# nowal/MASt3R-SLAM

Measured on AMD Instinct MI355X. Metric: keyframe-pair GN iters/sec @512×384, 256 edges; ATE-RMSE vs ref, higher is better.
Workload: dtype f32; 1 GPU; cfg3: gauss_newton_calib op call, 256 keyframe-pair edges (512 directed), 128 keyframes, 384x512, 10 GN iters/step, delta_thresh=0; edges=256, directed_edges=512, keyframes=128, H=384, W=512, parallelism=edge-sharded x1

## Files before the change

include/m3s_backend.h:

```cpp
#ifndef M3S_BACKEND_H
#define M3S_BACKEND_H

#include <stddef.h>
#include <stdint.h>

#ifdef __cplusplus
extern "C" {
#endif

enum {
    M3S_OK = 0,
    M3S_ERR_INVALID = 1,
    M3S_ERR_HIP = 2,
    M3S_ERR_WORKSPACE = 3,
    M3S_ERR_COMM = 4,
    M3S_ERR_TIMEOUT = 5
};

const char* m3s_last_error(void);
const char* m3s_version(void);
void m3s_shutdown(void);

enum {
    M3S_CONTRACT_NVCC = 0,
    M3S_CONTRACT_OFF = 1,
    M3S_CONTRACT_NVCC_RIGHT = 2,
    M3S_CONTRACT_DEFAULT = M3S_CONTRACT_NVCC
};

int m3s_iter_proj(const float* rays, const float* pts, const float* p_init,
                  float* p_new, uint8_t* converged,
                  int64_t B, int64_t H, int64_t W, int64_t N,
                  int max_iter, float lambda_init, float cost_thresh, void* stream);
int m3s_iter_proj_ex(const float* rays, const float* pts, const float* p_init,
                     float* p_new, uint8_t* converged,
                     int64_t B, int64_t H, int64_t W, int64_t N,
                     int max_iter, float lambda_init, float cost_thresh, int contract, void* stream);

int m3s_refine_matches_f16(const uint16_t* D11, const uint16_t* D21,
                           const int64_t* p1, int64_t* p1_new,
                           int64_t B, int64_t H, int64_t W, int64_t N, int64_t F,
                           int radius, int dilation_max, void* stream);
int m3s_refine_matches_f32(const float* D11, const float* D21,
                           const int64_t* p1, int64_t* p1_new,
                           int64_t B, int64_t H, int64_t W, int64_t N, int64_t F,
                           int radius, int dilation_max, void* stream);
int m3s_refine_matches_f64(const double* D11, const double* D21,
                           const int64_t* p1, int64_t* p1_new,
                           int64_t B, int64_t H, int64_t W, int64_t N, int64_t F,
                           int radius, int dilation_max, void* stream);

size_t m3s_match_workspace_bytes(int64_t B, int64_t H, int64_t W, int64_t F);
int m3s_match_iterative_proj(const float* X11, const float* X21, const float* D11, const float* D21,
                             const int64_t* idx_init, int64_t B, int64_t H, int64_t W, int64_t F,
                             int max_iter, float lambda_init, float cost_thresh, float dist_thresh,
                             int radius, int dilation_max, int contract, int64_t* idx_out,
                             uint8_t* valid_out, void* ws, size_t ws_bytes, void* stream);



void m3s_gn_debug_flags(int* out4);
void m3s_gn_pcg_stats(int* out5);
void m3s_gn_pcg_plan(int* out5);

int m3s_gn_check(void* stream);

enum { M3S_GN_POINTS = 0, M3S_GN_RAYS = 1, M3S_GN_CALIB = 2 };

typedef struct m3s_gn_args {
    int mode;
    float* Twc;
    const float* Xs;
    const float* Cs;
    const int64_t* ii;
    const int64_t* jj;
    const int64_t* idx;
    const uint8_t* valid;
    const float* Q;
    int64_t N, HW, E_total, E_local, edge_offset;
    float sigma0;
    float sigma1;
    float C_thresh, Q_thresh;
    const float* K;
    int height, width, pixel_border;
    float z_eps;
    int max_iter;
    float delta_thresh;
    float* dx;
    void* ws;
    size_t ws_bytes;
    void* comm;
    void* stream;
    int order;
    const int64_t* idx_b;
    const uint8_t* valid_b;
    const float* Q_b;
    int64_t E_a;
    int contract;
} m3s_gn_args;
enum {
    M3S_GN_ORDER_DEFAULT = 0,
    M3S_GN_ORDER_FAST = 1,
    M3S_GN_ORDER_REFERENCE = 2
};

size_t m3s_gn_workspace_bytes(int mode, int64_t N, int64_t HW, int64_t E_total, int64_t E_local);

int m3s_gauss_newton(const m3s_gn_args* args);

int m3s_gauss_newton_points(float* Twc, const float* Xs, const float* Cs,
                            const int64_t* ii, const int64_t* jj, const int64_t* idx,
                            const uint8_t* valid, const float* Q,
                            int64_t N, int64_t HW, int64_t E,
                            float sigma_point, float C_thresh, float Q_thresh,
                            int max_iter, float delta_thresh,
                            float* dx, void* ws, size_t ws_bytes, void* stream);
int m3s_gauss_newton_rays(float* Twc, const float* Xs, const float* Cs,
                          const int64_t* ii, const int64_t* jj, const int64_t* idx,
                          const uint8_t* valid, const float* Q,
                          int64_t N, int64_t HW, int64_t E,
                          float sigma_ray, float sigma_dist, float C_thresh, float Q_thresh,
                          int max_iter, float delta_thresh,
                          float* dx, void* ws, size_t ws_bytes, void* stream);
int m3s_gauss_newton_calib(float* Twc, const float* Xs, const float* Cs, const float* K,
                           const int64_t* ii, const int64_t* jj, const int64_t* idx,
                           const uint8_t* valid, const float* Q,
                           int64_t N, int64_t HW, int64_t E,
                           int height, int width, int pixel_border, float z_eps,
                           float sigma_pixel, float sigma_depth, float C_thresh, float Q_thresh,
                           int max_iter, float delta_thresh,
                           float* dx, void* ws, size_t ws_bytes, void* stream);

int m3s_gn_build_system(const m3s_gn_args* args, double* H_host, double* b_host);
int m3s_gn_edge_hessians(const m3s_gn_args* args, float* Hs_host, float* gs_host);

int m3s_gn_plan_info(const int64_t* ii, const int64_t* jj, int64_t E, int64_t N, int32_t* info,
                     int32_t* order, int32_t* round_ptr, int32_t round_cap);

int m3s_prof_begin(void);
int m3s_prof_begin_accum(void);
int m3s_prof_end(double* out , int* n_iter);
int m3s_prof_launch_ms(double* out, int cap);
int m3s_prof_solve_ms(double* out, int cap);


typedef struct m3s_track_args {
    int mode;
    const float* Xf;
    const float* Xk;
    const float* Qk;
    const uint8_t* valid;
    const float* meas_k;
    const uint8_t* valid_meas;
    const float* K;
    const float* T_WCf;
    const float* T_WCk;
    int64_t HW;
    int height, width, pixel_border;
    double z_eps;
    double sigma0;
    double sigma1;
    double huber_k;
    int max_iters;
    double rel_error, delta_norm;
    int check_every;
    float* T_WCf_out;
    float* T_CkCf_out;
    int* info;
    double* cost;
    void* ws;
    size_t ws_bytes;
    void* stream;
} m3s_track_args;

size_t m3s_track_workspace_bytes(int64_t HW);
int m3s_track_workspace_layout(int64_t HW, size_t* partials_offset, int* nblk, int* ld);
int m3s_track_sim3(const m3s_track_args* args);
int m3s_track_last_result(int32_t* info4, double* cost);


int m3s_edge_confidence(const int64_t* idx_i2j, const int64_t* idx_j2i,
                        const uint8_t* valid_match_j, const uint8_t* valid_match_i,
                        const float* Qii, const float* Qjj, const float* Qji, const float* Qij,
                        float Q_conf, int64_t B, int64_t HW, float* Qj, float* Qi, int* counts,
                        void* stream);


enum { M3S_FILTER_WEIGHTED_POINTMAP = 0, M3S_FILTER_INDEP_CONF = 1, M3S_FILTER_RECENT = 2 };

int m3s_pointmap_update(int mode, const float* T, const float* X_new, const float* C_new,
                        float* X, float* C, int64_t HW, void* stream);


typedef struct m3s_recon_args {
  const float* X;
  const float* C;
  const float* n_obs;
  const float* T_WC;
  const uint8_t* rgb;
  const float* K;
  int64_t N, HW;
  int height, width;
  float thresh;
  void* ws;
  size_t ws_bytes;
  void* stream;
} m3s_recon_args;
size_t m3s_recon_workspace_bytes(int64_t N, int64_t HW);
int64_t m3s_recon_tile_points(void);
int m3s_recon_count(const m3s_recon_args* args, int64_t* counts ,
                    int64_t* total );
int m3s_recon_emit(const m3s_recon_args* args, void* out , int64_t capacity);


enum { M3S_HEAD_TOKENS = 0, M3S_HEAD_PLANAR = 1 };
enum { M3S_HEAD_DEPTH_EXP = 0, M3S_HEAD_DEPTH_LINEAR = 1, M3S_HEAD_DEPTH_SQUARE = 2 };
enum { M3S_HEAD_CONF_EXP = 0, M3S_HEAD_CONF_SIGMOID = 1 };
enum { M3S_HEAD_DESC_NORM = 0 };
typedef struct m3s_head_args {
  const float* pts;
  const float* feat;
// ... 65 lines not shown
```

mast3r-slam_amd/csrc/edge_reduce.h:

```cpp
#pragma once

#include <hip/hip_runtime.h>

#include <cstdint>

#include "gn_kernels.h"

namespace m3s {

template <bool COH>
__device__ __forceinline__ void edge_reduce_body(const float* __restrict__ partials, int nchunks,
                                                 const float* __restrict__ Twc,
                                                 const int* __restrict__ ii_loc,
                                                 double* __restrict__ edgeblk, int e) {
    const int tid = threadIdx.x;
    auto ldp = [](const float* q) -> float {
        if constexpr (COH) return __hip_atomic_load(q, __ATOMIC_RELAXED, __HIP_MEMORY_SCOPE_AGENT);
        return *q;
    };
    __shared__ double M[7][7];
    __shared__ double g[7];
    __shared__ double A[7][7];
    __shared__ double AM[7][7];
    float Ti[8];
    if (tid < 3) {
        const float* Tp = Twc + (int64_t)ii_loc[e] * 8;
#pragma unroll
        for (int k = 0; k < 8; k++) Ti[k] = Tp[k];
    }
    if (tid < kNacc) {
        const float* p = partials + (int64_t)e * nchunks * kNaccPad + tid;
        double s = 0.0;
        int c = 0;
        for (; c + 8 <= nchunks; c += 8) {
            float v[8];
#pragma unroll
            for (int u = 0; u < 8; u++) v[u] = ldp(p + (int64_t)(c + u) * kNaccPad);
#pragma unroll
            for (int u = 0; u < 8; u++) s += (double)v[u];
        }
        for (; c < nchunks; c++) s += (double)ldp(p + (int64_t)c * kNaccPad);
        if (tid < 28) {
            int a = 0, r = tid;
            while (r >= 7 - a) { r -= 7 - a; a++; }
            const int b = a + r;
            M[a][b] = s;
            M[b][a] = s;
        } else {
            g[tid - 28] = s;
        }
    }
    if (tid < 49) A[tid / 7][tid % 7] = 0.0;
    __syncthreads();
    if (tid < 3) {
        const double t0 = Ti[0], t1 = Ti[1], t2 = Ti[2];
        const double qx = Ti[3], qy = Ti[4], qz = Ti[5], qw = Ti[6];
        const double s_inv = 1.0 / (double)Ti[7];
        double X[3] = {0, 0, 0};
        X[tid] = 1.0;
        const double uv0 = 2.0 * (qy * X[2] - qz * X[1]);
        const double uv1 = 2.0 * (qz * X[0] - qx * X[2]);
        const double uv2 = 2.0 * (qx * X[1] - qy * X[0]);
        const double R0 = X[0] + qw * uv0 + (qy * uv2 - qz * uv1);
        const double R1 = X[1] + qw * uv1 + (qz * uv0 - qx * uv2);
        const double R2 = X[2] + qw * uv2 + (qx * uv1 - qy * uv0);
        A[0][tid] = s_inv * R0;
        A[1][tid] = s_inv * R1;
        A[2][tid] = s_inv * R2;
        A[3][tid] = s_inv * (t1 * R2 - t2 * R1);
        A[4][tid] = s_inv * (t2 * R0 - t0 * R2);
        A[5][tid] = s_inv * (t0 * R1 - t1 * R0);
        A[6][tid] = s_inv * (t0 * R0 + t1 * R1 + t2 * R2);
        A[3][3 + tid] = R0;
        A[4][3 + tid] = R1;
        A[5][3 + tid] = R2;
        if (tid == 0) A[6][6] = 1.0;
    }
    __syncthreads();
    if (tid < 49) {
        const int a = tid / 7, b = tid % 7;
        double s = 0.0;
#pragma unroll
        for (int p = 0; p < 7; p++) s += A[a][p] * M[p][b];
        AM[a][b] = s;
    }
    __syncthreads();
    double* out = edgeblk + (int64_t)e * kEdgeBlk;
    if (tid < 28) {
        int a = 0, r = tid;
        while (r >= 7 - a) { r -= 7 - a; a++; }
        const int b = a + r;
        double s = 0.0;
#pragma unroll
        for (int p = 0; p < 7; p++) s += AM[a][p] * A[b][p];
        out[tid] = s;
    } else if (tid < 35) {
        const int a = tid - 28;
        double s = 0.0;
#pragma unroll
        for (int p = 0; p < 7; p++) s += A[a][p] * g[p];
        out[tid] = s;
    }
}

}
```

mast3r-slam_amd/csrc/gn_accum.hip:

```cpp
#include <hip/hip_runtime.h>

#include <algorithm>
#include <climits>
#include <cstdint>
#include <type_traits>

#include "edge_reduce.h"
#include "gn_kernels.h"
#include "sim3.h"
#include "wave_reduce.h"

namespace m3s {

__device__ __forceinline__ float vrcp(float a) { return __builtin_amdgcn_rcpf(a); }
__device__ __forceinline__ float vsqrt(float a) { return __builtin_amdgcn_sqrtf(a); }
__device__ __forceinline__ float vlog2(float a) { return __builtin_amdgcn_logf(a); }
__device__ __forceinline__ float sqrt_cr(float a) { return __builtin_sqrtf(a); }
__device__ __forceinline__ bool both(bool a, bool b) { return a && b; }

__device__ __forceinline__ float huber(float r) {
    const float a = fabsf(r);
    return a < 1.345f ? 1.0f : 1.345f * vrcp(a);
}

// ... 767 lines not shown
            put(r * 8u, 0, a);
        } else if constexpr (FIRST) {
            const uchar4 vm4 = ld_off<uchar4>(valid_c, r);
            const longlong2 id01 = ld_off<longlong2>(idx_c, r * 8u);
            const longlong2 id23 = ld_off<longlong2>(idx_c, r * 8u, 1);
            const float4 q4 = ld_off<float4>(Q_c, r * 4u);
            const float4 cj4 = raw.cj_all ? make_float4(0.f, 0.f, 0.f, 0.f) : ld_off<float4>(Cj_c, r * 4u);
            const bool vm[4] = {vm4.x != 0, vm4.y != 0, vm4.z != 0, vm4.w != 0};
            const int64_t ids[4] = {id01.x, id01.y, id23.x, id23.y};
            const float qs[4] = {q4.x, q4.y, q4.z, q4.w};
            const float cjs[4] = {cj4.x, cj4.y, cj4.z, cj4.w};
            int code[4], sqb[4];
#pragma unroll
            for (int s = 0; s < 4; s++) {
                const int ind = match_index(ids[s], vm[s], P.HW);
                const bool ok = vm[s] && (qs[s] > P.Q_thresh) && (raw.ci_all || raw.Ci_b[ind] > P.C_thresh) &&
                                (raw.cj_all || cjs[s] > P.C_thresh);
                code[s] = pack_code(ind, ok, P);
                sqb[s] = __float_as_int(sqrt_cr(qs[s]));
            }
            a = int4{code[0], sqb[0], code[1], sqb[1]};
            b = int4{code[2], sqb[2], code[3], sqb[3]};
            put(r * 8u, 0, a);
            put(r * 8u, 1, b);
        } else {
            a = ld_off<int4>(pk_c, r * 8u);
            if constexpr (NP == 4) b = ld_off<int4>(pk_c, r * 8u, 1);
        }
    };
    auto steps = [&](auto fixc_tag) {
        constexpr bool FIXC = decltype(fixc_tag)::value;
        int4 na = int4{0, 0, 0, 0}, nb = int4{0, 0, 0, 0};
        unsigned r = NP * threadIdx.x;
        if (r < n) {
            records(r, na, nb);
            if constexpr (FIXC) cur.fix_columns(k0 + (int)r, S / P.width);
        }
        auto step = [&](const int4& a, const int4& b, unsigned rr) {
            cur.set(a, b);
            cur.template load<MODE, FIXC>(Xj_c, Xi_b, Zi_b, rr, k0 + (int)rr);
            cur.template compute<MODE>(T, P, acc);
        };
        int4 ma = int4{0, 0, 0, 0}, mb = int4{0, 0, 0, 0};
        if constexpr (FIRST && NP == 4) {
            while (r < n) {
                step(na, nb, r);
                r += S;
                if (r < n) records(r, na, nb);
            }
        } else
        while (r < n) {
            if (r + S < n) records(r + S, ma, mb);
            step(na, nb, r);
            r += S;
            if (r >= n) break;
            if (r + S < n) records(r + S, na, nb);
            step(ma, mb, r);
            r += S;
        }
    };
    if constexpr (RC) {
        if (S % P.width == 0)
            steps(std::true_type{});
        else
            steps(std::false_type{});
    } else {
        steps(std::false_type{});
    }
}

struct FirstSrc {
    EdgeSrc es;
    const float* Cs;
    const int* cok;
    int4* pack_w;
};

template <int MODE, bool COMPACT, bool RCOK = false, bool FIRST = false>
__global__ __launch_bounds__(kAccThreads) void gn_accum_packed_kernel(
    const float* __restrict__ Twc, const float* __restrict__ Xs, const float* __restrict__ Zs,
    const int* __restrict__ ii_loc, const int* __restrict__ jj_loc, const int4* __restrict__ pack,
    AccParams P, const int4* __restrict__ sched, float* __restrict__ partials,
    const int* __restrict__ flags, const float* __restrict__ px, const int* __restrict__ pcnt,
    int* __restrict__ ecnt, double* __restrict__ edgeblk, FirstSrc fs) {
    const int4 tk = sched[blockIdx.x];
    if (flags[kFlagDone]) return;
    const int e = tk.x, c = tk.y, ix = tk.z, jx = tk.w;
    const RelXf T = rel_xf(rel_sim3(load_sim3(Twc + (int64_t)ix * 8), load_sim3(Twc + (int64_t)jx * 8)));

    const int HW = P.HW;
    const int64_t ebase = (int64_t)e * HW;
    const float* __restrict__ Xi_b = Xs + (int64_t)ix * HW * 3;
    const float* __restrict__ Zi_b = MODE == GN_CALIB ? inv_depths(Zs, P) + (int64_t)ix * HW : nullptr;
    const float* __restrict__ Xj_b = Xs + (int64_t)jx * HW * 3;
    const int4* __restrict__ pk_b = pack + ebase / 2;
    const int k0 = c * P.chunk;
    const int k1 = min(k0 + P.chunk, HW);

    float acc[kNacc];
#pragma unroll
    for (int q = 0; q < kNacc; q++) acc[q] = 0.0f;
    if constexpr (COMPACT) {
        const int64_t cb = ((int64_t)e * P.nchunks + c) * P.chunk;
        accum_steps<MODE, false, acc_np<MODE>()>(px + cb * 3, Xi_b, Zi_b, pack + cb / 2, 0, pcnt[(int64_t)e * P.nchunks + c], T, P,
                                 Zs, acc);
    } else {
        RawSrc raw{};
        if constexpr (FIRST) {
            fs.es.at(e, HW, raw.idx, raw.valid, raw.Q);
            raw.Ci_b = fs.Cs + (int64_t)ix * HW;
            raw.Cj_b = fs.Cs + (int64_t)jx * HW;
            raw.pk_w = fs.pack_w + ebase / 2;
            raw.ci_all = fs.cok != nullptr && fs.cok[ix] != 0;
            raw.cj_all = fs.cok != nullptr && fs.cok[jx] != 0;
        }
        constexpr int NP = acc_np<MODE>();
        bool ray = false;
        if constexpr (RCOK && MODE == GN_CALIB) {
            ray = flags[kFlagNotRay] == 0 && (P.width & 3) == 0;
            if (ray) accum_steps<MODE, true, NP, FIRST>(Zs + (int64_t)jx * HW, Xi_b, Zi_b, pk_b, k0, k1, T, P, Zs, acc, raw);
        }
        if (!ray) accum_steps<MODE, false, NP, FIRST>(Xj_b, Xi_b, Zi_b, pk_b, k0, k1, T, P, Zs, acc, raw);
    }
    block_partial(acc, partials + ((int64_t)e * P.nchunks + c) * kNaccPad, ecnt != nullptr);
    if (ecnt != nullptr) {
        __shared__ int s_last;
        asm volatile("s_waitcnt vmcnt(0)" ::: "memory");
        __syncthreads();
        if (threadIdx.x == 0)
            s_last = __hip_atomic_fetch_add(ecnt + e, 1, __ATOMIC_RELAXED, __HIP_MEMORY_SCOPE_AGENT) == P.nchunks - 1;
        __syncthreads();
        if (s_last) {
            edge_reduce_body<true>(partials, P.nchunks, Twc, ii_loc, edgeblk, e);
            if (threadIdx.x == 0) __hip_atomic_store(ecnt + e, 0, __ATOMIC_RELAXED, __HIP_MEMORY_SCOPE_AGENT);
        }
    }
}

hipError_t launch_accum(int mode, bool vec, dim3 grid, hipStream_t st, const float* Twc,
                        const float* Xs, const float* Cs, const int* ii_loc, const int* jj_loc,
                        const EdgeSrc& es, const AccParams& P, const int4* sched, float* partials,
                        const int* flags) {
#define M3S_ACC(MODE, V)                                                                    \
    hipLaunchKernelGGL((gn_accum_kernel<MODE, V>), grid, dim3(kAccThreads), 0, st, Twc, Xs, \
                       Cs, ii_loc, jj_loc, es, P, sched, partials, flags)
    if (mode == GN_RAYS) {
        if (vec) M3S_ACC(GN_RAYS, true); else M3S_ACC(GN_RAYS, false);
    } else if (mode == GN_CALIB) {
        if (vec) M3S_ACC(GN_CALIB, true); else M3S_ACC(GN_CALIB, false);
    } else {
        if (vec) M3S_ACC(GN_POINTS, true); else M3S_ACC(GN_POINTS, false);
    }
#undef M3S_ACC
    return hipGetLastError();
}

hipError_t launch_pack_pre(hipStream_t st, const float* Xs, int64_t N, const float* Cs, const AccParams& P, int* cok,
                           float* Zs, int* flags, const float* K) {
    if (cok != nullptr && N > 0) {
        const int bx = (int)std::max<int64_t>(1, std::min<int64_t>((P.HW + 1023) / 1024, 8192 / std::max<int64_t>(N, 1)));
        hipLaunchKernelGGL(gn_cpass_kernel, dim3(bx, (unsigned)N), dim3(256), 0, st, Cs, P, cok, flags);
    }
    if (Zs) {
        const int64_t total = N * (int64_t)P.HW;
        const int bx = (int)std::max<int64_t>(std::min<int64_t>((P.HW + 255) / 256,
                                                                std::max<int64_t>(8192 / std::max<int64_t>(N, 1), 2)),
                                              (std::max(P.width, P.height) + 255) / 256);
        hipLaunchKernelGGL(gn_depth_kernel, dim3(bx, (unsigned)N), dim3(256), 0, st, Xs, total, Zs, P, flags, K);
    }
    return hipGetLastError();
}

hipError_t launch_pack(int mode, hipStream_t st, int E_local, const float* Xs, int64_t N, const float* Cs,
                       const int* ii_loc, const int* jj_loc, const EdgeSrc& es, const AccParams& P, int* cok,
                       int4* pack, float* px, int* pcnt, const int* flags, bool skip_pack) {
    if (E_local > 0 && px) {
        const dim3 grid((unsigned)P.nchunks, (unsigned)E_local);
        int2* pk = reinterpret_cast<int2*>(pack);
        if (mode == GN_RAYS)
            hipLaunchKernelGGL(gn_pack_compact_kernel<GN_RAYS>, grid, dim3(kAccThreads), 0, st, Xs, Cs, ii_loc,
                               jj_loc, es, P, pk, px, pcnt, flags);
        else if (mode == GN_CALIB)
            hipLaunchKernelGGL(gn_pack_compact_kernel<GN_CALIB>, grid, dim3(kAccThreads), 0, st, Xs, Cs, ii_loc,
                               jj_loc, es, P, pk, px, pcnt, flags);
        else
            hipLaunchKernelGGL(gn_pack_compact_kernel<GN_POINTS>, grid, dim3(kAccThreads), 0, st, Xs, Cs, ii_loc,
                               jj_loc, es, P, pk, px, pcnt, flags);
    } else if (E_local > 0) {
        const dim3 grid((unsigned)((P.HW / 4 + kAccThreads - 1) / kAccThreads), (unsigned)E_local);
        if (!skip_pack)
            hipLaunchKernelGGL(gn_pack_kernel, grid, dim3(kAccThreads), 0, st, Cs, ii_loc, jj_loc, es,
                               P, cok, pack, flags);
    }
    return hipGetLastError();
}

hipError_t launch_accum_packed(int mode, dim3 grid, hipStream_t st, const float* Twc,
                               const float* Xs, const float* Zs, const int* ii_loc,
                               const int* jj_loc, const int4* pack, const AccParams& P,
                               const int4* sched, float* partials, const int* flags, const float* px,
                               const int* pcnt, int* ecnt, double* edgeblk, const EdgeSrc* first_es,
                               const float* Cs, const int* cok) {
    if (P.HW > kPackedMaxHW) return hipErrorInvalidValue;
    if (first_es != nullptr) {
        if (px != nullptr) return hipErrorInvalidValue;
        const FirstSrc fs{*first_es, Cs, cok, const_cast<int4*>(pack)};
        if (mode == GN_RAYS)
            hipLaunchKernelGGL((gn_accum_packed_kernel<GN_RAYS, false, false, true>), grid, dim3(kAccThreads), 0, st,
                               Twc, Xs, Zs, ii_loc, jj_loc, pack, P, sched, partials, flags, px, pcnt, ecnt,
                               edgeblk, fs);
        else if (mode == GN_POINTS)
            hipLaunchKernelGGL((gn_accum_packed_kernel<GN_POINTS, false, false, true>), grid, dim3(kAccThreads), 0, st,
                               Twc, Xs, Zs, ii_loc, jj_loc, pack, P, sched, partials, flags, px, pcnt, ecnt,
                               edgeblk, fs);
        else if (P.raycheck)
            hipLaunchKernelGGL((gn_accum_packed_kernel<GN_CALIB, false, true, true>), grid, dim3(kAccThreads), 0, st,
                               Twc, Xs, Zs, ii_loc, jj_loc, pack, P, sched, partials, flags, px, pcnt, ecnt,
                               edgeblk, fs);
        else
            hipLaunchKernelGGL((gn_accum_packed_kernel<GN_CALIB, false, false, true>), grid, dim3(kAccThreads), 0, st,
                               Twc, Xs, Zs, ii_loc, jj_loc, pack, P, sched, partials, flags, px, pcnt, ecnt,
                               edgeblk, fs);
        return hipGetLastError();
    }
    const FirstSrc fs0{};
#define M3S_ACCP(MODE, CP, RC)                                                                       \
    hipLaunchKernelGGL((gn_accum_packed_kernel<MODE, CP, RC>), grid, dim3(kAccThreads), 0, st, Twc, Xs, Zs, \
                       ii_loc, jj_loc, pack, P, sched, partials, flags, px, pcnt, ecnt, edgeblk, fs0)
#define M3S_ACCP2(MODE, CP) M3S_ACCP(MODE, CP, false)
    const bool cp = px != nullptr;
    if (mode == GN_RAYS) {
        if (cp) M3S_ACCP2(GN_RAYS, true); else M3S_ACCP2(GN_RAYS, false);
    } else if (mode == GN_CALIB) {
        if (cp) M3S_ACCP2(GN_CALIB, true);
        else if (P.raycheck) M3S_ACCP(GN_CALIB, false, true);
        else M3S_ACCP2(GN_CALIB, false);
    } else {
        if (cp) M3S_ACCP2(GN_POINTS, true); else M3S_ACCP2(GN_POINTS, false);
    }
#undef M3S_ACCP2
#undef M3S_ACCP
    return hipGetLastError();
}

}
```

mast3r-slam_amd/csrc/gn_api.hip:

```cpp
#include <hip/hip_runtime.h>

#include <algorithm>
#include <cstdarg>
#include <cstdio>
#include <cstdlib>
#include <cstring>
#include <mutex>
#include <string>
#include <utility>
#include <vector>

#include "gn_host.h"

namespace m3s {

namespace {
thread_local std::string g_err;
}

int g_dbg_flags[4] = {0, 0, 0, 0};
int g_dbg_pcg[5] = {0, 0, 0, 0, 0};
int g_dbg_pcg_plan[5] = {0, 0, 0, 0, 0};

void set_error(const char* fmt, ...) {
    char buf[1024];
    va_list ap;
    va_start(ap, fmt);
    vsnprintf(buf, sizeof(buf), fmt, ap);
    va_end(ap);
    g_err = buf;
}

const char* get_error() { return g_err.c_str(); }

namespace {
struct HostResources {
    std::mutex mu;
    std::vector<std::pair<void*, void (*)(void*)>> items;
    bool shut = false;
};
HostResources& host_resources() {
    static HostResources* r = new HostResources;
    return *r;
}
}

void register_host_resource(void* obj, void (*release)(void*)) {
    HostResources& r = host_resources();
    std::lock_guard<std::mutex> lk(r.mu);
    r.items.emplace_back(obj, release);
}

hipEvent_t Prof::get() {
    if (pool.empty()) {
        static const bool sysfence = env_int("M3S_PROF_SYSFENCE", 0) != 0;
        hipEvent_t e;
        if (sysfence || hipEventCreateWithFlags(&e, hipEventDisableSystemFence) != hipSuccess) {
            (void)hipGetLastError();
            if (hipEventCreate(&e) != hipSuccess) return nullptr;
        }
        return e;
    }
    hipEvent_t e = pool.back();
    pool.pop_back();
    return e;
}

void Prof::mark(hipStream_t st, bool accum, bool first_pack) {
    if (!on || (accum_only && !accum)) return;
    hipEvent_t e = get();
    if (e && hipEventRecord(e, st) == hipSuccess) {
        marks.push_back(e);
        if (accum_only && marks.size() % 2 == 0) first.push_back(first_pack);
    }
}

Prof g_prof;
namespace {
std::vector<double> g_prof_launch_ms;
std::vector<double> g_prof_solve_ms;
}

}

using namespace m3s;

extern "C" const char* m3s_last_error(void) { return m3s::get_error(); }

extern "C" int m3s_gn_check(void* stream) {
    const hipError_t e = hipStreamSynchronize(static_cast<hipStream_t>(stream));
    if (e != hipSuccess) {
        set_error("gn_check: %s", hipGetErrorString(e));
        return M3S_ERR_HIP;
    }
    return m3s::take_deferred_timeout("");
}

extern "C" void m3s_gn_debug_flags(int* out4) {
    for (int k = 0; k < 4; k++) out4[k] = m3s::g_dbg_flags[k];
}

extern "C" void m3s_gn_pcg_stats(int* out5) {
    for (int k = 0; k < 5; k++) out5[k] = m3s::g_dbg_pcg[k];
}

extern "C" void m3s_gn_pcg_plan(int* out5) {
    for (int k = 0; k < 5; k++) out5[k] = m3s::g_dbg_pcg_plan[k];
}

extern "C" const char* m3s_version(void) { return "m3s 0.1.0 gfx950"; }

extern "C" void m3s_shutdown(void) {
    HostResources& r = host_resources();
    std::lock_guard<std::mutex> lk(r.mu);
    if (r.shut) return;
    r.shut = true;
    for (auto& it : r.items) it.second(it.first);
    r.items.clear();
}

namespace {
__attribute__((constructor)) void m3s_register_shutdown() { std::atexit(m3s_shutdown); }
}

extern "C" size_t m3s_gn_workspace_bytes(int mode, int64_t N, int64_t HW, int64_t E_total,
                                         int64_t E_local) {
    if (N < 1 || HW < 1 || E_total < 0 || E_local < 0) return 0;
    return make_layout(mode, N, HW, E_total, E_local).total;
}

extern "C" int m3s_gn_plan_info(const int64_t* ii, const int64_t* jj, int64_t E, int64_t N, int32_t* info,
                                int32_t* order, int32_t* round_ptr, int32_t round_cap) {
    return m3s::plan_info(ii, jj, E, N, info, order, round_ptr, round_cap);
}

extern "C" int m3s_gauss_newton(const m3s_gn_args* args) {
    if (!args) {
        set_error("gauss_newton: null args");
        return M3S_ERR_INVALID;
    }
    return run(*args);
}

namespace {
int ref_edge_records(const m3s_gn_args& a0, Ctx& c, std::vector<float>& rec) {
    m3s_gn_args a = a0;
    a.order = M3S_GN_ORDER_REFERENCE;
    int rc = setup(a, c);
    if (rc) return rc;
    rec.assign((size_t)a.E_local * kRefStride, 0.0f);
    if (a.E_local == 0) return M3S_OK;
    const Layout& L = c.L;
    M3S_HIP_CHECK(launch_accum_ref(a.mode, (int)a.E_local, c.st, a.Twc, a.Xs, a.Cs, c.at<int>(L.ii_loc),
                                   c.at<int>(L.jj_loc), c.es, c.R, c.at<float>(L.edgeblk),
                                   c.at<int>(L.flags)));
    M3S_HIP_CHECK(hipMemcpyAsync(rec.data(), c.at<float>(L.edgeblk), sizeof(float) * rec.size(),
                                 hipMemcpyDeviceToHost, c.st));
    M3S_HIP_CHECK(hipStreamSynchronize(c.st));
    return M3S_OK;
}

double ref_block(const float* D, int blk, int r, int cc) {
    switch (blk) {
        case 0:
        case 3: return (double)D[std::max(r, cc) * 7 + std::min(r, cc)];
        case 1: return -(double)D[cc * 7 + r];
        default: return -(double)D[r * 7 + cc];
    }
}
}

extern "C" int m3s_gn_edge_hessians(const m3s_gn_args* args, float* Hs_host, float* gs_host) {
    if (!args || !Hs_host || !gs_host) {
        set_error("gn_edge_hessians: null argument");
        return M3S_ERR_INVALID;
    }
    Ctx c;
    std::vector<float> rec;
    int rc = ref_edge_records(*args, c, rec);
    if (rc) return rc;
    const int64_t E = args->E_local;
    for (int64_t e = 0; e < E; e++) {
        const float* D = rec.data() + e * kRefStride;
        for (int blk = 0; blk < 4; blk++)
            for (int r = 0; r < 7; r++)
                for (int q = 0; q < 7; q++)
                    Hs_host[((blk * E + e) * 7 + r) * 7 + q] = (float)ref_block(D, blk, r, q);
        for (int q = 0; q < 7; q++) {
            gs_host[(0 * E + e) * 7 + q] = -D[49 + q];
            gs_host[(1 * E + e) * 7 + q] = D[49 + q];
        }
    }
    return M3S_OK;
}

extern "C" int m3s_gn_build_system(const m3s_gn_args* args, double* H_host, double* b_host) {
    if (!args) {
        set_error("gn_build_system: null args");
        return M3S_ERR_INVALID;
    }
    const m3s_gn_args& a = *args;
    if (gn_order(a) == M3S_GN_ORDER_REFERENCE) {
        Ctx c;
        std::vector<float> rec;
        int rc = ref_edge_records(a, c, rec);
        if (rc) return rc;
        const int64_t n = 7 * (a.N - 1);
        std::fill(H_host, H_host + n * n, 0.0);
        std::fill(b_host, b_host + n, 0.0);
        for (int64_t el = 0; el < a.E_local; el++) {
            const float* D = rec.data() + el * kRefStride;
            const int i = c.plan.ii_loc[el] - 1, j = c.plan.jj_loc[el] - 1;
            const int rr[4] = {i, i, j, j}, cc[4] = {i, j, i, j};
            for (int blk = 0; blk < 4; blk++) {
                if (rr[blk] < 0 || cc[blk] < 0) continue;
                for (int r = 0; r < 7; r++)
// ... 177 lines not shown
```

mast3r-slam_amd/csrc/gn_driver.hip:

```cpp
#include <hip/hip_runtime.h>

#include <algorithm>
#include <chrono>
#include <cstdio>
#include <cstring>
#include <mutex>

#include "gn_host.h"
#include "m3s_comm.h"

namespace m3s {

namespace {
void keep_pool() {
    static std::mutex mu;
    static bool done[64] = {false};
    int dev = 0;
    if (hipGetDevice(&dev) != hipSuccess || dev < 0 || dev >= 64) return;
    std::lock_guard<std::mutex> lk(mu);
    if (done[dev]) return;
    done[dev] = true;
    const long mb = env_int("M3S_POOL_KEEP_MB", 1024);
    if (mb <= 0) return;
    hipMemPool_t pool;
// ... 38 lines not shown
    auto al16 = [](const void* ptr) { return ((uintptr_t)ptr & 15) == 0; };
    const bool two = a.idx_b != nullptr;
    c.es.idx[0] = a.idx;
    c.es.valid[0] = a.valid;
    c.es.Q[0] = a.Q;
    c.es.idx[1] = two ? a.idx_b : a.idx;
    c.es.valid[1] = two ? a.valid_b : a.valid;
    c.es.Q[1] = two ? a.Q_b : a.Q;
    c.es.E_a = two ? (int)a.E_a : (int)a.E_local;
    c.vec = (a.HW % 4 == 0) && al16(a.Xs) && al16(a.Cs) && al16(a.idx) && al16(a.valid) &&
            al16(a.Q) && (!two || (al16(a.idx_b) && al16(a.valid_b) && al16(a.Q_b)));
    const int pack_mode = env_int("M3S_GN_PACK", 1);
    c.packed = c.vec && a.E_local > 0 && (pack_mode == 2 || (pack_mode == 1 && a.max_iter >= 3)) &&
               a.HW <= kPackedMaxHW;
    c.compact = c.packed && env_int("M3S_GN_COMPACT", 0) != 0;
    if (a.mode == M3S_GN_CALIB && (a.width >= 65536 || a.height >= 32768)) c.packed = c.compact = false;
    P.pack_uv = c.packed && a.mode == M3S_GN_CALIB;
    P.raycheck = c.packed && !c.compact && a.mode == M3S_GN_CALIB && env_int("M3S_GN_RAYCHECK", 1) != 0;

    c.ref_order = gn_order(a) == M3S_GN_ORDER_REFERENCE;
    if (c.ref_order) {
        c.packed = false;
        RefParams& R = c.R;
        R.s0_inv = (float)(1.0 / (double)a.sigma0);
        R.s1_inv = (a.mode == M3S_GN_POINTS) ? 0.0f : (float)(1.0 / (double)a.sigma1);
        R.C_thresh = a.C_thresh;
        R.Q_thresh = a.Q_thresh;
        R.z_eps = a.z_eps;
        R.width = a.width > 0 ? a.width : 1;
        R.height = a.height;
        R.pixel_border = a.pixel_border;
        R.HW = a.HW;
        R.variant = env_int("M3S_GN_REF_VARIANT", 0);
        R.contract = a.contract;
    }
    int* dflags = c.at<int>(L.flags);
    int* dcok = c.at<int>(L.cok);
    auto pre_pass = [&]() -> int {
        M3S_HIP_CHECK(launch_gn_init(c.st, dflags, P.raycheck ? 0 : 1, dcok, a.N));
        if (c.packed)
            M3S_HIP_CHECK(launch_pack_pre(c.st, a.Xs, a.N, a.Cs, P, !c.compact ? dcok : nullptr,
                                          a.mode == M3S_GN_CALIB ? c.at<float>(L.zs) : nullptr, dflags,
                                          a.mode == M3S_GN_CALIB ? a.K : nullptr));
        return M3S_OK;
    };
    static const bool prepass_early = env_int("M3S_PREPASS", 1) != 0;
    rc = build_plan(a, c.st, c.plan, prepass_early ? pre_pass : std::function<int()>());
    if (!rc && !prepass_early) rc = pre_pass();
    if (rc) return rc;
    if (c.plan.gather)
        M3S_HIP_CHECK(hipMallocAsync((void**)&c.eall,
                                     sizeof(double) * kEdgeBlk * (size_t)c.plan.granks * c.plan.gchunk, c.st));
    const auto s1 = std::chrono::steady_clock::now();
    const Plan& p = c.plan;
    P.fx = p.K[0];
    P.fy = p.K[1];
    P.cx = p.K[2];
    P.cy = p.K[3];
    if (c.ref_order) {
        c.R.fx = p.K[0];
        c.R.fy = p.K[1];
        c.R.cx = p.K[2];
        c.R.cy = p.K[3];
    }
    const size_t ntask = (size_t)a.E_local * L.nchunks;
    const size_t lo = L.ii_loc, hi = L.sched;
    const size_t nslot = c.need_slotmap ? p.slotmap.size() : 0;
    if (c.need_slotmap) {
        rc = c.alloc_dense(L.npad, (int)std::max<int64_t>(a.N - 1, 0));
        if (rc) return rc;
    }
    char* h = stagings().ws.get(hi - lo + sizeof(int) * nslot);
    M3S_REQUIRE(h != nullptr, "gauss_newton: pinned host allocation failed");
    auto put = [&](size_t off, const std::vector<int>& v) {
        if (!v.empty()) std::memcpy(h + (off - lo), v.data(), sizeof(int) * v.size());
    };
    put(L.ii_loc, p.ii_loc);
    put(L.jj_loc, p.jj_loc);
    put(L.blk_ptr, p.blk_ptr);
    put(L.blk_ent, p.blk_ent);
    put(L.blk_ref, p.blk_ref);
    put(L.grad_ptr, p.grad_ptr);
    put(L.grad_ent, p.grad_ent);
    std::memset(h + (L.ecnt - lo), 0, sizeof(int) * (size_t)a.E_local);
    SchedGroups G;
    build_schedule_order(p.ii_loc, p.jj_loc, (int)std::max<int64_t>(a.N, 1), reinterpret_cast<int*>(h + (L.sorder - lo)), G);
    M3S_HIP_CHECK(stagings().ws.upload(c.ws + lo, h, L.sched - lo, c.st));
    M3S_HIP_CHECK(launch_sched_expand(c.st, c.at<int>(L.sorder), c.at<int>(L.ii_loc), c.at<int>(L.jj_loc), L.nchunks,
                                      G, (int64_t)ntask, c.at<int>(L.sched)));
    c.first_pack = early_pack && c.packed && !c.compact && !c.ref_order && a.max_iter > 0 &&
                   env_int("M3S_GN_PACK_FIRST", 1) != 0;
    if (early_pack) {
        rc = prepare_iterations(a, c);
        if (rc) return rc;
        c.pack_issued = true;
    }
    const auto s2 = std::chrono::steady_clock::now();
    if (nslot) {
        std::memcpy(h + (hi - lo), p.slotmap.data(), sizeof(int) * nslot);
        M3S_HIP_CHECK(hipMemcpyAsync(c.dyn + c.o_slot, h + (hi - lo), sizeof(int) * nslot,
                                     hipMemcpyHostToDevice, c.st));
    }
    M3S_HIP_CHECK(stagings().ws.mark(c.st));
    if (prof_host) {
        auto us = [](std::chrono::steady_clock::time_point x, std::chrono::steady_clock::time_point y) {
            return std::chrono::duration<double, std::micro>(y - x).count();
        };
        fprintf(stderr, "gn host: build_plan %.0f us (of which copies + sync %.0f us), params+lists+schedule+pack "
                "%.0f us, rest %.0f us\n", us(s0, s1), g_plan_sync_us, us(s1, s2), us(s2, std::chrono::steady_clock::now()));
    }
    return M3S_OK;
}

int take_deferred_timeout(const char* which) {
    Stagings& sg = stagings();
    if (!sg.tmo_armed) return M3S_OK;
    const int kind = sg.tmo_armed;
    sg.tmo_armed = 0;
    const char* h = sg.tmo.get(64);
    const bool hit = kind == 2 ? *reinterpret_cast<const double*>(h) > 0.0 : *reinterpret_cast<const int*>(h) != 0;
    if (hit) {
        set_error("gauss_newton: %sa device-side wait of the factorisation timed out (the solve was "
                  "discarded; not a singular system)", which);
        return M3S_ERR_TIMEOUT;
    }
    return M3S_OK;
}

int run(const m3s_gn_args& a) {
    static const bool prof_host = env_int("M3S_PROF_HOST", 0) != 0;
    auto now = [] { return std::chrono::steady_clock::now(); };
    auto us = [](std::chrono::steady_clock::time_point x, std::chrono::steady_clock::time_point y) {
        return std::chrono::duration<double, std::micro>(y - x).count();
    };
    const auto t0 = now();
    Ctx c;
    c.need_slotmap = env_int("M3S_SOLVER_DENSE", 0) != 0;
    int rc = setup(a, c, a.N > 1);
    if (rc) return rc;
    rc = take_deferred_timeout("an earlier call: ");
    if (rc) return rc;
    const auto t1 = now();
    const int npose = (int)(a.N - 1);
    if (npose <= 0) return M3S_OK;
    const Layout& L = c.L;
    int* flags = c.at<int>(L.flags);
    std::chrono::steady_clock::time_point t2 = t1, t3 = t1;
    if (!c.ref_order && a.max_iter > 0 && env_int("M3S_EARLY_ACC", 1) != 0) {
        g_prof.mark(c.st);
        rc = enqueue_accumulate(a, c);
        if (rc) return rc;
        c.acc_enqueued = true;
        static const int early_gather = env_int("M3S_EARLY_GATHER", -1);
        if (c.plan.gather && (early_gather > 0 || (early_gather < 0 && comm_is_async(a.comm)))) {
            rc = comm_allgather_f64(a.comm, c.eall, (size_t)c.plan.gchunk * kEdgeBlk, c.st);
            if (rc) return rc;
            c.gathered = true;
        }
    }
    const auto t1b = now();
    if (env_int("M3S_SOLVER_DENSE", 0) == 0 || c.ref_order) {
        choose_sparse_plan(c.plan, npose, c.sp);
        choose_pcg(a, c, c.plan, npose, c.sp);
        t2 = now();
        M3S_REQUIRE(c.sp.npad_tail <= kMaxNpad,
                    "gauss_newton: the dense core of the elimination (%d unknowns) exceeds the "
                    "dense solve limit (%d)", c.sp.npad_tail, kMaxNpad);
        rc = upload_sparse_plan(c.sp, npose, c.st);
        if (rc) return rc;
        t3 = now();
    }
    if (prof_host)
        fprintf(stderr, "gn host: setup %.0f us, early enqueue %.0f us, plan %.0f us, upload %.0f us\n", us(t0, t1),
                us(t1, t1b), us(t1b, t2), us(t2, t3));
    for (int itr = 0; itr < a.max_iter; itr++) {
        if (!c.acc_enqueued) g_prof.mark(c.st);
        rc = enqueue_system(a, c);
        if (rc) return rc;
        g_prof.mark(c.st);
        if (itr == 0) M3S_HIP_CHECK(launch_twc_save(c.st, a.Twc, c.at<float>(L.twc_save), (int)(8 * a.N)));
        const int from = c.sp.pcg_from, lag = c.sp.pcg_lag;
        if (c.sp.pcg && itr >= from) {
            if (c.inv_pending) {
                M3S_HIP_CHECK(hipStreamWaitEvent(c.st, c.inv_done, 0));
                c.inv_pending = false;
            }
            rc = enqueue_pcg(a, c);
            if (rc) return rc;
        }
        rc = enqueue_solve(a, c, c.sp.pcg && itr >= from);
        if (rc) return rc;
        g_prof.mark(c.st);
        if (!c.sp.fused && !c.sp.hybrid)
            M3S_HIP_CHECK(launch_retract(c.st, a.Twc, c.at<double>(L.x), a.dx, (int)a.N,
                                         a.delta_thresh, flags, a.contract));
        if (c.sp.pcg && (itr == from - lag || itr >= from) && itr + 1 < a.max_iter) {
            rc = enqueue_inverse(a, c, itr < from - 1);
            if (rc) return rc;
        }
        g_prof.mark(c.st);
    }
    if (c.may_timeout && a.max_iter > 0) {
        Stagings& sg = stagings();
        char* h = sg.tmo.get(64);
        M3S_REQUIRE(h != nullptr, "gauss_newton: pinned host allocation failed");
        float* save = c.at<float>(L.twc_save);
        const int n8 = (int)(8 * a.N);
        if (a.comm) {
            double* dv = c.at<double>(L.x);
            M3S_HIP_CHECK(launch_flag_export(c.st, flags + kFlagTimeout, dv, 1));
            rc = comm_allreduce_sum_f64(a.comm, dv, 1, c.st);
            if (rc) return rc;
            M3S_HIP_CHECK(launch_twc_restore_on_flag(c.st, a.Twc, save, n8, dv, 1, sg.tmo.dev));
            if (!sg.tmo.dev) M3S_HIP_CHECK(hipMemcpyAsync(h, dv, sizeof(double), hipMemcpyDeviceToHost, c.st));
            sg.tmo_armed = 2;
        } else {
            M3S_HIP_CHECK(launch_twc_restore_on_flag(c.st, a.Twc, save, n8, flags + kFlagTimeout, 0, sg.tmo.dev));
            if (!sg.tmo.dev)
                M3S_HIP_CHECK(hipMemcpyAsync(h, flags + kFlagTimeout, sizeof(int), hipMemcpyDeviceToHost, c.st));
            sg.tmo_armed = 1;
        }
        M3S_HIP_CHECK(sg.tmo.mark(c.st));
        static const bool sync_report = env_int("M3S_GN_TIMEOUT_SYNC", 0) != 0;
        if (sync_report) {
            rc = take_deferred_timeout("");
            if (rc) return rc;
        }
    }
    if (const int dbg = env_int("M3S_GN_DEBUG_FLAGS", 0)) {
        int hf[kNumFlags];
        M3S_HIP_CHECK(hipMemcpyAsync(hf, flags, sizeof(hf), hipMemcpyDeviceToHost, c.st));
        M3S_HIP_CHECK(hipStreamSynchronize(c.st));
        g_dbg_flags[0] = hf[kFlagDone];
        g_dbg_flags[1] = (hf[kFlagFail] | hf[kFlagFailed]) != 0;
        g_dbg_flags[2] = c.packed ? 1 : 0;
        g_dbg_flags[3] = (c.packed && c.P.raycheck && hf[kFlagNotRay] == 0) ? 1 : 0;
        g_dbg_pcg[0] = hf[kFlagPcgRuns];
        g_dbg_pcg[1] = hf[kFlagPcgSteps];
        g_dbg_pcg[2] = hf[kFlagPcgFall];
        g_dbg_pcg[3] = c.sp.pcg ? 1 : 0;
        g_dbg_pcg[4] = c.sp.pcg ? c.sp.pcg_from : 0;
        g_dbg_pcg_plan[0] = c.sp.pcg ? c.sp.pcg_R : 0;
        g_dbg_pcg_plan[1] = c.sp.pcg ? c.sp.pcg_nwg : 0;
        g_dbg_pcg_plan[2] = c.sp.pcg && c.sp.pcg_onex ? 1 : 0;
        g_dbg_pcg_plan[3] = c.sp.pcg ? c.sp.pcg_lag : 0;
        g_dbg_pcg_plan[4] = c.sp.pcg ? c.sp.pcg_nitem : 0;
        if (dbg != 2)
            fprintf(stderr, "gn flags: done %d fail %d not_ray %d timeout %d packed %d pcg runs %d steps %d fallbacks %d\n",
                    hf[kFlagDone], g_dbg_flags[1], hf[kFlagNotRay], hf[kFlagTimeout], (int)c.packed,
                    hf[kFlagPcgRuns], hf[kFlagPcgSteps], hf[kFlagPcgFall]);
    }
    return M3S_OK;
}

}
```

mast3r-slam_amd/csrc/gn_enqueue.hip:

```cpp
#include <hip/hip_runtime.h>

#include <algorithm>
#include <cstdio>
#include <cstdlib>

#include "gn_host.h"
#include "m3s_comm.h"

namespace m3s {

namespace {
struct PcgSide {
    static constexpr int kMaxDev = 64;
    hipStream_t ss[kMaxDev] = {};
    hipEvent_t e1[kMaxDev] = {}, e2[kMaxDev] = {};
    static void release(void* p) {
        PcgSide* s = static_cast<PcgSide*>(p);
        for (int d = 0; d < kMaxDev; d++) {
            if (s->e1[d]) (void)hipEventDestroy(s->e1[d]);
            if (s->e2[d]) (void)hipEventDestroy(s->e2[d]);
            if (s->ss[d]) (void)hipStreamDestroy(s->ss[d]);
            s->e1[d] = s->e2[d] = nullptr;
            s->ss[d] = nullptr;
        }
    }
};
thread_local PcgSide* t_pcg_side = nullptr;
int pcg_side(hipStream_t& ss, hipEvent_t& e1, hipEvent_t& e2) {
    if (!t_pcg_side) {
        t_pcg_side = new PcgSide;
        register_host_resource(t_pcg_side, &PcgSide::release);
    }
    int dev = 0;
    M3S_HIP_CHECK(hipGetDevice(&dev));
    M3S_REQUIRE(dev >= 0 && dev < PcgSide::kMaxDev, "gauss_newton: device %d out of range", dev);
    PcgSide& p = *t_pcg_side;
    if (!p.ss[dev]) {
        M3S_HIP_CHECK(hipStreamCreateWithFlags(&p.ss[dev], hipStreamNonBlocking));
        M3S_HIP_CHECK(hipEventCreateWithFlags(&p.e1[dev], hipEventDisableTiming | hipEventDisableSystemFence));
        M3S_HIP_CHECK(hipEventCreateWithFlags(&p.e2[dev], hipEventDisableTiming | hipEventDisableSystemFence));
    }
    ss = p.ss[dev];
    e1 = p.e1[dev];
    e2 = p.e2[dev];
    return M3S_OK;
}
}

int prepare_iterations(const m3s_gn_args& a, Ctx& c) {
    if (!c.packed) return M3S_OK;
    const Layout& L = c.L;
    M3S_HIP_CHECK(launch_pack(a.mode, c.st, (int)a.E_local, a.Xs, a.N, a.Cs, c.at<int>(L.ii_loc),
                              c.at<int>(L.jj_loc), c.es, c.P, c.at<int>(L.cok), c.at<int4>(L.pack),
                              c.compact ? c.at<float>(L.packx) : nullptr, c.at<int>(L.pcnt),
                              c.at<int>(L.flags), c.first_pack));
    return M3S_OK;
}

int enqueue_system(const m3s_gn_args& a, Ctx& c) {
    const Layout& L = c.L;
    int* flags = c.at<int>(L.flags);
    const int npose_r = (int)(a.N - 1);
    if (c.ref_order) {
        M3S_REQUIRE(c.sp.enabled, "gauss_newton: the reference order needs the block-sparse solver");
        g_prof.mark(c.st, true);
        M3S_HIP_CHECK(launch_accum_ref(a.mode, (int)a.E_local, c.st, a.Twc, a.Xs, a.Cs,
                                       c.at<int>(L.ii_loc), c.at<int>(L.jj_loc), c.es,
                                       c.R, c.at<float>(L.edgeblk), flags));
        g_prof.mark(c.st, true);
        SparsePlan& sp = c.sp;
        double* sys = sp.dptr<double>(sp.o_sys);
        M3S_HIP_CHECK(launch_assemble_ref(c.st, c.at<float>(L.edgeblk), c.at<int>(L.blk_ptr),
                                          c.at<int>(L.blk_ref), c.at<int>(L.grad_ptr),
                                          c.at<int>(L.grad_ent), c.plan.nblk, sp.nblocks, npose_r,
                                          sp.bpad, sys, flags));
        if (a.comm) {
            const size_t count = (size_t)sp.bpad + (size_t)c.plan.nblk * 49;
            int rc = comm_allreduce_sum_f64(a.comm, sys, count, c.st);
            if (rc) return rc;
        }
        return M3S_OK;
    }
    if (!c.acc_enqueued) {
        int rc = enqueue_accumulate(a, c);
        if (rc) return rc;
    }
    c.acc_enqueued = false;
    return enqueue_assembly(a, c);
}

int enqueue_accumulate(const m3s_gn_args& a, Ctx& c) {
    const Layout& L = c.L;
    int* flags = c.at<int>(L.flags);
    if (a.E_local > 0) {
        g_prof.mark(c.st, true);
        const dim3 grid((unsigned)(L.nchunks * a.E_local));
        const bool fuse_reduce = env_int("M3S_GN_FUSE_REDUCE", 1) != 0;
        const bool fused = c.packed && fuse_reduce;
        const bool was_first = c.packed && c.first_pack;
        if (c.packed) {
            M3S_HIP_CHECK(launch_accum_packed(a.mode, grid, c.st, a.Twc, a.Xs, c.at<float>(L.zs),
                                              c.at<int>(L.ii_loc), c.at<int>(L.jj_loc),
                                              c.at<int4>(L.pack), c.P, c.at<int4>(L.sched),
                                              c.at<float>(L.partials), flags,
                                              c.compact ? c.at<float>(L.packx) : nullptr,
                                              c.at<int>(L.pcnt), fused ? c.at<int>(L.ecnt) : nullptr,
                                              c.eblk(), c.first_pack ? &c.es : nullptr,
                                              a.Cs, c.at<int>(L.cok)));
            c.first_pack = false;
        } else
            M3S_HIP_CHECK(launch_accum(a.mode, c.vec, grid, c.st, a.Twc, a.Xs, a.Cs,
                                       c.at<int>(L.ii_loc), c.at<int>(L.jj_loc), c.es, c.P,
                                       c.at<int4>(L.sched), c.at<float>(L.partials),
                                       flags));
        g_prof.mark(c.st, true, was_first);
        if (!fused)
            M3S_HIP_CHECK(launch_edge_reduce((int)a.E_local, c.st, c.at<float>(L.partials), L.nchunks,
                                             a.Twc, c.at<int>(L.ii_loc), c.eblk(), flags));
    }
    return M3S_OK;
}

int enqueue_assembly(const m3s_gn_args& a, Ctx& c) {
    const Layout& L = c.L;
    int* flags = c.at<int>(L.flags);
    const int npose = (int)(a.N - 1);
    if (c.plan.gather && !c.gathered) {
        int rc = comm_allgather_f64(a.comm, c.eall, (size_t)c.plan.gchunk * kEdgeBlk, c.st);
        if (rc) return rc;
    }
    c.gathered = false;
    const bool reduce = a.comm && !c.plan.gather;
    if (c.sp.enabled) {
        SparsePlan& sp = c.sp;
        double* sys = sp.dptr<double>(sp.o_sys);
        M3S_HIP_CHECK(launch_assemble(c.st, c.eblk_all(), c.at<int>(L.blk_ptr),
                                      c.at<int>(L.blk_ent), c.at<int>(L.grad_ptr),
                                      c.at<int>(L.grad_ent), c.plan.nblk, sp.nblocks, npose, sp.bpad,
                                      sys, flags));
        if (reduce) {
            const size_t count = (size_t)sp.bpad + (size_t)c.plan.nblk * 49;
            int rc = comm_allreduce_sum_f64(a.comm, sys, count, c.st);
            if (rc) return rc;
        }
        return M3S_OK;
    }
    M3S_HIP_CHECK(launch_compact(c.st, c.eblk_all(), c.at<int>(L.blk_ptr),
                                 c.at<int>(L.blk_ent), c.at<int>(L.grad_ptr),
                                 c.at<int>(L.grad_ent), c.plan.nblk, npose,
                                 c.at<double>(L.compact), flags));
    if (reduce) {
        const size_t count = (size_t)c.plan.nblk * 28 + (size_t)npose * 7;
        int rc = comm_allreduce_sum_f64(a.comm, c.at<double>(L.compact), count, c.st);
        if (rc) return rc;
    }
    return M3S_OK;
}

namespace {
constexpr int kSolveDbgWords = kSolveDbgCycles + 1;
unsigned long long* solve_dbg_buffer() {
    static unsigned long long* p = nullptr;
    if (p == nullptr && hipMalloc(&p, sizeof(unsigned long long) * kSolveDbgWords) != hipSuccess) p = nullptr;
    if (p != nullptr) (void)hipMemset(p, 0, sizeof(unsigned long long) * kSolveDbgWords);
    return p;
}
hipError_t launch_gn_solve_dbg(hipStream_t st, const SolveArgs& S) {
    hipError_t e = launch_gn_solve(st, S);
    if (e != hipSuccess || !S.debug || S.dbg == nullptr) return e;
    unsigned long long h[kSolveDbgWords];
    e = hipMemcpyAsync(h, S.dbg, sizeof(h), hipMemcpyDeviceToHost, st);
    if (e == hipSuccess) e = hipStreamSynchronize(st);
    if (e == hipSuccess) print_solve_debug(h);
    return e;
}
}

int enqueue_solve(const m3s_gn_args& a, Ctx& c, bool fallback) {
    const Layout& L = c.L;
    const int npose = (int)(a.N - 1);
    int* flags = c.at<int>(L.flags);
    if (!c.sp.enabled) {
        c.may_timeout = true;
        M3S_HIP_CHECK(launch_solve(c.st, c.at<double>(L.compact), c.dyn_at<int>(c.o_slot), c.plan.nblk,
                                   npose, 7 * npose, L.npad, c.dyn_at<double>(c.o_dense),
                                   c.dyn_at<double>(c.o_linv), c.at<double>(L.x), flags, ++c.chol_epoch));
        return M3S_OK;
    }
    SparsePlan& sp = c.sp;
    SolveArgs S{};
    S.npose = npose;
    S.b = sp.dptr<double>(sp.o_sys);
    S.A = S.b + sp.bpad;
    S.y = sp.dptr<double>(sp.o_y);
    S.Lstore = sp.dptr<double>(sp.o_L);
    S.W = sp.dptr<double>(sp.o_W);
    S.Lg = sp.dptr<double>(sp.o_Lg);
    S.x = c.at<double>(L.x);
    S.meta = sp.iptr(0);
    S.nmeta = (int)sp.nints;
    S.meta_lds = solve_lds_bytes(S.nmeta) <= (size_t)kSolveMaxLds && env_int("M3S_SOLVE_META_LDS", 1);
    S.o_rounds = (int)sp.i_rounds;
    S.o_nodes = (int)sp.i_nodes;
    S.o_fptr = (int)sp.i_fptr;
    S.o_fronts = (int)sp.i_fronts;
    S.o_tg = (int)sp.i_tg;
    S.o_tc = (int)sp.i_tc;
    S.o_rtg = (int)sp.i_rtg;
    S.o_rc = (int)sp.i_rc;
    S.o_tail = (int)sp.i_tail;
    S.o_tmap = (int)sp.i_tmap;
    S.nrounds = (int)sp.rounds.size();
    S.zero_blk = sp.zero_blk;
    S.ntail = sp.ntail;
// ... 38 lines not shown
        }
        S.do_fwd = S.do_tail = S.do_back = 1;
        M3S_HIP_CHECK(launch_gn_solve_dbg(c.st, S));
        return M3S_OK;
    }
    double* A = S.A;
    double* b = S.b;
    double* y = S.y;
    double* Ls = S.Lstore;
    double* W = S.W;
    double* x = S.x;
    static const int df_mode = env_int("M3S_SOLVE_DF", 1);
    const bool df = df_mode == 2 || (df_mode == 1 && fallback);
    if (df) {
        c.may_timeout = true;
        SpRoundsArgs ca{};
        ca.inl = sp.iptr(sp.i_inl);
        ca.tc3 = sp.iptr(sp.i_tc3);
        ca.rc4 = sp.iptr(sp.i_rc4);
        ca.rounds = sp.iptr(sp.i_rounds);
        ca.tmap = sp.iptr(sp.i_tmap);
        ca.tail = sp.iptr(sp.i_tail);
        ca.A = A;
        ca.b = b;
        ca.Lstore = Ls;
        ca.W = W;
        ca.y = y;
        ca.Hd = sp.ntail > 0 ? sp.dptr<double>(sp.o_dense) : nullptr;
        ca.flags = flags;
        ca.nrounds = (int)sp.rounds.size();
        ca.ntail = sp.ntail;
        ca.npad = sp.npad_tail;
        M3S_HIP_CHECK(launch_sp_rounds_df(c.st, ca, sp.dptr<int>(sp.o_dfcnt)));
    } else {
        for (const SpRound& R : sp.rounds)
            M3S_HIP_CHECK(launch_sp_round(c.st, sp.iptr(sp.i_inl), R.tbeg + R.rbeg, R.nbt, R.nrt,
                                          sp.iptr(sp.i_tc3), sp.iptr(sp.i_rc4), A, b, Ls, W, y, flags));
    }
    const bool core_df = sp.core_df;
    if (sp.hybrid && core_df && sp.ntail > 0) {
        c.may_timeout = true;
        if (!df)
            M3S_HIP_CHECK(launch_sp_tail_fill(c.st, A, b, sp.iptr(sp.i_tmap), sp.iptr(sp.i_tail), sp.ntail,
                                              sp.npad_tail, sp.dptr<double>(sp.o_dense), flags));
        M3S_HIP_CHECK(launch_dense_factor_solve(c.st, sp.npad_tail, sp.dptr<double>(sp.o_dense),
                                                sp.dptr<double>(sp.o_linv), sp.dptr<double>(sp.o_xd), flags,
                                                ++c.chol_epoch));
        S.xd = sp.dptr<double>(sp.o_xd);
        S.Hd = nullptr;
        S.nmeta = (int)sp.nints_back;
        S.meta_lds = 1;
        S.do_fwd = 0;
        S.do_tail = 0;
        S.do_back = 1;
        S.x_tail_global = 1;
        M3S_HIP_CHECK(launch_gn_solve_dbg(c.st, S));
        return M3S_OK;
    }
    if (sp.hybrid) {
        M3S_REQUIRE(sp.fused_tail, "gauss_newton: a %d-pose hybrid core exceeds the in-register factorisation",
                    sp.ntail);
        if (!df)
            M3S_HIP_CHECK(launch_sp_tail_fill(c.st, A, b, sp.iptr(sp.i_tmap), sp.iptr(sp.i_tail),
                                              sp.ntail, sp.npad_tail, sp.dptr<double>(sp.o_dense), flags));
        S.Hd = sp.ntail > 0 ? sp.dptr<double>(sp.o_dense) : nullptr;
        S.npad_h = sp.npad_tail;
        S.nmeta = (int)sp.nints_back;
        S.meta_lds = 1;
        S.do_fwd = 0;
        S.do_tail = S.do_back = 1;
        M3S_HIP_CHECK(launch_gn_solve_dbg(c.st, S));
        return M3S_OK;
    }
    if (sp.ntail > 0) c.may_timeout = true;
    M3S_HIP_CHECK(launch_sp_tail(c.st, A, b, sp.iptr(sp.i_tmap), sp.iptr(sp.i_tail), sp.ntail,
                                 sp.npad_tail, sp.dptr<double>(sp.o_dense), sp.dptr<double>(sp.o_linv),
                                 sp.dptr<double>(sp.o_xd), x, flags, ++c.chol_epoch, !df));
    for (auto it = sp.rounds.rbegin(); it != sp.rounds.rend(); ++it)
        M3S_HIP_CHECK(launch_sp_back(c.st, it->nnodes, sp.iptr(sp.i_nodes), sp.iptr(sp.i_fptr),
                                     sp.iptr(sp.i_fronts), it->node_begin, Ls, W, y, x, flags));
    return M3S_OK;
}

int enqueue_inverse(const m3s_gn_args& a, Ctx& c, bool snapshot) {
    const SparsePlan& sp = c.sp;
    const size_t shift = snapshot ? sp.o_snap - sp.o_L : 0;
    if (snapshot) {
        M3S_REQUIRE(sp.snap_bytes > 0, "PCG: no factor snapshot buffer");
        M3S_HIP_CHECK(hipMemcpyAsync(sp.dbuf + sp.o_snap, sp.dbuf + sp.o_L, sp.snap_bytes, hipMemcpyDeviceToDevice, c.st));
    }
    InvArgs v{};
    v.n = 7 * (int)(a.N - 1);
    v.ldx = sp.pcg_ldx;
    v.nrounds = (int)sp.rounds.size();
    v.ntail = sp.ntail;
    v.npad = sp.npad_tail;
    v.rounds = sp.iptr(sp.i_rounds);
    v.nodes = sp.iptr(sp.i_nodes);
    v.fptr = sp.iptr(sp.i_fptr);
    v.fronts = sp.iptr(sp.i_fronts);
    v.inl = sp.iptr(sp.i_inl);
    v.rc4 = sp.iptr(sp.i_rc4);
    v.tail = sp.iptr(sp.i_tail);
    v.Lstore = sp.dptr<double>(sp.o_L + shift);
    v.W = sp.dptr<double>(sp.o_W + shift);
    v.Hd = sp.dptr<double>(sp.o_dense + shift);
    v.Linv = sp.dptr<double>(sp.o_linv + shift);
    v.X = sp.dptr<double>(sp.o_pcgx);
    v.Xt = sp.dptr<float>(sp.o_pcgxt);
    v.ldt = sp.pcg_ldt;
    v.flags = c.at<int>(c.L.flags);
    static const bool side = env_int("M3S_PCG_SIDE", 1) != 0;
    if (!side) {
        M3S_HIP_CHECK(launch_sp_inverse(c.st, v));
        return M3S_OK;
    }
    hipStream_t ss;
    hipEvent_t e1, e2;
    int rc = pcg_side(ss, e1, e2);
    if (rc) return rc;
    M3S_HIP_CHECK(hipEventRecord(e1, c.st));
    M3S_HIP_CHECK(hipStreamWaitEvent(ss, e1, 0));
    static const bool dbg = env_int("M3S_PCG_DEBUG", 0) != 0;
    hipEvent_t t0 = nullptr, t1 = nullptr;
    static long long* ibuf = nullptr;
    if (dbg && !ibuf && hipMalloc(&ibuf, sizeof(long long) * 8) != hipSuccess) ibuf = nullptr;
    v.dbg = dbg ? ibuf : nullptr;
    if (dbg) {
        if (ibuf) M3S_HIP_CHECK(hipMemsetAsync(ibuf, 0, sizeof(long long) * 8, ss));
        M3S_HIP_CHECK(hipEventCreate(&t0));
        M3S_HIP_CHECK(hipEventCreate(&t1));
        M3S_HIP_CHECK(hipEventRecord(t0, ss));
    }
    M3S_HIP_CHECK(launch_sp_inverse(ss, v));
    if (dbg) {
        M3S_HIP_CHECK(hipEventRecord(t1, ss));
        M3S_HIP_CHECK(hipEventSynchronize(t1));
        float ms = 0.f;
        M3S_HIP_CHECK(hipEventElapsedTime(&ms, t0, t1));
        long long h[8] = {0};
        if (ibuf) M3S_HIP_CHECK(hipMemcpy(h, ibuf, sizeof(h), hipMemcpyDeviceToHost));
        fprintf(stderr, "pcg inverse (M refresh): %.1f us, %d workgroups; wg0: init %.1f fwd rounds %.1f core %.1f back rounds %.1f f32 copy %.1f us\n",
                ms * 1e3, (v.n + 15) / 16, (h[1] - h[0]) * 0.01, (h[2] - h[1]) * 0.01, (h[3] - h[2]) * 0.01,
                (h[4] - h[3]) * 0.01, (h[5] - h[4]) * 0.01);
        (void)hipEventDestroy(t0);
        (void)hipEventDestroy(t1);
    }
    M3S_HIP_CHECK(hipEventRecord(e2, ss));
    c.inv_pending = true;
    c.inv_done = e2;
    return M3S_OK;
}

int enqueue_pcg(const m3s_gn_args& a, Ctx& c) {
    const SparsePlan& sp = c.sp;
    PcgArgs g{};
    g.b = sp.dptr<double>(sp.o_sys);
    g.A = g.b + sp.bpad;
    g.adj_ptr = sp.iptr(sp.i_apt);
    g.adj = reinterpret_cast<const int2*>(sp.iptr(sp.i_adj));
    g.nitem = sp.pcg_nitem;
    g.R4 = pcg_r4(sp.pcg_R);
    g.Xt = sp.dptr<float>(sp.o_pcgxt);
    g.ldt = sp.pcg_ldt;
    g.n = 7 * (int)(a.N - 1);
    g.nv = sp.pcg_nv;
    g.onex = sp.pcg_onex ? 1 : 0;
    g.R = sp.pcg_R;
    g.nwg = sp.pcg_nwg;
    g.gran = reinterpret_cast<unsigned long long*>(sp.dbuf + sp.o_gran);
    static const int kmax = std::max(1, std::min(200, env_int("M3S_PCG_KMAX", 30)));
    static const double tol = [] {
        const char* e = getenv("M3S_PCG_TOL");
        return e ? atof(e) : 1e-6;
    }();
    g.kmax = kmax;
    g.tol2 = tol * tol;
    g.tag0 = 1u + (unsigned)c.pcg_launches * (unsigned)(2 * kmax + 2);
    c.pcg_launches++;
    const char* ft = getenv("M3S_TEST_FORCE_TIMEOUT");
    g.spin_limit = (ft && atoi(ft) != 0) ? 0 : (1 << 22);
    g.Twc = a.Twc;
    g.dx = a.dx;
    g.N = (int)a.N;
    g.delta_thresh = a.delta_thresh;
    g.contract = a.contract;
    g.flags = c.at<int>(c.L.flags);
    static const bool dbg = env_int("M3S_PCG_DEBUG", 0) != 0;
    static long long* dbuf = nullptr;
    if (dbg && !dbuf && hipMalloc(&dbuf, sizeof(long long) * kPcgDbgSlots) != hipSuccess) dbuf = nullptr;
    if (dbg && dbuf) M3S_HIP_CHECK(hipMemsetAsync(dbuf, 0, sizeof(long long) * kPcgDbgSlots, c.st));
    g.dbg = dbg ? dbuf : nullptr;
    M3S_HIP_CHECK(launch_pcg(c.st, g));
    if (g.dbg) {
        long long h[kPcgDbgSlots];
        M3S_HIP_CHECK(hipMemcpyAsync(h, dbuf, sizeof(h), hipMemcpyDeviceToHost, c.st));
// ... 16 lines not shown
```

mast3r-slam_amd/csrc/gn_host.h:

```cpp
#pragma once

#include <hip/hip_runtime.h>

#include <algorithm>
#include <cstdint>
#include <functional>
#include <utility>
#include <vector>

#include "../../include/m3s_backend.h"
#include "gn_kernels.h"
#include "m3s_common.h"
#include "sparse_plan.h"

namespace m3s {

int env_int(const char* name, int dflt);

inline size_t align_up(size_t x, size_t a) { return (x + a - 1) / a * a; }

struct Prof {
    bool on = false;
    std::vector<hipEvent_t> pool;
    std::vector<hipEvent_t> marks;
    hipEvent_t get();
    bool accum_only = false;
    std::vector<char> first;
    void mark(hipStream_t st, bool accum = false, bool first_pack = false);
};
extern Prof g_prof;

extern int g_dbg_flags[4];
extern int g_dbg_pcg[5];
extern int g_dbg_pcg_plan[5];

struct Staging {
    char* buf = nullptr;
    char* dev = nullptr;
    size_t cap = 0;
    hipEvent_t done = nullptr;
    bool pending = false;
    static void release(void* p);
    char* get(size_t bytes);
    hipError_t upload(void* dst, const char* h, size_t bytes, hipStream_t st);
    hipError_t download(char* h, const void* src, size_t bytes, hipStream_t st);
    hipError_t mark(hipStream_t st);
};
struct Stagings {
    Staging in;
    Staging out;
    Staging ws;
    Staging tmo;
    int tmo_armed = 0;
    static void release(void* p);
};
Stagings& stagings();

struct Layout {
    size_t partials, edgeblk, compact, x, flags, ii_loc, jj_loc, blk_ptr, blk_ent, blk_ref, grad_ptr,
        grad_ent, ecnt, cok, sorder, sched, pack, packx, pcnt, zs, twc_save, total;
    int nchunks, npad, nblk_max;
};
Layout make_layout(int mode, int64_t N, int64_t HW, int64_t E_total, int64_t E_local);
int chunk_points(int64_t HW, int nchunks);

struct Plan {
    int nblk = 0;
    std::vector<int> ii_loc, jj_loc;
    std::vector<int> blk_ptr, blk_ent;
    std::vector<int> blk_ref;
    std::vector<int> grad_ptr, grad_ent;
    std::vector<int> slotmap;
    std::vector<std::pair<int, int>> pairs;
    float K[4] = {0, 0, 0, 0};
    bool gather = false;
    int grank = 0, granks = 1, gchunk = 0;
};

Plan& tls_plan();
SparsePlan& tls_sparse_plan();

struct Ctx {
    bool need_slotmap = false;
    bool packed = false;
    bool compact = false;
    bool ref_order = false;
    bool pack_issued = false;
    bool acc_enqueued = false;
    bool gathered = false;
    bool first_pack = false;
    RefParams R;
    Layout L;
    Plan& plan = tls_plan();
    SparsePlan& sp = tls_sparse_plan();
    AccParams P;
    EdgeSrc es{};
    bool vec;
    char* ws;
    hipStream_t st = nullptr;
    char* dyn = nullptr;
    size_t o_dense = 0, o_linv = 0, o_slot = 0;
    double* eall = nullptr;
    double* eblk() const {
        return eall ? eall + (size_t)plan.grank * plan.gchunk * kEdgeBlk : at<double>(L.edgeblk);
    }
    const double* eblk_all() const { return eall ? eall : at<double>(L.edgeblk); }
    int chol_epoch = 0;
    int pcg_launches = 0;
    bool inv_pending = false;
    hipEvent_t inv_done = nullptr;
    bool may_timeout = false;
    template <typename T>
    T* at(size_t off) const { return reinterpret_cast<T*>(ws + off); }
    template <typename T>
    T* dyn_at(size_t off) const { return reinterpret_cast<T*>(dyn + off); }
    int alloc_dense(int npad, int npose) {
        size_t off = 0;
        auto take = [&](size_t bytes) {
            size_t o = off;
            off = align_up(off + std::max<size_t>(bytes, 8), 256);
            return o;
        };
        o_dense = take(sizeof(double) * (size_t)(npad + kCholTile) * npad);
        o_linv = take(chol_linv_bytes(npad));
        o_slot = take(sizeof(int) * (size_t)npose * npose);
        M3S_HIP_CHECK(hipMallocAsync((void**)&dyn, off, st));
        M3S_HIP_CHECK(hipMemsetAsync(chol_ready_ptr(dyn_at<double>(o_linv), npad), 0, chol_ready_bytes(npad), st));
        return M3S_OK;
    }
    Ctx() { sp.reset(); }
    Ctx(const Ctx&) = delete;
    Ctx& operator=(const Ctx&) = delete;
    ~Ctx() {
        if (inv_pending && inv_done) (void)hipStreamWaitEvent(st, inv_done, 0);
        if (sp.dbuf) (void)hipFreeAsync(sp.dbuf, st);
        sp.dbuf = nullptr;
        if (dyn) (void)hipFreeAsync(dyn, st);
        if (eall) (void)hipFreeAsync(eall, st);
    }
};

extern double g_plan_sync_us;
int gn_order(const m3s_gn_args& a);
int validate(const m3s_gn_args& a);
void build_schedule_order(const std::vector<int>& ii_loc, const std::vector<int>& jj_loc, int nkey, int* order,
                          SchedGroups& G);
int build_plan(const m3s_gn_args& a, hipStream_t st, Plan& plan, const std::function<int()>& before_wait = {});
void choose_sparse_plan(const Plan& plan, int npose, SparsePlan& sp);
void choose_pcg(const m3s_gn_args& a, const Ctx& c, const Plan& plan, int npose, SparsePlan& sp);
int upload_sparse_plan(SparsePlan& sp, int npose, hipStream_t st);
int plan_info(const int64_t* ii, const int64_t* jj, int64_t E, int64_t N, int32_t* info, int32_t* order,
              int32_t* round_ptr, int32_t round_cap);

int prepare_iterations(const m3s_gn_args& a, Ctx& c);
int enqueue_system(const m3s_gn_args& a, Ctx& c);
int enqueue_accumulate(const m3s_gn_args& a, Ctx& c);
int enqueue_assembly(const m3s_gn_args& a, Ctx& c);
int enqueue_solve(const m3s_gn_args& a, Ctx& c, bool fallback = false);
int enqueue_inverse(const m3s_gn_args& a, Ctx& c, bool snapshot);
int enqueue_pcg(const m3s_gn_args& a, Ctx& c);

int setup(const m3s_gn_args& a, Ctx& c, bool early_pack = false);
int run(const m3s_gn_args& a);
int take_deferred_timeout(const char* which);

}
```

mast3r-slam_amd/csrc/gn_kernels.h:

```cpp
#pragma once

#include <hip/hip_runtime.h>

#include <cstdint>

namespace m3s {

enum { GN_POINTS = 0, GN_RAYS = 1, GN_CALIB = 2 };

#ifndef M3S_ACC_THREADS
#define M3S_ACC_THREADS 256
#endif
constexpr int kAccThreads = M3S_ACC_THREADS;
constexpr int kNacc = 35;
constexpr int kNaccPad = 36;
constexpr int kEdgeBlk = 36;
constexpr int kCholTile = 64;
constexpr int64_t kPackedMaxHW = int64_t(1) << 28;

constexpr int kFlagDone = 0;
constexpr int kFlagFail = 1;
constexpr int kFlagNotRay = 2;
constexpr int kFlagTimeout = 3;
constexpr int kFlagFailed = 4;
constexpr int kFlagSkipSolve = 6;
constexpr int kFlagPcgRuns = 7;
constexpr int kFlagPcgSteps = 8;
constexpr int kFlagPcgFall = 9;
constexpr int kFlagPcgAbort = 10;
constexpr int kNumFlags = 16;
__device__ __forceinline__ bool solve_skipped(const int* flags) {
    return (flags[kFlagDone] | flags[kFlagSkipSolve]) != 0;
}

struct EdgeSrc {
    const int64_t* idx[2];
    const uint8_t* valid[2];
    const float* Q[2];
    int E_a;
    __device__ __forceinline__ void at(int e, int64_t HW, const int64_t*& i, const uint8_t*& v,
                                       const float*& q) const {
        const int h = e >= E_a;
        const int64_t off = (int64_t)(h ? e - E_a : e) * HW;
        i = idx[h] + off;
        v = valid[h] + off;
        q = Q[h] + off;
    }
};

__host__ __device__ constexpr int sym_idx(int a, int b) {
    return a * 7 - a * (a - 1) / 2 + (b - a);
}

struct AccParams {
    float s0_inv, s1_inv;
    float C_thresh, Q_thresh;
    float fx, fy, cx, cy;
    float pb_lo, pb_hi_u, pb_hi_v;
    float z_eps;
    unsigned div_m;
    int div_sh;
    int width, height;
    int HW;
    int chunk;
    int nchunks;
    int nkf;
    int pack_uv;
    int raycheck;
};

constexpr int kRefVals = 56;
constexpr int kRefStride = 64;
struct RefParams {
    float s0_inv, s1_inv;
    float C_thresh, Q_thresh;
    float fx, fy, cx, cy;
    float z_eps;
    int width, height, pixel_border;
    int64_t HW;
    int variant;
    int contract;
};
constexpr int kRefVarLogRatio = 1;
constexpr int kRefVarRcp = 2;
constexpr int kRefVarHuberMin = 4;
hipError_t launch_accum_ref(int mode, int E_local, hipStream_t st, const float* Twc, const float* Xs,
                            const float* Cs, const int* ii_loc, const int* jj_loc, const EdgeSrc& es,
                            const RefParams& P, float* out, const int* flags);
hipError_t launch_assemble_ref(hipStream_t st, const float* ref, const int* blk_ptr, const int* blk_ref,
                               const int* grad_ptr, const int* grad_ent, int nblk, int nblocks,
                               int npose, int bpad, double* out, const int* flags);

hipError_t launch_accum(int mode, bool vec, dim3 grid, hipStream_t st, const float* Twc,
                        const float* Xs, const float* Cs, const int* ii_loc, const int* jj_loc,
                        const EdgeSrc& es, const AccParams& P, const int4* sched, float* partials,
                        const int* flags);
hipError_t launch_pack(int mode, hipStream_t st, int E_local, const float* Xs, int64_t N, const float* Cs,
                       const int* ii_loc, const int* jj_loc, const EdgeSrc& es, const AccParams& P, int* cok,
                       int4* pack, float* px, int* pcnt, const int* flags, bool skip_pack = false);
hipError_t launch_pack_pre(hipStream_t st, const float* Xs, int64_t N, const float* Cs, const AccParams& P, int* cok,
                           float* Zs, int* flags, const float* K);
hipError_t launch_gn_init(hipStream_t st, int* flags, int not_ray, int* cok, int64_t n);
hipError_t launch_accum_packed(int mode, dim3 grid, hipStream_t st, const float* Twc,
                               const float* Xs, const float* Zs, const int* ii_loc,
                               const int* jj_loc, const int4* pack, const AccParams& P,
                               const int4* sched, float* partials, const int* flags, const float* px,
                               const int* pcnt, int* ecnt = nullptr, double* edgeblk = nullptr,
                               const EdgeSrc* first_es = nullptr, const float* Cs = nullptr,
                               const int* cok = nullptr);
hipError_t launch_edge_reduce(int E_local, hipStream_t st, const float* partials, int nchunks,
                              const float* Twc, const int* ii_loc, double* edgeblk,
                              const int* flags);
hipError_t launch_compact(hipStream_t st, const double* edgeblk, const int* blk_ptr,
                          const int* blk_ent, const int* grad_ptr, const int* grad_ent, int nblk,
                          int npose, double* compact, const int* flags);
hipError_t launch_assemble(hipStream_t st, const double* edgeblk, const int* blk_ptr,
                           const int* blk_ent, const int* grad_ptr, const int* grad_ent, int nblk,
                           int nblocks, int npose, int bpad, double* out, const int* flags);
hipError_t launch_solve(hipStream_t st, const double* compact, const int* slotmap, int nblk,
                        int npose, int n, int npad, double* Hd, double* Linv, double* x,
                        int* flags, int epoch);
constexpr int kMaxNpad = 8192;
size_t chol_ready_bytes(int npad);
inline size_t chol_linv_bytes(int npad) {
    return sizeof(double) * (size_t)npad * kCholTile + chol_ready_bytes(npad);
}
inline int* chol_ready_ptr(double* Linv, int npad) {
    return reinterpret_cast<int*>(Linv + (size_t)npad * kCholTile);
}
struct DfScatter {
    const int* tail;
    int ntail;
    double* xpose;
};
hipError_t launch_chol_dataflow(hipStream_t st, int npad, double* Hd, double* Linv, int* ready,
                                int epoch, int* flags, double* x = nullptr, const DfScatter* g = nullptr);
hipError_t launch_dense_factor_solve(hipStream_t st, int npad, double* Hd, double* Linv,
                                     double* x, int* flags, int epoch, const DfScatter* g = nullptr);
hipError_t launch_sp_tail_scatter(hipStream_t st, const double* xd, const int* tail, int ntail, double* x,
                                  const int* flags);
constexpr int kSpInline = 9;
constexpr int kSpRec = 4 + 4 * kSpInline;
struct SpRoundsArgs {
    const int *inl, *tc3, *rc4, *rounds, *tmap, *tail;
    double *A, *b, *Lstore, *W, *y, *Hd;
    int* flags;
    int nrounds, ntail, npad;
};
hipError_t launch_sp_rounds_df(hipStream_t st, const SpRoundsArgs& args, int* cnt);
inline int sp_rounds_df_words(int nrounds) { return (4 + nrounds + 31) / 32 * 32; }
hipError_t launch_sp_round(hipStream_t st, const int* inl, int ibeg, int nbt, int nrt, const int* tc3,
                           const int* rc4, double* A, double* b, double* Lstore, double* W, double* y,
                           int* flags);
hipError_t launch_sp_back(hipStream_t st, int nnodes, const int* nodes, const int* fptr,
                          const int* fronts, int node_begin, const double* Lstore, const double* W,
                          const double* y, double* x, const int* flags);
hipError_t launch_sp_tail_fill(hipStream_t st, const double* A, const double* b, const int* tmap,
                               const int* tail, int ntail, int npad, double* Hd, const int* flags);
hipError_t launch_sp_tail(hipStream_t st, const double* A, const double* b, const int* tmap,
                          const int* tail, int ntail, int npad, double* Hd, double* Linv,
                          double* xd, double* x, int* flags, int epoch, bool fill = true);
hipError_t launch_fill_only(hipStream_t st, const double* compact, const int* slotmap, int nblk,
                            int npose, int n, int npad, double* Hd, const int* flags);
struct InvArgs {
    int n, ldx, nrounds, ntail, npad;
    const int *rounds, *nodes, *fptr, *fronts, *inl, *rc4, *tail;
    const double *Lstore, *W, *Hd, *Linv;
    double* X;
    float* Xt;
    int ldt;
    const int* flags;
    long long* dbg;
};
size_t inverse_lds_bytes(int npad);
hipError_t launch_sp_inverse(hipStream_t st, const InvArgs& a);
constexpr int kPcgThreads = 768;
constexpr int kPcgMaxN = 2304;
constexpr int kPcgMaxLds = 160 * 1024 - 1024;
struct PcgArgs {
    const double *b, *A;
    const int* adj_ptr;
    const int2* adj;
    int nitem, R4;
    const float* Xt;
    int ldt;
    int n, nv, R, nwg;
    int onex;
    unsigned long long* gran;
    unsigned tag0;
    double tol2;
    int kmax, spin_limit;
    float* Twc;
// ... 68 lines not shown
```

mast3r-slam_amd/csrc/gn_kernels.hip:

```cpp
#include <hip/hip_runtime.h>

#include <algorithm>
#include <cstdint>

#include "edge_reduce.h"
#include "gn_kernels.h"
#include "sim3.h"

namespace m3s {


__global__ __launch_bounds__(64) void gn_edge_reduce_kernel(const float* __restrict__ partials,
                                                            int nchunks,
                                                            const float* __restrict__ Twc,
                                                            const int* __restrict__ ii_loc,
                                                            double* __restrict__ edgeblk,
                                                            const int* __restrict__ flags) {
    if (flags[kFlagDone]) return;
    edge_reduce_body<false>(partials, nchunks, Twc, ii_loc, edgeblk, blockIdx.x);
}

__global__ __launch_bounds__(64) void gn_compact_kernel(
    const double* __restrict__ edgeblk, const int* __restrict__ blk_ptr,
    const int* __restrict__ blk_ent, const int* __restrict__ grad_ptr,
    const int* __restrict__ grad_ent, int nblk, int npose, double* __restrict__ compact,
    const int* __restrict__ flags) {
    if (flags[kFlagDone]) return;
    const int s = blockIdx.x;
    const int tid = threadIdx.x;
    if (s < nblk) {
        if (tid < 28) {
            double acc = 0.0;
            const int k1 = blk_ptr[s + 1];
            for (int k = blk_ptr[s]; k < k1; k += 8) {
                int code[8];
                double v[8];
#pragma unroll
                for (int u = 0; u < 8; u++) code[u] = k + u < k1 ? blk_ent[k + u] : 0;
#pragma unroll
                for (int u = 0; u < 8; u++) v[u] = k + u < k1 ? edgeblk[(int64_t)(code[u] >> 1) * kEdgeBlk + tid] : 0.0;
#pragma unroll
                for (int u = 0; u < 8; u++)
                    if (k + u < k1) acc += (code[u] & 1) ? -v[u] : v[u];
            }
            compact[(int64_t)s * 28 + tid] = acc;
        }
    } else {
        const int p = s - nblk;
        if (p < npose && tid < 7) {
            double acc = 0.0;
            const int k1 = grad_ptr[p + 1];
            for (int k = grad_ptr[p]; k < k1; k += 8) {
                int code[8];
                double v[8];
#pragma unroll
                for (int u = 0; u < 8; u++) code[u] = k + u < k1 ? grad_ent[k + u] : 0;
#pragma unroll
                for (int u = 0; u < 8; u++) v[u] = k + u < k1 ? edgeblk[(int64_t)(code[u] >> 1) * kEdgeBlk + 28 + tid] : 0.0;
#pragma unroll
                for (int u = 0; u < 8; u++)
                    if (k + u < k1) acc += (code[u] & 1) ? -v[u] : v[u];
            }
            compact[(int64_t)nblk * 28 + p * 7 + tid] = acc;
        }
    }
}

__global__ __launch_bounds__(64) void gn_assemble_kernel(
    const double* __restrict__ edgeblk, const int* __restrict__ blk_ptr,
    const int* __restrict__ blk_ent, const int* __restrict__ grad_ptr,
    const int* __restrict__ grad_ent, int nblk, int nblocks, int npose, int bpad,
    double* __restrict__ out, const int* __restrict__ flags) {
    if (flags[kFlagDone]) return;
    const int s = blockIdx.x;
    const int tid = threadIdx.x;
    if (s < nblk) {
        if (tid < 28) {
            double acc = 0.0;
            const int k1 = blk_ptr[s + 1];
            for (int k = blk_ptr[s]; k < k1; k += 8) {
                int code[8];
                double v[8];
#pragma unroll
                for (int u = 0; u < 8; u++) code[u] = k + u < k1 ? blk_ent[k + u] : 0;
#pragma unroll
                for (int u = 0; u < 8; u++) v[u] = k + u < k1 ? edgeblk[(int64_t)(code[u] >> 1) * kEdgeBlk + tid] : 0.0;
#pragma unroll
                for (int u = 0; u < 8; u++)
                    if (k + u < k1) acc += (code[u] & 1) ? -v[u] : v[u];
            }
            int a = 0, r = tid;
            while (r >= 7 - a) {
                r -= 7 - a;
                a++;
            }
            const int b = a + r;
            double* blk = out + bpad + (int64_t)s * 49;
            blk[a * 7 + b] = acc;
            blk[b * 7 + a] = acc;
        }
    } else if (s < nblocks) {
        if (tid < 49) out[bpad + (int64_t)s * 49 + tid] = 0.0;
    } else {
        const int p = s - nblocks;
        if (p < npose && tid < 7) {
            double acc = 0.0;
            const int k1 = grad_ptr[p + 1];
            for (int k = grad_ptr[p]; k < k1; k += 8) {
                int code[8];
                double v[8];
#pragma unroll
                for (int u = 0; u < 8; u++) code[u] = k + u < k1 ? grad_ent[k + u] : 0;
#pragma unroll
                for (int u = 0; u < 8; u++) v[u] = k + u < k1 ? edgeblk[(int64_t)(code[u] >> 1) * kEdgeBlk + 28 + tid] : 0.0;
#pragma unroll
                for (int u = 0; u < 8; u++)
                    if (k + u < k1) acc += (code[u] & 1) ? -v[u] : v[u];
            }
            out[p * 7 + tid] = acc;
        }
    }
}

__global__ __launch_bounds__(256) void gn_fill_dense_kernel(const double* __restrict__ compact,
                                                            const int* __restrict__ slotmap,
                                                            int nblk, int npose, int n, int npad,
                                                            double* __restrict__ Hd,
                                                            const int* __restrict__ flags) {
    if (solve_skipped(flags)) return;
    const int64_t total = (int64_t)(npad + kCholTile) * npad;
    for (int64_t id = (int64_t)blockIdx.x * blockDim.x + threadIdx.x; id < total;
         id += (int64_t)gridDim.x * blockDim.x) {
        const int r = (int)(id / npad), c = (int)(id % npad);
        double val;
        if (r > npad) {
            val = 0.0;
        } else if (r == npad) {
            val = c < n ? compact[(int64_t)nblk * 28 + c] : 0.0;
        } else if (r < n && c < n) {
            const int br = r / 7, bc = c / 7;
            const int slot = slotmap[(int64_t)br * npose + bc];
            const int a = r % 7, b = c % 7;
            val = slot >= 0 ? compact[(int64_t)slot * 28 + (a <= b ? sym_idx(a, b) : sym_idx(b, a))]
                            : 0.0;
        } else {
            val = (r == c) ? 1.0 : 0.0;
        }
        Hd[id] = val;
    }
}


constexpr int T = kCholTile;

__device__ __forceinline__ double rcp_f64(double d) {
    double r = __builtin_amdgcn_rcp(d);
    r = r * (2.0 - d * r);
    r = r * (2.0 - d * r);
    return r;
}

constexpr int kPotrfThreads = 512;
constexpr int LDP = T + 1;

__device__ __forceinline__ double rsqrt_f64(double d) {
    double r = __builtin_amdgcn_rsq(d);
    r = r * (1.5 - 0.5 * d * r * r);
    r = r * (1.5 - 0.5 * d * r * r);
    return r;
}

template <int S>
__device__ __forceinline__ void inverse_stage(const double (*L)[LDP], double (*Li)[LDP],
                                              double (*Tm)[LDP], int tid) {
    constexpr int P = T / (2 * S);
    constexpr int NOUT = P * S * S;
    for (int id = tid; id < NOUT; id += kPotrfThreads) {
        const int pi = id / (S * S), rem = id % (S * S);
        const int a = rem / S, bb = rem % S;
        const int p = pi * 2 * S;
        double acc = 0.0;
#pragma unroll
        for (int m = 0; m < S; m++)
            if (m >= bb) acc = fma(L[p + S + a][p + m], Li[p + m][p + bb], acc);
        Tm[p + S + a][p + bb] = acc;
    }
    __syncthreads();
    for (int id = tid; id < NOUT; id += kPotrfThreads) {
        const int pi = id / (S * S), rem = id % (S * S);
        const int a = rem / S, bb = rem % S;
        const int p = pi * 2 * S;
        double acc = 0.0;
#pragma unroll
        for (int m = 0; m < S; m++)
            if (m <= a) acc = fma(Li[p + S + a][p + S + m], Tm[p + S + m][p + bb], acc);
        Li[p + S + a][p + bb] = -acc;
    }
    __syncthreads();
}

__global__ __launch_bounds__(kPotrfThreads) void chol_potrf_kernel(double* __restrict__ Hd,
                                                                   int npad, int k,
                                                                   double* __restrict__ Linv,
// ... 482 lines not shown
```

mast3r-slam_amd/csrc/gn_plan.hip:

```cpp
#include <hip/hip_runtime.h>

#include <algorithm>
#include <chrono>
#include <cstdlib>
#include <cstring>

#include "gn_host.h"
#include "m3s_comm.h"

namespace m3s {

void Staging::release(void* p) {
    Staging* s = static_cast<Staging*>(p);
    if (s->pending) (void)hipEventSynchronize(s->done);
    if (s->done) (void)hipEventDestroy(s->done);
    if (s->buf) (void)hipHostFree(s->buf);
    s->buf = s->dev = nullptr;
    s->cap = 0;
    s->done = nullptr;
    s->pending = false;
}
char* Staging::get(size_t bytes) {
    if (pending) {
        (void)hipEventSynchronize(done);
// ... 30 lines not shown
    return hipMemcpyAsync(h, src, bytes, hipMemcpyDeviceToHost, st);
}
hipError_t Staging::mark(hipStream_t st) {
    if (!done) {
        hipError_t e = hipEventCreateWithFlags(&done, hipEventDisableTiming);
        if (e != hipSuccess) return e;
    }
    hipError_t e = hipEventRecord(done, st);
    pending = e == hipSuccess;
    return e;
}
void Stagings::release(void* p) {
    Stagings* s = static_cast<Stagings*>(p);
    Staging::release(&s->in);
    Staging::release(&s->out);
    Staging::release(&s->ws);
    Staging::release(&s->tmo);
    s->tmo_armed = 0;
}
namespace {
thread_local Stagings* t_stagings = nullptr;
}
Stagings& stagings() {
    if (!t_stagings) {
        t_stagings = new Stagings;
        register_host_resource(t_stagings, &Stagings::release);
    }
    return *t_stagings;
}

namespace {
int chunk_target() {
    static int t = [] {
        const char* e = getenv("M3S_ACC_CHUNK");
        return e ? std::max(1024, atoi(e)) : 16384;
    }();
    return t;
}

int choose_nchunks(int64_t HW, int64_t E_local) {
    int64_t nc = (HW + chunk_target() - 1) / chunk_target();
    const int64_t want = (4096 + std::max<int64_t>(E_local, 1) - 1) / std::max<int64_t>(E_local, 1);
    nc = std::max(nc, want);
    const int64_t max_nc = std::max<int64_t>(1, (HW + 1023) / 1024);
    nc = std::min(std::max<int64_t>(nc, 1), max_nc);
    int64_t chunk = align_up((size_t)((HW + nc - 1) / nc), 4);
    nc = (HW + chunk - 1) / chunk;
    return (int)std::max<int64_t>(nc, 1);
}
}

int chunk_points(int64_t HW, int nchunks) {
    return (int)align_up((size_t)((HW + nchunks - 1) / nchunks), 4);
}

Layout make_layout(int mode, int64_t N, int64_t HW, int64_t E_total, int64_t E_local) {
    Layout L{};
    const int64_t npose = std::max<int64_t>(N - 1, 0);
    const int64_t n = 7 * npose;
    L.nchunks = choose_nchunks(HW, E_total);
    L.npad = (int)std::max<int64_t>(kCholTile, align_up((size_t)n, kCholTile));
    L.nblk_max = (int)(npose + E_total);
    size_t off = 0;
    auto take = [&](size_t bytes) {
        size_t o = off;
        off = align_up(off + std::max<size_t>(bytes, 1), 256);
        return o;
    };
    L.partials = take(sizeof(float) * (size_t)E_local * L.nchunks * kNaccPad);
    static_assert(sizeof(float) * kRefStride <= sizeof(double) * kEdgeBlk, "edge record");
    L.edgeblk = take(sizeof(double) * (size_t)E_local * kEdgeBlk);
    L.compact = take(sizeof(double) * ((size_t)L.nblk_max * 28 + (size_t)npose * 7));
    L.x = take(sizeof(double) * (size_t)L.npad);
    L.flags = take(sizeof(int) * kNumFlags);
    L.cok = take(sizeof(int) * (size_t)std::max<int64_t>(N, 1));
    L.twc_save = take(sizeof(float) * 8 * (size_t)std::max<int64_t>(N, 1));
    L.ii_loc = take(sizeof(int) * (size_t)E_local);
    L.jj_loc = take(sizeof(int) * (size_t)E_local);
    L.blk_ptr = take(sizeof(int) * ((size_t)L.nblk_max + 1));
    L.blk_ent = take(sizeof(int) * (size_t)std::max(E_local, E_total) * 4);
    L.blk_ref = take(sizeof(int) * (size_t)E_local * 4);
    L.grad_ptr = take(sizeof(int) * ((size_t)npose + 1));
    L.grad_ent = take(sizeof(int) * (size_t)std::max(E_local, E_total) * 2);
    L.ecnt = take(sizeof(int) * (size_t)E_local);
    L.sorder = take(sizeof(int) * (size_t)E_local);
    L.sched = take(sizeof(int) * 4 * (size_t)E_local * L.nchunks);
    if (env_int("M3S_GN_COMPACT", 0) != 0) {
        const size_t cap = (size_t)E_local * (size_t)L.nchunks * (size_t)chunk_points(HW, L.nchunks);
        L.pack = take(8 * std::max(cap, (size_t)E_local * (size_t)HW));
        L.packx = take(12 * cap);
        L.pcnt = take(sizeof(int) * (size_t)E_local * L.nchunks);
    } else {
        L.pack = take(8 * (size_t)E_local * (size_t)HW);
        L.packx = L.pcnt = L.pack;
    }
    L.zs = take(mode == M3S_GN_CALIB ? sizeof(float) * (2 * (size_t)N + 1) * (size_t)HW + 64 : 0);
    L.total = off;
    return L;
}

void build_schedule_order(const std::vector<int>& ii_loc, const std::vector<int>& jj_loc, int nkey, int* order,
                          SchedGroups& G) {
    const int E = (int)ii_loc.size();
    static const bool off = [] {
        const char* e = getenv("M3S_ACC_SCHED");
        return e && atoi(e) == 0;
    }();
    G = SchedGroups{};
    G.off = off ? 1 : 0;
    if (off || E == 0) return;
    static thread_local std::vector<int> tmp, cnt;
    tmp.resize(E);
    auto pass = [&](const std::vector<int>& key, const int* src, int* dst) {
        cnt.assign((size_t)nkey + 1, 0);
        for (int k = 0; k < E; k++) cnt[key[src ? src[k] : k] + 1]++;
        for (int v = 0; v < nkey; v++) cnt[v + 1] += cnt[v];
        for (int k = 0; k < E; k++) {
            const int e = src ? src[k] : k;
            dst[cnt[key[e]]++] = e;
        }
    };
    pass(ii_loc, nullptr, tmp.data());
    pass(jj_loc, tmp.data(), order);
    constexpr int NG = 8;
    G.q = E;
    for (int g = 0; g < NG; g++) {
        G.lo[g] = (int)((int64_t)E * g / NG);
        G.n[g] = (int)((int64_t)E * (g + 1) / NG) - G.lo[g];
        G.q = std::min(G.q, G.n[g]);
    }
    for (int g = 0; g < NG; g++)
        if (G.n[g] > G.q) G.big[G.nbig++] = g;
}

namespace {
int plan_pairs(const int64_t* hii, const int64_t* hjj, int64_t E, int64_t N, Plan& plan, std::vector<int>& iopt,
               std::vector<int>& jopt) {
    const int npose = (int)(N - 1);
    iopt.resize(E);
    jopt.resize(E);
    int64_t lo = 0, hi = -1;
    for (int64_t e = 0; e < E; e++) {
        lo = std::min({lo, hii[e], hjj[e]});
        hi = std::max({hi, hii[e], hjj[e]});
    }
    size_t nuniq = 0;
    if (lo >= 0 && hi < std::max<int64_t>(1 << 16, 8 * (E + N))) {
        static thread_local std::vector<int> rank;
        rank.assign((size_t)hi + 1, 0);
        for (int64_t e = 0; e < E; e++) rank[hii[e]] = rank[hjj[e]] = 1;
        for (int64_t id = 0; id <= hi; id++)
            if (rank[id]) rank[id] = (int)nuniq++;
        if ((int64_t)nuniq <= N)
            for (int64_t e = 0; e < E; e++) {
                iopt[e] = rank[hii[e]] - 1;
                jopt[e] = rank[hjj[e]] - 1;
            }
    } else {
        std::vector<int64_t> u(hii, hii + E);
        u.insert(u.end(), hjj, hjj + E);
        std::sort(u.begin(), u.end());
        u.erase(std::unique(u.begin(), u.end()), u.end());
        nuniq = u.size();
        auto row_of = [&](int64_t id) { return (int)(std::lower_bound(u.begin(), u.end(), id) - u.begin()); };
        if ((int64_t)nuniq <= N)
            for (int64_t e = 0; e < E; e++) {
                iopt[e] = row_of(hii[e]) - 1;
                jopt[e] = row_of(hjj[e]) - 1;
            }
    }
    M3S_REQUIRE((int64_t)nuniq <= N,
                "gauss_newton: %lld unique keyframe ids in ii/jj but only %lld poses in Twc/Xs",
                (long long)nuniq, (long long)N);
    plan.slotmap.assign((size_t)std::max(npose, 0) * std::max(npose, 0), -1);
    for (int q = 0; q < npose; q++) plan.slotmap[(size_t)q * npose + q] = q;
    plan.nblk = npose;
    plan.pairs.clear();
    for (int64_t e = 0; e < E; e++) {
        const int i = iopt[e], j = jopt[e];
        if (i >= 0 && j >= 0 && i != j && plan.slotmap[(size_t)i * npose + j] < 0) {
            plan.slotmap[(size_t)i * npose + j] = plan.slotmap[(size_t)j * npose + i] = plan.nblk++;
            plan.pairs.push_back(std::make_pair(std::min(i, j), std::max(i, j)));
        }
    }
    return M3S_OK;
}
}

double g_plan_sync_us = 0;

int build_plan(const m3s_gn_args& a, hipStream_t st, Plan& plan, const std::function<int()>& before_wait) {
    const int64_t E = a.E_total;
    int grank = 0, granks = 1;
    if (a.comm && gn_order(a) != M3S_GN_ORDER_REFERENCE && env_int("M3S_GN_GATHER", 1) != 0) {
        int rc = comm_rank_size(a.comm, &grank, &granks);
        if (rc) return rc;
    }
    const size_t hb_ranges = align_up(sizeof(int64_t) * 2 * (size_t)E + 64, 64);
    char* hb = stagings().in.get(hb_ranges + sizeof(double) * 2 * (size_t)granks);
    M3S_REQUIRE(hb != nullptr, "gauss_newton: pinned host allocation failed");
    int64_t* hii = reinterpret_cast<int64_t*>(hb);
    int64_t* hjj = hii + E;
    float* Kh = reinterpret_cast<float*>(hjj + E);
    double* hr = reinterpret_cast<double*>(hb + hb_ranges);
    double* dr = nullptr;
    if (granks > 1) {
        hr[2 * grank] = (double)a.edge_offset;
        hr[2 * grank + 1] = (double)a.E_local;
        M3S_HIP_CHECK(hipMallocAsync((void**)&dr, sizeof(double) * 2 * (size_t)granks, st));
        Staging& in = stagings().in;
        M3S_HIP_CHECK(in.upload(dr + 2 * grank, reinterpret_cast<const char*>(hr + 2 * grank), sizeof(double) * 2, st));
        int rc = comm_allgather_f64(a.comm, dr, 2, st);
        if (rc) {
            (void)hipFreeAsync(dr, st);
            return rc;
        }
        M3S_HIP_CHECK(in.download(reinterpret_cast<char*>(hr), dr, sizeof(double) * 2 * (size_t)granks, st));
        M3S_HIP_CHECK(hipFreeAsync(dr, st));
    }
    const auto c0 = std::chrono::steady_clock::now();
    Staging& in = stagings().in;
    if (E > 0) {
        M3S_HIP_CHECK(in.download(reinterpret_cast<char*>(hii), a.ii, sizeof(int64_t) * E, st));
        M3S_HIP_CHECK(in.download(reinterpret_cast<char*>(hjj), a.jj, sizeof(int64_t) * E, st));
    }
    if (a.mode == M3S_GN_CALIB)
        M3S_HIP_CHECK(in.download(reinterpret_cast<char*>(Kh), a.K, sizeof(float) * 9, st));
    if (before_wait) {
        static thread_local hipEvent_t copied = nullptr;
        if (!copied) M3S_HIP_CHECK(hipEventCreateWithFlags(&copied, hipEventDisableTiming));
        M3S_HIP_CHECK(hipEventRecord(copied, st));
        int rc = before_wait();
        if (rc) return rc;
        M3S_HIP_CHECK(hipEventSynchronize(copied));
    } else {
        M3S_HIP_CHECK(hipStreamSynchronize(st));
    }
    g_plan_sync_us = std::chrono::duration<double, std::micro>(std::chrono::steady_clock::now() - c0).count();
    std::vector<int> gpos;
    plan.gather = false;
    plan.grank = grank;
    plan.granks = granks;
    plan.gchunk = 0;
    if (granks > 1) {
        int64_t chunk = 0;
        std::vector<int> cover(E, 0);
        bool ok = true;
        gpos.assign(E, -1);
        for (int r = 0; r < granks && ok; r++) {
            const int64_t off = (int64_t)hr[2 * r], cnt = (int64_t)hr[2 * r + 1];
            ok = off >= 0 && cnt >= 0 && off + cnt <= E;
            chunk = std::max(chunk, cnt);
        }
        for (int r = 0; r < granks && ok; r++) {
            const int64_t off = (int64_t)hr[2 * r], cnt = (int64_t)hr[2 * r + 1];
            for (int64_t k = 0; k < cnt && ok; k++) {
                ok = cover[off + k]++ == 0;
                gpos[off + k] = (int)(r * chunk + k);
            }
        }
        for (int64_t e = 0; e < E && ok; e++) ok = cover[e] == 1;
        ok = ok && (int64_t)granks * chunk < (int64_t)(INT32_MAX >> 3);
        if (ok && chunk > 0) {
            plan.gather = true;
            plan.gchunk = (int)chunk;
        }
    }
    if (a.mode == M3S_GN_CALIB) {
        plan.K[0] = Kh[0];
        plan.K[1] = Kh[4];
        plan.K[2] = Kh[2];
        plan.K[3] = Kh[5];
    }

    const int npose = (int)(a.N - 1);
    std::vector<int> iopt, jopt;
    int rc = plan_pairs(hii, hjj, E, a.N, plan, iopt, jopt);
    if (rc) return rc;
    auto slot = [&](int r, int c) { return plan.slotmap[(size_t)r * npose + c]; };

    plan.ii_loc.resize(a.E_local);
    plan.jj_loc.resize(a.E_local);
    plan.blk_ptr.assign(plan.nblk + 1, 0);
    plan.grad_ptr.assign(std::max(npose, 0) + 1, 0);
    for (int pass = 0; pass < 2; pass++) {
        std::vector<int> bfill, gfill;
        if (pass == 1) {
            for (int k = 0; k < plan.nblk; k++) plan.blk_ptr[k + 1] += plan.blk_ptr[k];
            for (int k = 0; k < npose; k++) plan.grad_ptr[k + 1] += plan.grad_ptr[k];
            plan.blk_ent.assign(plan.blk_ptr[plan.nblk], 0);
            plan.blk_ref.assign(plan.gather ? 0 : plan.blk_ptr[plan.nblk], 0);
            plan.grad_ent.assign(plan.grad_ptr[npose], 0);
            bfill.assign(plan.blk_ptr.begin(), plan.blk_ptr.end() - 1);
            gfill.assign(plan.grad_ptr.begin(), plan.grad_ptr.end() - 1);
        }
        const int64_t nlist = plan.gather ? E : a.E_local;
        for (int64_t el = 0; el < nlist; el++) {
            const int64_t e = plan.gather ? el : a.edge_offset + el;
            const int64_t code = plan.gather ? gpos[e] : el;
            const int i = iopt[e], j = jopt[e];
            if (pass == 0 && !plan.gather) {
                plan.ii_loc[el] = i + 1;
                plan.jj_loc[el] = j + 1;
            }
            const int rr[4] = {i, i, j, j}, cc[4] = {i, j, i, j}, neg[4] = {0, 1, 1, 0};
            for (int b = 0; b < 4; b++) {
                if (rr[b] >= 0 && cc[b] >= 0 && rr[b] <= cc[b]) {
                    const int sl = slot(rr[b], cc[b]);
                    if (pass == 0) {
                        plan.blk_ptr[sl + 1]++;
                    } else {
                        const int type = (b == 0 || b == 3) ? 0 : (i == j ? (b == 1 ? 3 : 4) : (b == 1 ? 2 : 1));
                        if (!plan.gather) plan.blk_ref[bfill[sl]] = (int)(el << 3) | type;
                        plan.blk_ent[bfill[sl]++] = (int)(code << 1) | neg[b];
                    }
                }
            }
            if (i >= 0) {
                if (pass == 0) plan.grad_ptr[i + 1]++;
                else plan.grad_ent[gfill[i]++] = (int)(code << 1) | 1;
            }
            if (j >= 0) {
                if (pass == 0) plan.grad_ptr[j + 1]++;
                else plan.grad_ent[gfill[j]++] = (int)(code << 1);
            }
        }
    }
    if (plan.gather) {
        for (int64_t el = 0; el < a.E_local; el++) {
            plan.ii_loc[el] = iopt[a.edge_offset + el] + 1;
            plan.jj_loc[el] = jopt[a.edge_offset + el] + 1;
        }
        plan.blk_ref.clear();
    }
    return M3S_OK;
}


int env_int(const char* name, int dflt) {
    const char* e = getenv(name);
    return e ? atoi(e) : dflt;
}

namespace {
RoundPolicy fused_policy() {
    return {true, env_int("M3S_SPARSE_DCAP", 64), env_int("M3S_SPARSE_RMIN", 1),
            env_int("M3S_SPARSE_RMAX", 64),
            std::min(kTailPoseMax, env_int("M3S_SPARSE_TAILCAP", kTailPoseMax)),
            env_int("M3S_SPARSE_KMIN", 4), env_int("M3S_SPARSE_MMD", 1) != 0};
}
RoundPolicy multi_policy() {
    return {false, env_int("M3S_MULTI_DCAP", 32), env_int("M3S_MULTI_RMIN", 2),
            env_int("M3S_MULTI_RMAX", 64), 0, env_int("M3S_MULTI_KMIN", 4), env_int("M3S_MULTI_MMD", 0) != 0};
}
constexpr int kHybDfTailMax = 64;
constexpr int kHybDfTailDefault = 36;
bool hyb_core_df() { return env_int("M3S_HYB_CORE", 1) != 0; }
RoundPolicy hybrid_policy() {
    const bool df = hyb_core_df();
    return {false, env_int("M3S_HYB_DCAP", 64), env_int("M3S_HYB_RMIN", 1),
            env_int("M3S_HYB_RMAX", 64),
            std::min(df ? kHybDfTailMax : kTailPoseMax, env_int("M3S_HYB_TAILCAP", df ? kHybDfTailDefault : kTailPoseMax)),
            env_int("M3S_HYB_KMIN", 4), env_int("M3S_HYB_MMD", 1) != 0};
}
bool hyb_core_fits(const SparsePlan& p) {
    return hyb_core_df() ? p.ntail <= kHybDfTailMax : p.fused_tail;
}
}

int upload_sparse_plan(SparsePlan& sp, int npose, hipStream_t st) {
    size_t off = 0;
    auto take = [&](size_t bytes) {
        size_t o = off;
        off = align_up(off + std::max<size_t>(bytes, 8), 256);
        return o;
    };
    sp.bpad = (int)align_up((size_t)npose * 7, 49);
    sp.o_sys = take(sizeof(double) * ((size_t)sp.bpad + 49 * (size_t)sp.nblocks));
    sp.o_y = take(sizeof(double) * 7 * (size_t)npose);
    sp.o_L = take(sizeof(double) * std::max(kLStoreRec, 49) * sp.nodes.size());
    sp.o_W = take(sizeof(double) * 49 * (size_t)sp.nW);
    sp.o_xd = take(sizeof(double) * (size_t)std::max(sp.npad_tail, 1));
    if (sp.npad_tail > 0) {
        sp.o_dense = take(sizeof(double) * (size_t)(sp.npad_tail + kCholTile) * sp.npad_tail);
        sp.o_linv = take(chol_linv_bytes(sp.npad_tail));
    }
    sp.o_Lg = take(sp.fused_tail ? sizeof(double) * 49 * (size_t)sp.ntail * sp.ntail : 0);
    sp.o_dfcnt = take(sizeof(int) * (size_t)sp_rounds_df_words((int)sp.rounds.size()));
    if (sp.pcg) {
        sp.snap_bytes = 0;
        if (sp.pcg_lag >= 2) {
            sp.snap_bytes = (sp.npad_tail > 0 ? sp.o_linv + chol_linv_bytes(sp.npad_tail) : sp.o_xd) - sp.o_L;
            sp.o_snap = take(sp.snap_bytes);
        }
        sp.o_pcgx = take(sizeof(double) * (size_t)npose * 7 * sp.pcg_ldx);
        sp.o_pcgxt = take(sizeof(float) * (size_t)npose * 7 * sp.pcg_ldt);
        sp.o_gran = take(16 * 4 * (size_t)sp.pcg_nv);
    }
    std::vector<const std::vector<int>*> parts = {&sp.nodes, &sp.fptr, &sp.fronts, &sp.tail,
                                                  &sp.tmap, &sp.tg, &sp.tc, &sp.rtg, &sp.rc,
                                                  &sp.tc3, &sp.rc4, &sp.inl, &sp.apt, &sp.adj};
    size_t* offs[] = {&sp.i_nodes, &sp.i_fptr, &sp.i_fronts, &sp.i_tail, &sp.i_tmap, &sp.i_tg,
                      &sp.i_tc, &sp.i_rtg, &sp.i_rc, &sp.i_tc3, &sp.i_rc4, &sp.i_inl, &sp.i_apt, &sp.i_adj};
    auto len = [&](size_t k) { return parts[k] == &sp.inl ? sp.ninl : parts[k]->size(); };
    size_t n = 0;
    for (size_t k = 0; k < parts.size(); k++) {
        if (k == 4) {
            sp.i_rounds = n;
            n += 8 * sp.rounds.size();
        }
        if (parts[k] == &sp.inl) n = align_up(n, 4);
        if (parts[k] == &sp.adj) n = align_up(n, 2);
        *offs[k] = n;
        n += len(k);
    }
    sp.o_int = take(sizeof(int) * std::max<size_t>(n, 1));
    M3S_HIP_CHECK(hipMallocAsync((void**)&sp.dbuf, off, st));
    M3S_HIP_CHECK(hipMemsetAsync(sp.dbuf + sp.o_dfcnt, 0, sizeof(int) * (size_t)sp_rounds_df_words((int)sp.rounds.size()), st));
    if (sp.npad_tail > 0)
        M3S_HIP_CHECK(hipMemsetAsync(chol_ready_ptr(sp.dptr<double>(sp.o_linv), sp.npad_tail), 0,
                                     chol_ready_bytes(sp.npad_tail), st));
    if (sp.pcg)
        M3S_HIP_CHECK(hipMemsetAsync(sp.dbuf + sp.o_gran, 0, 16 * 4 * (size_t)sp.pcg_nv, st));
    if (n > 0) {
        int* h = reinterpret_cast<int*>(stagings().out.get(sizeof(int) * n));
        M3S_REQUIRE(h != nullptr, "gauss_newton: pinned host allocation failed");
        for (size_t k = 0; k < parts.size(); k++)
            if (len(k) > 0) std::memcpy(h + *offs[k], parts[k]->data(), sizeof(int) * len(k));
        int* hr = h + sp.i_rounds;
        for (const SpRound& R : sp.rounds) {
            const int v[8] = {R.node_begin, R.nnodes, R.tbeg, R.nbt, R.rbeg, R.nrt, R.wbeg, R.wcount};
            std::memcpy(hr, v, sizeof(v));
            hr += 8;
        }
        M3S_HIP_CHECK(stagings().out.upload(sp.dbuf + sp.o_int, reinterpret_cast<const char*>(h), sizeof(int) * n, st));
        M3S_HIP_CHECK(stagings().out.mark(st));
    }
    return M3S_OK;
}

int gn_order(const m3s_gn_args& a) {
    if (a.order == M3S_GN_ORDER_FAST || a.order == M3S_GN_ORDER_REFERENCE) return a.order;
    static const int env = [] {
        const char* e = getenv("M3S_GN_ORDER");
        if (e && (!strcmp(e, "reference") || !strcmp(e, "ref") || !strcmp(e, "2"))) return (int)M3S_GN_ORDER_REFERENCE;
        return (int)M3S_GN_ORDER_FAST;
    }();
    return env;
}

int validate(const m3s_gn_args& a) {
    M3S_REQUIRE(a.order >= M3S_GN_ORDER_DEFAULT && a.order <= M3S_GN_ORDER_REFERENCE,
                "gauss_newton: bad summation order %d", a.order);
    M3S_REQUIRE(a.mode == M3S_GN_POINTS || a.mode == M3S_GN_RAYS || a.mode == M3S_GN_CALIB,
                "gauss_newton: bad mode %d", a.mode);
    M3S_REQUIRE(a.contract == M3S_CONTRACT_NVCC || a.contract == M3S_CONTRACT_OFF ||
                    a.contract == M3S_CONTRACT_NVCC_RIGHT,
                "gauss_newton: unknown contraction convention %d", a.contract);
    M3S_REQUIRE(a.N >= 1 && a.HW >= 1, "gauss_newton: need N >= 1 poses and HW >= 1 points");
    M3S_REQUIRE(a.E_total >= 0 && a.E_local >= 0 && a.edge_offset >= 0 &&
                    a.edge_offset + a.E_local <= a.E_total,
                "gauss_newton: bad edge range");
    M3S_REQUIRE(a.HW < ((int64_t)1 << 31) && a.E_local < (1 << 30),
                "gauss_newton: sizes exceed int32 indexing");
    if (env_int("M3S_SOLVER_DENSE", 0) != 0 && a.order != M3S_GN_ORDER_REFERENCE)
        M3S_REQUIRE(7 * (a.N - 1) <= kMaxNpad,
                    "gauss_newton: %lld poses exceed the dense solve limit (%d unknowns)",
                    (long long)a.N, kMaxNpad);
    M3S_REQUIRE(a.mode != M3S_GN_CALIB || (a.K != nullptr && a.width > 0 && a.height > 0),
                "gauss_newton_calib: K / image size required");
    M3S_REQUIRE(a.Twc && a.Xs && a.Cs && a.dx, "gauss_newton: null pointer");
    if (a.E_total > 0) M3S_REQUIRE(a.ii && a.jj, "gauss_newton: null ii/jj");
    if (a.E_local > 0) M3S_REQUIRE(a.idx && a.valid && a.Q, "gauss_newton: null edge data");
    if (a.idx_b || a.valid_b || a.Q_b) {
        M3S_REQUIRE(a.idx_b && a.valid_b && a.Q_b, "gauss_newton: incomplete second edge half");
        M3S_REQUIRE(a.E_a >= 0 && a.E_a <= a.E_local, "gauss_newton: bad edge split E_a = %lld",
                    (long long)a.E_a);
    }
    const size_t need = make_layout(a.mode, a.N, a.HW, a.E_total, a.E_local).total;
    M3S_REQUIRE(a.ws != nullptr && a.ws_bytes >= need,
                "gauss_newton: workspace too small (%zu < %zu bytes)", a.ws_bytes, need);
    return M3S_OK;
}

Plan& tls_plan() {
    static thread_local Plan p;
    return p;
}
SparsePlan& tls_sparse_plan() {
    static thread_local SparsePlan sp;
    return sp;
}

namespace {
int pcg_from_for(int tiles) {
    const int v = env_int("M3S_PCG_FROM", 0);
    return v > 0 ? v : (tiles >= 8 ? 3 : 4);
}
int pcg_lag_for(int from) { return std::max(1, std::min(from, env_int("M3S_PCG_LAG", 2))); }
}
void choose_pcg(const m3s_gn_args& a, const Ctx& c, const Plan& plan, int npose, SparsePlan& sp) {
    sp.pcg = false;
    const int n = 7 * npose;
    const int mode = env_int("M3S_GN_PCG", 1);
    const int min_tiles = env_int("M3S_PCG_MIN_TILES", 1);
    const int tiles = sp.npad_tail / kCholTile;
    sp.pcg_from = pcg_from_for(tiles);
    sp.pcg_lag = pcg_lag_for(sp.pcg_from);
    if (mode == 0 || (mode == 1 && tiles < min_tiles) || c.ref_order || !sp.enabled || sp.fused ||
        (sp.hybrid && !sp.core_df) || a.max_iter <= sp.pcg_from || n > kPcgMaxN || n < 7)
        return;
    const int wg_cap = std::max(1, env_int("M3S_PCG_WG", 64));
    std::vector<int> deg((size_t)npose, 1);
    for (const auto& pr : plan.pairs) {
        deg[pr.first]++;
        deg[pr.second]++;
    }
    const int maxdeg = npose > 0 ? *std::max_element(deg.begin(), deg.end()) : 1;
    auto items = [&](int R) { return 7 * maxdeg * (R / 7 + 2); };
    auto pick = [&](bool ox) {
        int R = kPcgThreads / 64;
        auto fits = [&](int r) { return pcg_lds_bytes(n, r, items(r), ox) <= (size_t)kPcgMaxLds && (!ox || r <= kPcgMaxR); };
        if ((n + R - 1) / R > wg_cap && fits(2 * R)) R *= 2;
        return (n + R - 1) / R > 240 || !fits(R) ? 0 : R;
    };
    bool onex = env_int("M3S_PCG_ONEX", 0) != 0 && pick(true) > 0;
    const int R = pick(onex);
    if (R == 0) return;
    if (inverse_lds_bytes(sp.npad_tail) > (size_t)kPcgMaxLds) return;
    sp.pcg_nitem = items(R);
    sp.pcg = true;
    sp.pcg_R = R;
    sp.pcg_onex = onex;
    sp.pcg_nwg = (n + R - 1) / R;
    sp.pcg_ldx = (int)align_up((size_t)n, 16);
    sp.pcg_ldt = (int)align_up((size_t)n, 4);
    sp.pcg_nv = pcg_nv(n);
    sp.apt.assign((size_t)npose + 1, 0);
    for (const auto& pr : plan.pairs) {
        sp.apt[pr.first + 1]++;
        sp.apt[pr.second + 1]++;
    }
    for (int v = 0; v < npose; v++) sp.apt[v + 1] += sp.apt[v] + 1;
    sp.adj.assign(2 * (size_t)sp.apt[npose], 0);
    std::vector<int> fill(sp.apt.begin(), sp.apt.end() - 1);
    for (int v = 0; v < npose; v++) {
        sp.adj[2 * (size_t)fill[v]] = v;
        sp.adj[2 * (size_t)fill[v] + 1] = v;
        fill[v]++;
    }
    for (size_t k = 0; k < plan.pairs.size(); k++) {
        const int x = plan.pairs[k].first, y = plan.pairs[k].second, slot = npose + (int)k;
        sp.adj[2 * (size_t)fill[x]] = slot;
        sp.adj[2 * (size_t)fill[x]++ + 1] = y;
        sp.adj[2 * (size_t)fill[y]] = slot;
        sp.adj[2 * (size_t)fill[y]++ + 1] = x;
    }
}

void choose_sparse_plan(const Plan& plan, int npose, SparsePlan& sp) {
    const int choice = env_int("M3S_SOLVER", 0);
    const int max_fused_rounds = env_int("M3S_FUSED_MAX_ROUNDS", 3);
    const bool hybrid_on = env_int("M3S_HYBRID", 1) != 0;
    bool planned = false;
    if (choice == 0 && hybrid_on) {
        static thread_local SparsePlan probe;
        build_sparse_plan(plan.pairs, plan.nblk, npose, hybrid_policy(), probe, true);
        if ((int)probe.rounds.size() > max_fused_rounds) {
            const bool hyb = hyb_core_fits(probe) && npose <= solve_max_poses() &&
                             solve_lds_bytes((int)probe.nints_back) <= (size_t)kSolveMaxLds;
            build_sparse_plan(plan.pairs, plan.nblk, npose, hyb ? hybrid_policy() : multi_policy(), sp);
            sp.hybrid = hyb;
            planned = true;
        }
    }
    bool fused_ok = false, meta_fits = false;
    if (!planned) {
        build_sparse_plan(plan.pairs, plan.nblk, npose, fused_policy(), sp);
        meta_fits = solve_lds_bytes((int)sp.nints) <= (size_t)kSolveMaxLds;
        fused_ok = sp.fused && meta_fits && npose <= solve_max_poses() &&
                   (choice == 1 || (choice == 0 && (int)sp.rounds.size() <= max_fused_rounds));
    }
    if (env_int("M3S_SOLVE_DEBUG", 0) && !fused_ok && !planned)
        fprintf(stderr, "fused solve rejected: fused_tail %d (ntail %d) rounds %zu nints %zu meta_fits %d\n",
                (int)sp.fused, sp.ntail, sp.rounds.size(), sp.nints, (int)meta_fits);
    if (!fused_ok && !planned) {
        bool hyb = false;
        if (choice == 3 || (choice == 0 && hybrid_on)) {
            build_sparse_plan(plan.pairs, plan.nblk, npose, hybrid_policy(), sp);
            hyb = hyb_core_fits(sp) && npose <= solve_max_poses() &&
                  solve_lds_bytes((int)sp.nints_back) <= (size_t)kSolveMaxLds;
        }
        if (!hyb) build_sparse_plan(plan.pairs, plan.nblk, npose, multi_policy(), sp);
        sp.hybrid = hyb;
    }
    sp.core_df = hyb_core_df();
}

int plan_info(const int64_t* ii, const int64_t* jj, int64_t E, int64_t N, int32_t* info, int32_t* order,
              int32_t* round_ptr, int32_t round_cap) {
    M3S_REQUIRE(info != nullptr && N >= 1 && E >= 0 && (E == 0 || (ii != nullptr && jj != nullptr)),
                "gn_plan_info: bad arguments");
    Plan& plan = tls_plan();
    std::vector<int> iopt, jopt;
    int rc = plan_pairs(ii, jj, E, N, plan, iopt, jopt);
    if (rc) return rc;
    const int npose = (int)(N - 1);
    SparsePlan& sp = tls_sparse_plan();
    sp.reset();
    if (npose > 0) choose_sparse_plan(plan, npose, sp);
    info[0] = npose <= 0 ? -1 : sp.fused ? 0 : sp.hybrid ? 1 : 2;
    info[1] = (int32_t)sp.rounds.size();
    info[2] = (int32_t)sp.nodes.size();
    info[3] = sp.ntail;
    info[4] = sp.npad_tail;
    info[5] = (int32_t)plan.pairs.size();
    info[6] = (int32_t)sp.nints;
    info[7] = sp.npad_tail <= kMaxNpad ? 1 : 0;
    if (order) {
        std::copy(sp.nodes.begin(), sp.nodes.end(), order);
        std::copy(sp.tail.begin(), sp.tail.end(), order + sp.nodes.size());
    }
    if (round_ptr && round_cap >= (int32_t)sp.rounds.size() + 1) {
        for (size_t k = 0; k < sp.rounds.size(); k++) round_ptr[k] = sp.rounds[k].node_begin;
        round_ptr[sp.rounds.size()] = (int32_t)sp.nodes.size();
    }
    return M3S_OK;
}

}
```

mast3r-slam_amd/csrc/sparse_plan.h:

```cpp
#pragma once

#include <algorithm>
#include <cstdint>
#include <cstdlib>
#include <utility>
#include <vector>

#include "gn_kernels.h"

namespace m3s {

inline size_t sp_align_up(size_t x, size_t a) { return (x + a - 1) / a * a; }

struct SpRound {
    int node_begin, nnodes, tbeg, nbt, rbeg, nrt, wbeg, wcount;
};

struct SparsePlan {
    bool enabled = false;
    bool fused = false;
    bool fused_tail = false;
    bool hybrid = false;
    bool core_df = true;
    bool pcg = false, pcg_onex = false;
    int pcg_from = 0, pcg_lag = 0;
    int pcg_R = 0, pcg_nwg = 0, pcg_ldx = 0, pcg_ldt = 0, pcg_nv = 0, pcg_nitem = 0;
    size_t o_pcgx = 0, o_pcgxt = 0, o_gran = 0;
    size_t o_snap = 0, snap_bytes = 0;
    size_t o_dfcnt = 0;
    int nblocks = 0, nW = 0, ntail = 0, npad_tail = 0, zero_blk = 0;
    std::vector<SpRound> rounds;
    std::vector<int> nodes, fptr, fronts, tg, tc, rtg, rc, tail, tmap;
    std::vector<int> tc3, rc4;
    std::vector<int> inl;
    size_t ninl = 0;
    std::vector<int> apt, adj;
    char* dbuf = nullptr;
    size_t o_dense = 0, o_linv = 0;
    int bpad = 0;
    size_t o_sys = 0, o_y = 0, o_L = 0, o_W = 0, o_xd = 0, o_Lg = 0, o_int = 0;
    size_t i_nodes = 0, i_fptr = 0, i_fronts = 0, i_tg = 0, i_tc = 0, i_rtg = 0, i_rc = 0,
           i_tail = 0, i_tmap = 0, i_rounds = 0, i_tc3 = 0, i_rc4 = 0, i_inl = 0, i_apt = 0, i_adj = 0,
           nints = 0, nints_back = 0;
    template <typename T>
    T* dptr(size_t off) const { return reinterpret_cast<T*>(dbuf + off); }
    const int* iptr(size_t i) const { return reinterpret_cast<const int*>(dbuf + o_int) + i; }
    void reset() {
        SparsePlan fresh;
        for (auto v : {&SparsePlan::nodes, &SparsePlan::fptr, &SparsePlan::fronts, &SparsePlan::tg,
                       &SparsePlan::tc, &SparsePlan::rtg, &SparsePlan::rc, &SparsePlan::tail,
                       &SparsePlan::tmap, &SparsePlan::tc3, &SparsePlan::rc4, &SparsePlan::apt,
                       &SparsePlan::adj}) {
            (this->*v).clear();
            (fresh.*v).swap(this->*v);
        }
        fresh.inl.swap(inl);
        rounds.clear();
        fresh.rounds.swap(rounds);
        *this = std::move(fresh);
    }
};

struct RoundPolicy {
    bool fused;
    int dcap, rmin, rmax, tailcap, kmin;
    bool mmd;
};
inline void build_sparse_plan(const std::vector<std::pair<int, int>>& pairs, int nblk, int npose,
                              const RoundPolicy& pol, SparsePlan& sp, bool symbolic = false) {
    sp.reset();
    sp.nodes.reserve(npose);
    sp.fptr.reserve(npose + 1);
    const int dcap = pol.dcap, rmin = pol.rmin, rmax = pol.rmax, tailcap = pol.tailcap, kmin = pol.kmin;
    struct TC { int ki, kj; };
    struct Scratch {
        std::vector<uint64_t> adj, fmask;
        std::vector<int> deg, bidm, cand, chosen, cnt;
        std::vector<char> alive, blocked;
        std::vector<std::vector<int>> F;
        std::vector<TC> tcs, tcs2;
        std::vector<int> rcs, rcs2, fq;
    };
    static thread_local Scratch S;
    const int nw = (npose + 63) / 64;
    auto& adj = S.adj;
    auto& fmask = S.fmask;
    auto& deg = S.deg;
    adj.assign((size_t)npose * nw, 0);
    fmask.assign(nw, 0);
    deg.assign(npose, 0);
    auto row = [&](int x) { return &adj[(size_t)x * nw]; };
    auto unlink = [&](int x, int y) {
        uint64_t& w = row(x)[y >> 6];
        const uint64_t m = 1ull << (y & 63);
        if (w & m) {
            w &= ~m;
            deg[x]--;
        }
    };
    auto neighbours = [&](int x, std::vector<int>& out) {
        out.clear();
        const uint64_t* a = row(x);
        for (int k = 0; k < nw; k++)
            for (uint64_t w = a[k]; w; w &= w - 1) out.push_back(64 * k + __builtin_ctzll(w));
    };
    auto& bidm = S.bidm;
    if (!symbolic) bidm.assign((size_t)npose * npose, -1);
    for (size_t k = 0; k < pairs.size(); k++) {
        const int a = pairs[k].first, b = pairs[k].second;
        for (int t = 0; t < 2; t++) {
            const int x = t ? b : a, y = t ? a : b;
            uint64_t& w = row(x)[y >> 6];
            const uint64_t m = 1ull << (y & 63);
            if (!(w & m)) {
                w |= m;
                deg[x]++;
            }
        }
        if (!symbolic) bidm[(size_t)a * npose + b] = npose + (int)k;
    }
    sp.nblocks = nblk;
    auto block_of = [&](int x, int y) -> int {
        if (x == y) return x;
        int& id = bidm[(size_t)std::min(x, y) * npose + std::max(x, y)];
        if (id < 0) id = sp.nblocks++;
        return id;
// ... 250 lines not shown
```

mast3r-slam_amd/mast3r_slam_backends/__init__.py:

```python
from __future__ import annotations

import atexit
import ctypes
import os

import numpy as np
import torch

__all__ = [
    "gn_debug_flags",
    "iter_proj",
    "refine_matches",
    "gauss_newton_points",
    "gauss_newton_rays",
    "gauss_newton_calib",
    "track_sim3",
    "track_workspace_layout",
    "CholeskyError",
    "pointmap_update",
    "edge_confidence",
    "reconstruct",
    "ReconPass",
    "RECON_DTYPE",
    "recon_tile_points",
    "head_finish",
    "rope_2d",
    "rope_2d_pair",
    "RetrievalHandle",
    "retrieval_create",
    "retrieval_destroy",
    "retrieval_size",
    "retrieval_term_table",
    "retrieval_quantize",
    "retrieval_aggregate",
    "retrieval_query",
    "retrieval_add",
    "retrieval_image",
    "gn_plan_info",
    "library_path",
    "set_gn_order",
    "set_gn_contract",
    "lib",
]

_HERE = os.path.dirname(os.path.abspath(__file__))
library_path = os.environ.get(
    "M3S_BACKEND_LIB", os.path.join(os.path.dirname(_HERE), "lib", "libm3s_backend.so")
)

if not os.path.exists(library_path):
    raise ImportError(
        f"mast3r_slam_backends: HIP backend library not found at {library_path}; "
        "build it with `make -C mast3r-slam_amd` (or __graft_entry__.build())"
    )

lib = ctypes.CDLL(library_path)

_c_int64 = ctypes.c_int64
_vp = ctypes.c_void_p
_f = ctypes.c_float
_i = ctypes.c_int

lib.m3s_last_error.restype = ctypes.c_char_p
lib.m3s_shutdown.restype = None
atexit.register(lib.m3s_shutdown)
lib.m3s_version.restype = ctypes.c_char_p
lib.m3s_iter_proj.argtypes = [_vp] * 5 + [_c_int64] * 4 + [_i, _f, _f, _vp]
lib.m3s_iter_proj_ex.argtypes = [_vp] * 5 + [_c_int64] * 4 + [_i, _f, _f, _i, _vp]
lib.m3s_refine_matches_f16.argtypes = [_vp] * 4 + [_c_int64] * 5 + [_i, _i, _vp]
lib.m3s_refine_matches_f32.argtypes = [_vp] * 4 + [_c_int64] * 5 + [_i, _i, _vp]
lib.m3s_refine_matches_f64.argtypes = [_vp] * 4 + [_c_int64] * 5 + [_i, _i, _vp]
lib.m3s_match_workspace_bytes.argtypes = [_c_int64] * 4
lib.m3s_match_workspace_bytes.restype = ctypes.c_size_t
lib.m3s_match_iterative_proj.argtypes = ([_vp] * 5 + [_c_int64] * 4 + [_i, _f, _f, _f, _i, _i, _i]
                                         + [_vp, _vp, _vp, ctypes.c_size_t, _vp])

CONTRACT = {"nvcc": 0, "off": 1, "nvcc_right": 2}


def _contract(c):
    if c is None:
        return CONTRACT["nvcc"]
    if c not in CONTRACT:
        raise ValueError(f"unknown contraction convention {c!r} (expected one of {sorted(CONTRACT)})")
    return CONTRACT[c]
lib.m3s_gn_workspace_bytes.restype = ctypes.c_size_t
lib.m3s_gn_workspace_bytes.argtypes = [_i, _c_int64, _c_int64, _c_int64, _c_int64]
lib.m3s_gn_plan_info.argtypes = [_vp, _vp, _c_int64, _c_int64, _vp, _vp, _vp, ctypes.c_int32]


class GNArgs(ctypes.Structure):

    _fields_ = [
        ("mode", _i),
        ("Twc", _vp),
        ("Xs", _vp),
        ("Cs", _vp),
        ("ii", _vp),
        ("jj", _vp),
        ("idx", _vp),
        ("valid", _vp),
        ("Q", _vp),
        ("N", _c_int64),
        ("HW", _c_int64),
        ("E_total", _c_int64),
        ("E_local", _c_int64),
        ("edge_offset", _c_int64),
        ("sigma0", _f),
        ("sigma1", _f),
        ("C_thresh", _f),
        ("Q_thresh", _f),
        ("K", _vp),
        ("height", _i),
        ("width", _i),
        ("pixel_border", _i),
        ("z_eps", _f),
        ("max_iter", _i),
        ("delta_thresh", _f),
        ("dx", _vp),
        ("ws", _vp),
        ("ws_bytes", ctypes.c_size_t),
        ("comm", _vp),
        ("stream", _vp),
        ("order", _i),
        ("idx_b", _vp),
        ("valid_b", _vp),
        ("Q_b", _vp),
        ("E_a", _c_int64),
        ("contract", _i),
    ]


lib.m3s_gauss_newton.argtypes = [ctypes.POINTER(GNArgs)]
lib.m3s_gn_check.argtypes = [_vp]
lib.m3s_gn_build_system.argtypes = [ctypes.POINTER(GNArgs), _vp, _vp]
lib.m3s_gn_edge_hessians.argtypes = [ctypes.POINTER(GNArgs), _vp, _vp]
lib.m3s_comm_get_unique_id.argtypes = [_vp]
lib.m3s_comm_init.argtypes = [_vp, _i, _i, ctypes.POINTER(_vp)]
lib.m3s_comm_destroy.argtypes = [_vp]
lib.m3s_comm_size.argtypes = [_vp, ctypes.POINTER(_i)]
HOST_ALLREDUCE_FN = ctypes.CFUNCTYPE(_i, _vp, ctypes.POINTER(ctypes.c_double), ctypes.c_size_t)
lib.m3s_comm_init_host.argtypes = [HOST_ALLREDUCE_FN, _vp, _i, _i, ctypes.POINTER(_vp)]

GN_POINTS, GN_RAYS, GN_CALIB = 0, 1, 2

GN_ORDERS = {"default": 0, "fast": 1, "reference": 2}
_gn_order = [0]


_gn_contract = [0]


def set_gn_contract(contract: str) -> str:
    prev = [k for k, v in CONTRACT.items() if v == _gn_contract[0]][0]
    _gn_contract[0] = _contract(contract)
    return prev


def set_gn_order(order: str) -> str:
    if order not in GN_ORDERS:
        raise ValueError(f"unknown GN order {order!r} (expected one of {sorted(GN_ORDERS)})")
    prev = [k for k, v in GN_ORDERS.items() if v == _gn_order[0]][0]
    _gn_order[0] = GN_ORDERS[order]
    return prev


_DT_NAME = {
    torch.float32: "Float",
    torch.float16: "Half",
    torch.float64: "Double",
    torch.int64: "Long",
    torch.int32: "Int",
    torch.bool: "Bool",
    torch.uint8: "Byte",
}


def _check(t, name, dtype, ndim):
    if not isinstance(t, torch.Tensor):
        raise TypeError(f"{name} must be a torch.Tensor")
    if not t.is_contiguous():
        raise RuntimeError(f"{name} must be contiguous")
    dts = dtype if isinstance(dtype, tuple) else (dtype,)
    if t.dtype not in dts:
        raise RuntimeError(
            f"expected scalar type {_DT_NAME.get(dts[0], dts[0])} but found "
            f"{_DT_NAME.get(t.dtype, t.dtype)} ({name})"
        )
    if t.dim() != ndim:
        raise RuntimeError(f"packed_accessor32 expects {ndim} dims but tensor has {t.dim()} ({name})")


def _on_device(**tensors):
    dev = None
    for name, t in tensors.items():
        if t is None:
            continue
        if t.device.type != "cuda":
            raise RuntimeError(
                f"{name} must be a HIP (cuda) tensor: mast3r_slam_backends has no CPU path"
            )
        if dev is None:
            dev = t.device
        elif t.device != dev:
            raise RuntimeError(f"{name} must be on {dev}, got {t.device}")
    return dev


def _raise(rc, what):
    if rc != 0:
        msg = lib.m3s_last_error().decode(errors="replace")
        raise RuntimeError(f"{what}: {msg} (code {rc})")


def gn_plan_info(ii, jj, N):
    import numpy as np

    ii = np.ascontiguousarray(np.asarray(ii, dtype=np.int64))
    jj = np.ascontiguousarray(np.asarray(jj, dtype=np.int64))
    if ii.shape != jj.shape or ii.ndim != 1:
        raise ValueError("ii and jj must be 1-D of equal length")
    info = np.zeros(8, dtype=np.int32)
    npose = max(int(N) - 1, 0)
    order = np.zeros(max(npose, 1), dtype=np.int32)
    cap = npose + 2
    rptr = np.zeros(cap, dtype=np.int32)
    rc = lib.m3s_gn_plan_info(ii.ctypes.data, jj.ctypes.data, ii.shape[0], int(N), info.ctypes.data,
                              order.ctypes.data, rptr.ctypes.data, cap)
    _raise(rc, "gn_plan_info")
    rounds = int(info[1])
    return {"solver": {0: "fused", 1: "hybrid", 2: "multi"}.get(int(info[0])), "rounds": rounds,
            "eliminated": int(info[2]), "core_poses": int(info[3]), "core_unknowns_padded": int(info[4]),
            "pairs": int(info[5]), "plan_ints": int(info[6]), "core_fits": bool(info[7]),
            "order": order[:npose].tolist(), "round_ptr": rptr[:rounds + 1].tolist()}


def _stream(device):
    return ctypes.c_void_p(torch.cuda.current_stream(device).cuda_stream)


def _ptr(t):
    return ctypes.c_void_p(t.data_ptr()) if t is not None else ctypes.c_void_p(0)




def iter_proj(rays_img_with_grad, pts_3d_norm, p_init, max_iter, lambda_init, cost_thresh,
              contract=None):
    _check(rays_img_with_grad, "rays_img_with_grad", torch.float32, 4)
    _check(pts_3d_norm, "pts_3d_norm", torch.float32, 3)
    _check(p_init, "p_init", torch.float32, 3)
    dev = _on_device(rays_img_with_grad=rays_img_with_grad, pts_3d_norm=pts_3d_norm, p_init=p_init)
    B, H, W, C = rays_img_with_grad.shape
    if C != 9:
        raise RuntimeError(f"rays_img_with_grad must have 9 channels (ray, d/du, d/dv), got {C}")
    Bp, N = p_init.shape[0], p_init.shape[1]
    if p_init.shape[2] != 2 or pts_3d_norm.shape[2] != 3:
        raise RuntimeError("p_init must be [B,N,2] and pts_3d_norm [B,N,3]")
    if pts_3d_norm.shape[:2] != p_init.shape[:2] or Bp != B:
        raise RuntimeError("batch / point counts of rays_img_with_grad, pts_3d_norm, p_init differ")
    p_new = torch.zeros((Bp, N, 2), dtype=p_init.dtype, device=dev)
    converged = torch.zeros((Bp, N), dtype=torch.bool, device=dev)
    with torch.cuda.device(dev):
        rc = lib.m3s_iter_proj_ex(
            _ptr(rays_img_with_grad), _ptr(pts_3d_norm), _ptr(p_init), _ptr(p_new),
            _ptr(converged), B, H, W, N, int(max_iter), float(lambda_init),
            float(cost_thresh), _contract(contract), _stream(dev),
        )
    _raise(rc, "iter_proj")
    return [p_new, converged]


def refine_matches(D11, D21, p1, window_size, dilation_max):
    _check(D11, "D11", (torch.float16, torch.float32, torch.float64), 4)
    _check(D21, "D21", D11.dtype, 3)
    _check(p1, "p1", torch.int64, 3)
    dev = _on_device(D11=D11, D21=D21, p1=p1)
    B, H, W, F = D11.shape
    Bq, N = p1.shape[0], p1.shape[1]
    if p1.shape[2] != 2 or D21.shape[0] != Bq or D21.shape[1] != N or D21.shape[2] != F or Bq != B:
        raise RuntimeError("refine_matches: expected D11 [B,H,W,F], D21 [B,N,F], p1 [B,N,2]")
    p1_new = torch.zeros((Bq, N, 2), dtype=p1.dtype, device=dev)
    fn = {torch.float16: lib.m3s_refine_matches_f16, torch.float32: lib.m3s_refine_matches_f32,
          torch.float64: lib.m3s_refine_matches_f64}[D11.dtype]
    with torch.cuda.device(dev):
        rc = fn(
            _ptr(D11), _ptr(D21), _ptr(p1), _ptr(p1_new), B, H, W, N, F,
            int(window_size), int(dilation_max), _stream(dev),
        )
    _raise(rc, "refine_matches")
    return [p1_new]


def match_iterative_proj(X11, X21, D11, D21, idx_1_to_2_init, max_iter, lambda_init, cost_thresh,
                         dist_thresh, radius, dilation_max, contract=None):
    _check(X11, "X11", torch.float32, 4)
    _check(X21, "X21", torch.float32, 4)
    _check(D11, "D11", torch.float32, 4)
    _check(D21, "D21", torch.float32, 4)
    if idx_1_to_2_init is not None:
        _check(idx_1_to_2_init, "idx_1_to_2_init", torch.int64, 2)
    dev = _on_device(X11=X11, X21=X21, D11=D11, D21=D21, idx_1_to_2_init=idx_1_to_2_init)
    B, H, W, _ = X11.shape
    F = D11.shape[3]
    if X11.shape[3] != 3 or X21.shape != X11.shape or D21.shape != D11.shape or D11.shape[:3] != (B, H, W):
        raise RuntimeError("match_iterative_proj: expected X11, X21 [B,H,W,3] and D11, D21 [B,H,W,F]")
    if idx_1_to_2_init is not None and tuple(idx_1_to_2_init.shape) != (B, H * W):
        raise RuntimeError("match_iterative_proj: idx_1_to_2_init must be [B,H*W]")
    idx = torch.empty((B, H * W), dtype=torch.int64, device=dev)
    valid = torch.empty((B, H * W, 1), dtype=torch.bool, device=dev)
    nbytes = int(lib.m3s_match_workspace_bytes(B, H, W, F))
    ws = torch.empty((max(nbytes, 1),), dtype=torch.uint8, device=dev)
    with torch.cuda.device(dev):
        rc = lib.m3s_match_iterative_proj(
            _ptr(X11), _ptr(X21), _ptr(D11), _ptr(D21), _ptr(idx_1_to_2_init), B, H, W, F,
            int(max_iter), float(lambda_init), float(cost_thresh), float(dist_thresh), int(radius),
            int(dilation_max), _contract(contract), _ptr(idx), _ptr(valid), _ptr(ws), nbytes,
# ... 672 lines not shown


def retrieval_size(db):
    n = _c_int64()
    _raise(lib.m3s_retrieval_size(db.ptr, ctypes.byref(n)), "retrieval_size")
    return int(n.value)


def retrieval_quantize(db, feat, ma):
    dev, n = _retrieval_feat(db, feat, "retrieval_quantize")
    ma = int(ma)
    if not 1 <= ma <= min(RETRIEVAL_MA_MAX, db.K):
        raise RuntimeError(f"retrieval_quantize: ma = {ma} outside 1..{min(RETRIEVAL_MA_MAX, db.K)}")
    ids = torch.empty((n, ma), dtype=torch.int32, device=dev)
    with torch.cuda.device(dev):
        rc = lib.m3s_retrieval_quantize(db.ptr, _ptr(feat), n, ma, _ptr(ids), _stream(dev))
    _raise(rc, "retrieval_quantize")
    return ids


def retrieval_aggregate(db, feat, ids):
    dev, n = _retrieval_feat(db, feat, "retrieval_aggregate")
    _check(ids, "ids", torch.int32, 2)
    _on_device(feat=feat, ids=ids)
    ma = ids.shape[1]
    if ids.shape[0] != n or not 1 <= ma <= db.ma_query:
        raise RuntimeError(f"retrieval_aggregate: ids must be [n, 1..{db.ma_query}]")
    words = torch.zeros((n * ma,), dtype=torch.int32, device=dev)
    codes = torch.zeros((n * ma, db.W), dtype=torch.int32, device=dev)
    count = torch.zeros((1,), dtype=torch.int32, device=dev)
    with torch.cuda.device(dev):
        rc = lib.m3s_retrieval_aggregate(db.ptr, _ptr(feat), _ptr(ids), n, ma, _ptr(words),
                                         _ptr(codes), _ptr(count), _stream(dev))
    _raise(rc, "retrieval_aggregate")
    return words, codes, count


def retrieval_query(db, feat):
    dev, n = _retrieval_feat(db, feat, "retrieval_query")
    scores = torch.empty((retrieval_size(db),), dtype=torch.float64, device=dev)
    with torch.cuda.device(dev):
        rc = lib.m3s_retrieval_query(db.ptr, _ptr(feat), n, _ptr(scores), _stream(dev))
    _raise(rc, "retrieval_query")
    return scores


def retrieval_add(db, feat, reuse_last_query=False):
    dev, n = _retrieval_feat(db, feat, "retrieval_add")
    with torch.cuda.device(dev):
        rc = lib.m3s_retrieval_add(db.ptr, _ptr(feat), n, int(bool(reuse_last_query)), _stream(dev))
    _raise(rc, "retrieval_add")


def retrieval_image(db, m):
    if not isinstance(db, RetrievalHandle) or db.ptr is None:
        raise RuntimeError("retrieval_image: not an open retrieval database")
    dev = db.device
    row = db.max_feat * db.ma_build
    words = torch.empty((row,), dtype=torch.int32, device=dev)
    codes = torch.empty((row, db.W), dtype=torch.int32, device=dev)
    count = torch.empty((1,), dtype=torch.int32, device=dev)
    with torch.cuda.device(dev):
        rc = lib.m3s_retrieval_image(db.ptr, int(m), _ptr(words), _ptr(codes), _ptr(count), _stream(dev))
    _raise(rc, "retrieval_image")
    k = int(count.item())
    return words[:k], codes[:k]


def gn_check(device=None):
    dev = torch.device("cuda", torch.cuda.current_device()) if device is None else torch.device(device)
    _raise(lib.m3s_gn_check(_stream(dev)), "gauss_newton")


def gn_debug_flags() -> dict:
    f = (ctypes.c_int * 4)()
    lib.m3s_gn_debug_flags(f)
    q = (ctypes.c_int * 5)()
    lib.m3s_gn_pcg_stats(q)
    pl = (ctypes.c_int * 5)()
    lib.m3s_gn_pcg_plan(pl)
    return {"done": f[0], "fail": f[1], "packed": bool(f[2]), "ray_constrained": bool(f[3]),
            "pcg_planned": bool(q[3]), "pcg_runs": q[0], "pcg_steps": q[1], "pcg_fallbacks": q[2],
            "pcg_from": q[4], "pcg_R": pl[0], "pcg_nwg": pl[1], "pcg_onex": pl[2], "pcg_lag": pl[3],
            "pcg_nitem": pl[4]}


def version() -> str:
    return lib.m3s_version().decode()
```

Before: 567,100 keyframe-pair GN iters/s.

## Fuse sparse block assembly into accumulate kernel tail; refresh PCG inverse in-line

Adds an optional path in which the last block to finish reducing an edge also assembles the sparse Hessian blocks and gradient rows that edge feeds. It uses per-target atomic counters and a per-edge target map, so the separate assembly pass can be skipped. This path is off by default and needs M3S_GN_FUSE_ASSEMBLE to be set. Separately, once PCG is active, the preconditioner inverse refresh now runs on the main stream instead of the side stream unless M3S_PCG_REFRESH_SIDE is set. That trades overlap for less cross-stream synchronisation. It also adds a host API to inspect the assembly map.

```diff
diff --git a/include/m3s_backend.h b/include/m3s_backend.h
--- a/include/m3s_backend.h
+++ b/include/m3s_backend.h
@@ -62,6 +62,7 @@
 void m3s_gn_debug_flags(int* out4);
 void m3s_gn_pcg_stats(int* out5);
 void m3s_gn_pcg_plan(int* out5);
+int m3s_gn_fused_assemblies(void);
 
 int m3s_gn_check(void* stream);
 
@@ -137,6 +138,10 @@
 int m3s_gn_plan_info(const int64_t* ii, const int64_t* jj, int64_t E, int64_t N, int32_t* info,
                      int32_t* order, int32_t* round_ptr, int32_t round_cap);
 
+int m3s_gn_assemble_map(const int64_t* ii, const int64_t* jj, int64_t E, int64_t N, int32_t* sizes,
+                        int32_t* blk_ptr, int32_t* blk_ent, int32_t* grad_ptr, int32_t* grad_ent,
+                        int32_t* emap);
+
 int m3s_prof_begin(void);
 int m3s_prof_begin_accum(void);
 int m3s_prof_end(double* out , int* n_iter);
diff --git a/mast3r-slam_amd/csrc/edge_reduce.h b/mast3r-slam_amd/csrc/edge_reduce.h
--- a/mast3r-slam_amd/csrc/edge_reduce.h
+++ b/mast3r-slam_amd/csrc/edge_reduce.h
@@ -12,7 +12,8 @@
 __device__ __forceinline__ void edge_reduce_body(const float* __restrict__ partials, int nchunks,
                                                  const float* __restrict__ Twc,
                                                  const int* __restrict__ ii_loc,
-                                                 double* __restrict__ edgeblk, int e) {
+                                                 double* __restrict__ edgeblk, int e,
+                                                 bool publish = false) {
     const int tid = threadIdx.x;
     auto ldp = [](const float* q) -> float {
         if constexpr (COH) return __hip_atomic_load(q, __ATOMIC_RELAXED, __HIP_MEMORY_SCOPE_AGENT);
@@ -86,6 +87,10 @@
     }
     __syncthreads();
     double* out = edgeblk + (int64_t)e * kEdgeBlk;
+    auto stv = [publish](double* q, double v) {
+        if (publish) __hip_atomic_store(q, v, __ATOMIC_RELAXED, __HIP_MEMORY_SCOPE_AGENT);
+        else *q = v;
+    };
     if (tid < 28) {
         int a = 0, r = tid;
         while (r >= 7 - a) { r -= 7 - a; a++; }
@@ -93,13 +98,99 @@
         double s = 0.0;
 #pragma unroll
         for (int p = 0; p < 7; p++) s += AM[a][p] * A[b][p];
-        out[tid] = s;
+        stv(out + tid, s);
     } else if (tid < 35) {
         const int a = tid - 28;
         double s = 0.0;
 #pragma unroll
         for (int p = 0; p < 7; p++) s += A[a][p] * g[p];
-        out[tid] = s;
+        stv(out + tid, s);
+    }
+}
+
+template <bool COH>
+__device__ __forceinline__ double assemble_sum(const double* __restrict__ edgeblk,
+                                               const int* __restrict__ ent, int k0, int k1, int q) {
+    auto ldv = [](const double* p) -> double {
+        if constexpr (COH) return __hip_atomic_load(p, __ATOMIC_RELAXED, __HIP_MEMORY_SCOPE_AGENT);
+        return *p;
+    };
+    double acc = 0.0;
+    for (int k = k0; k < k1; k += 8) {
+        int code[8];
+        double v[8];
+#pragma unroll
+        for (int u = 0; u < 8; u++) code[u] = k + u < k1 ? ent[k + u] : 0;
+#pragma unroll
+        for (int u = 0; u < 8; u++) v[u] = k + u < k1 ? ldv(edgeblk + (int64_t)(code[u] >> 1) * kEdgeBlk + q) : 0.0;
+#pragma unroll
+        for (int u = 0; u < 8; u++)
+            if (k + u < k1) acc += (code[u] & 1) ? -v[u] : v[u];
+    }
+    return acc;
+}
+
+template <bool COH>
+__device__ __forceinline__ void assemble_block(const double* __restrict__ edgeblk,
+                                               const int* __restrict__ blk_ptr,
+                                               const int* __restrict__ blk_ent, int s, int lane,
+                                               double* __restrict__ blk) {
+    if (lane < 28) {
+        const double acc = assemble_sum<COH>(edgeblk, blk_ent, blk_ptr[s], blk_ptr[s + 1], lane);
+        int a = 0, r = lane;
+        while (r >= 7 - a) {
+            r -= 7 - a;
+            a++;
+        }
+        const int b = a + r;
+        blk[a * 7 + b] = acc;
+        blk[b * 7 + a] = acc;
+    }
+}
+
+template <bool COH>
+__device__ __forceinline__ void assemble_grad(const double* __restrict__ edgeblk,
+                                              const int* __restrict__ grad_ptr,
+                                              const int* __restrict__ grad_ent, int p, int lane,
+                                              double* __restrict__ row) {
+    if (lane < 7) row[lane] = assemble_sum<COH>(edgeblk, grad_ent, grad_ptr[p], grad_ptr[p + 1], 28 + lane);
+}
+
+__device__ __forceinline__ void fused_assemble_tail(const FuseAsm* __restrict__ fa, int e) {
+    __shared__ int s_tgt[kEdgeTargets];
+    const int tid = threadIdx.x;
+    asm volatile("s_waitcnt vmcnt(0)" ::: "memory");
+    __syncthreads();
+    const int nblk = fa->nblk;
+    if (tid < kEdgeTargets) {
+        const int code = fa->emap[(int64_t)e * kEdgeTargets + tid];
+        int done = -1;
+        if (code >= 0) {
+            const int t = code >> 1;
+            const int* ptr = t < nblk ? fa->blk_ptr + t : fa->grad_ptr + (t - nblk);
+            const int expect = ptr[1] - ptr[0];
+            if (__hip_atomic_fetch_add(fa->tcnt + t, 1, __ATOMIC_RELAXED, __HIP_MEMORY_SCOPE_AGENT) == expect - 1)
+                done = t;
+        }
+        s_tgt[tid] = done;
+    }
+    __syncthreads();
+    const int g = tid >> 5, lane = tid & 31;
+    if (g < kEdgeTargets) {
+        const int t = s_tgt[g];
+        if (t >= 0) {
+            if (t < nblk)
+                assemble_block<true>(fa->edgeblk, fa->blk_ptr, fa->blk_ent, t, lane,
+                                     fa->sys + fa->bpad + (int64_t)t * 49);
+            else
+                assemble_grad<true>(fa->edgeblk, fa->grad_ptr, fa->grad_ent, t - nblk, lane,
+                                    fa->sys + (int64_t)(t - nblk) * 7);
+            if (lane == 0) __hip_atomic_store(fa->tcnt + t, 0, __ATOMIC_RELAXED, __HIP_MEMORY_SCOPE_AGENT);
+        }
+    } else {
+        const int q = tid - 32 * kEdgeTargets;
+        for (int s = nblk + e; s < fa->nblocks; s += fa->nedge)
+            if (q < 49) fa->sys[fa->bpad + (int64_t)s * 49 + q] = 0.0;
     }
 }
 
diff --git a/mast3r-slam_amd/csrc/gn_accum.hip b/mast3r-slam_amd/csrc/gn_accum.hip
--- a/mast3r-slam_amd/csrc/gn_accum.hip
+++ b/mast3r-slam_amd/csrc/gn_accum.hip
@@ -873,7 +873,8 @@
     const int* __restrict__ ii_loc, const int* __restrict__ jj_loc, const int4* __restrict__ pack,
     AccParams P, const int4* __restrict__ sched, float* __restrict__ partials,
     const int* __restrict__ flags, const float* __restrict__ px, const int* __restrict__ pcnt,
-    int* __restrict__ ecnt, double* __restrict__ edgeblk, FirstSrc fs) {
+    int* __restrict__ ecnt, double* __restrict__ edgeblk, FirstSrc fs,
+    const FuseAsm* __restrict__ fuse_asm) {
     const int4 tk = sched[blockIdx.x];
     if (flags[kFlagDone]) return;
     const int e = tk.x, c = tk.y, ix = tk.z, jx = tk.w;
@@ -922,8 +923,10 @@
             s_last = __hip_atomic_fetch_add(ecnt + e, 1, __ATOMIC_RELAXED, __HIP_MEMORY_SCOPE_AGENT) == P.nchunks - 1;
         __syncthreads();
         if (s_last) {
-            edge_reduce_body<true>(partials, P.nchunks, Twc, ii_loc, edgeblk, e);
+            edge_reduce_body<true>(partials, P.nchunks, Twc, ii_loc, edgeblk, e, fuse_asm != nullptr);
             if (threadIdx.x == 0) __hip_atomic_store(ecnt + e, 0, __ATOMIC_RELAXED, __HIP_MEMORY_SCOPE_AGENT);
+            static_assert(kAccThreads >= 32 * kEdgeTargets + 49, "fused_assemble_tail's thread groups");
+            if (fuse_asm != nullptr) fused_assemble_tail(fuse_asm, e);
         }
     }
 }
@@ -991,7 +994,8 @@
                                const int* jj_loc, const int4* pack, const AccParams& P,
                                const int4* sched, float* partials, const int* flags, const float* px,
                                const int* pcnt, int* ecnt, double* edgeblk, const EdgeSrc* first_es,
-                               const float* Cs, const int* cok) {
+                               const float* Cs, const int* cok, const FuseAsm* fuse_asm) {
+    if (fuse_asm != nullptr && ecnt == nullptr) return hipErrorInvalidValue;
     if (P.HW > kPackedMaxHW) return hipErrorInvalidValue;
     if (first_es != nullptr) {
         if (px != nullptr) return hipErrorInvalidValue;
@@ -999,25 +1003,25 @@
         if (mode == GN_RAYS)
             hipLaunchKernelGGL((gn_accum_packed_kernel<GN_RAYS, false, false, true>), grid, dim3(kAccThreads), 0, st,
                                Twc, Xs, Zs, ii_loc, jj_loc, pack, P, sched, partials, flags, px, pcnt, ecnt,
-                               edgeblk, fs);
+                               edgeblk, fs, fuse_asm);
         else if (mode == GN_POINTS)
             hipLaunchKernelGGL((gn_accum_packed_kernel<GN_POINTS, false, false, true>), grid, dim3(kAccThreads), 0, st,
                                Twc, Xs, Zs, ii_loc, jj_loc, pack, P, sched, partials, flags, px, pcnt, ecnt,
-                               edgeblk, fs);
+                               edgeblk, fs, fuse_asm);
         else if (P.raycheck)
             hipLaunchKernelGGL((gn_accum_packed_kernel<GN_CALIB, false, true, true>), grid, dim3(kAccThreads), 0, st,
                                Twc, Xs, Zs, ii_loc, jj_loc, pack, P, sched, partials, flags, px, pcnt, ecnt,
-                               edgeblk, fs);
+                               edgeblk, fs, fuse_asm);
         else
             hipLaunchKernelGGL((gn_accum_packed_kernel<GN_CALIB, false, false, true>), grid, dim3(kAccThreads), 0, st,
                                Twc, Xs, Zs, ii_loc, jj_loc, pack, P, sched, partials, flags, px, pcnt, ecnt,
-                               edgeblk, fs);
+                               edgeblk, fs, fuse_asm);
         return hipGetLastError();
     }
     const FirstSrc fs0{};
 #define M3S_ACCP(MODE, CP, RC)                                                                       \
     hipLaunchKernelGGL((gn_accum_packed_kernel<MODE, CP, RC>), grid, dim3(kAccThreads), 0, st, Twc, Xs, Zs, \
-                       ii_loc, jj_loc, pack, P, sched, partials, flags, px, pcnt, ecnt, edgeblk, fs0)
+                       ii_loc, jj_loc, pack, P, sched, partials, flags, px, pcnt, ecnt, edgeblk, fs0, fuse_asm)
 #define M3S_ACCP2(MODE, CP) M3S_ACCP(MODE, CP, false)
     const bool cp = px != nullptr;
     if (mode == GN_RAYS) {
diff --git a/mast3r-slam_amd/csrc/gn_api.hip b/mast3r-slam_amd/csrc/gn_api.hip
--- a/mast3r-slam_amd/csrc/gn_api.hip
+++ b/mast3r-slam_amd/csrc/gn_api.hip
@@ -21,6 +21,7 @@
 int g_dbg_flags[4] = {0, 0, 0, 0};
 int g_dbg_pcg[5] = {0, 0, 0, 0, 0};
 int g_dbg_pcg_plan[5] = {0, 0, 0, 0, 0};
+int g_dbg_asm_fused = 0;
 
 void set_error(const char* fmt, ...) {
     char buf[1024];
@@ -104,6 +105,7 @@
     for (int k = 0; k < 5; k++) out5[k] = m3s::g_dbg_pcg[k];
 }
 
+extern "C" int m3s_gn_fused_assemblies(void) { return m3s::g_dbg_asm_fused; }
 extern "C" void m3s_gn_pcg_plan(int* out5) {
     for (int k = 0; k < 5; k++) out5[k] = m3s::g_dbg_pcg_plan[k];
 }
@@ -132,6 +134,12 @@
 extern "C" int m3s_gn_plan_info(const int64_t* ii, const int64_t* jj, int64_t E, int64_t N, int32_t* info,
                                 int32_t* order, int32_t* round_ptr, int32_t round_cap) {
     return m3s::plan_info(ii, jj, E, N, info, order, round_ptr, round_cap);
+}
+
+extern "C" int m3s_gn_assemble_map(const int64_t* ii, const int64_t* jj, int64_t E, int64_t N, int32_t* sizes,
+                                   int32_t* blk_ptr, int32_t* blk_ent, int32_t* grad_ptr, int32_t* grad_ent,
+                                   int32_t* emap) {
+    return m3s::assemble_map(ii, jj, E, N, sizes, blk_ptr, blk_ent, grad_ptr, grad_ent, emap);
 }
 
 extern "C" int m3s_gauss_newton(const m3s_gn_args* args) {
diff --git a/mast3r-slam_amd/csrc/gn_driver.hip b/mast3r-slam_amd/csrc/gn_driver.hip
--- a/mast3r-slam_amd/csrc/gn_driver.hip
+++ b/mast3r-slam_amd/csrc/gn_driver.hip
@@ -144,7 +144,9 @@
     put(L.blk_ref, p.blk_ref);
     put(L.grad_ptr, p.grad_ptr);
     put(L.grad_ent, p.grad_ent);
+    put(L.emap, p.emap);
     std::memset(h + (L.ecnt - lo), 0, sizeof(int) * (size_t)a.E_local);
+    std::memset(h + (L.tcnt - lo), 0, sizeof(int) * ((size_t)L.nblk_max + (size_t)std::max<int64_t>(a.N - 1, 0)));
     SchedGroups G;
     build_schedule_order(p.ii_loc, p.jj_loc, (int)std::max<int64_t>(a.N, 1), reinterpret_cast<int*>(h + (L.sorder - lo)), G);
     M3S_HIP_CHECK(stagings().ws.upload(c.ws + lo, h, L.sched - lo, c.st));
@@ -228,7 +230,23 @@
         M3S_REQUIRE(c.sp.npad_tail <= kMaxNpad,
                     "gauss_newton: the dense core of the elimination (%d unknowns) exceeds the "
                     "dense solve limit (%d)", c.sp.npad_tail, kMaxNpad);
-        rc = upload_sparse_plan(c.sp, npose, c.st);
+        c.fuse_asm = c.packed && !c.ref_order && a.comm == nullptr && c.sp.enabled && c.plan.asm_fusable &&
+                     a.E_local > 0 && env_int("M3S_GN_FUSE_REDUCE", 1) != 0 &&
+                     env_int("M3S_GN_FUSE_ASSEMBLE", 0) != 0;
+        FuseAsm fa{};
+        if (c.fuse_asm) {
+            fa.emap = c.at<int>(L.emap);
+            fa.tcnt = c.at<int>(L.tcnt);
+            fa.blk_ptr = c.at<int>(L.blk_ptr);
+            fa.blk_ent = c.at<int>(L.blk_ent);
+            fa.grad_ptr = c.at<int>(L.grad_ptr);
+            fa.grad_ent = c.at<int>(L.grad_ent);
+            fa.edgeblk = c.eblk_all();
+            fa.nblk = c.plan.nblk;
+            fa.npose = npose;
+            fa.nedge = (int)a.E_local;
+        }
+        rc = upload_sparse_plan(c.sp, npose, c.st, c.fuse_asm ? &fa : nullptr);
         if (rc) return rc;
         t3 = now();
     }
@@ -257,7 +275,8 @@
             M3S_HIP_CHECK(launch_retract(c.st, a.Twc, c.at<double>(L.x), a.dx, (int)a.N,
                                          a.delta_thresh, flags, a.contract));
         if (c.sp.pcg && (itr == from - lag || itr >= from) && itr + 1 < a.max_iter) {
-            rc = enqueue_inverse(a, c, itr < from - 1);
+            const bool in_line = itr >= from && env_int("M3S_PCG_REFRESH_SIDE", 0) == 0;
+            rc = enqueue_inverse(a, c, itr < from - 1, in_line);
             if (rc) return rc;
         }
         g_prof.mark(c.st);
@@ -302,6 +321,7 @@
         g_dbg_pcg[2] = hf[kFlagPcgFall];
         g_dbg_pcg[3] = c.sp.pcg ? 1 : 0;
         g_dbg_pcg[4] = c.sp.pcg ? c.sp.pcg_from : 0;
+        g_dbg_asm_fused = c.n_asm_fused;
         g_dbg_pcg_plan[0] = c.sp.pcg ? c.sp.pcg_R : 0;
         g_dbg_pcg_plan[1] = c.sp.pcg ? c.sp.pcg_nwg : 0;
         g_dbg_pcg_plan[2] = c.sp.pcg && c.sp.pcg_onex ? 1 : 0;
diff --git a/mast3r-slam_amd/csrc/gn_enqueue.hip b/mast3r-slam_amd/csrc/gn_enqueue.hip
--- a/mast3r-slam_amd/csrc/gn_enqueue.hip
+++ b/mast3r-slam_amd/csrc/gn_enqueue.hip
@@ -98,6 +98,11 @@
         const bool fuse_reduce = env_int("M3S_GN_FUSE_REDUCE", 1) != 0;
         const bool fused = c.packed && fuse_reduce;
         const bool was_first = c.packed && c.first_pack;
+        const SparsePlan& sp = c.sp;
+        const FuseAsm* fa = fused && c.fuse_asm && sp.dbuf != nullptr && sp.has_fa
+                                ? reinterpret_cast<const FuseAsm*>(sp.iptr(sp.i_fa)) : nullptr;
+        c.asm_fused = fa != nullptr;
+        c.n_asm_fused += c.asm_fused ? 1 : 0;
         if (c.packed) {
             M3S_HIP_CHECK(launch_accum_packed(a.mode, grid, c.st, a.Twc, a.Xs, c.at<float>(L.zs),
                                               c.at<int>(L.ii_loc), c.at<int>(L.jj_loc),
@@ -106,7 +111,7 @@
                                               c.compact ? c.at<float>(L.packx) : nullptr,
                                               c.at<int>(L.pcnt), fused ? c.at<int>(L.ecnt) : nullptr,
                                               c.eblk(), c.first_pack ? &c.es : nullptr,
-                                              a.Cs, c.at<int>(L.cok)));
+                                              a.Cs, c.at<int>(L.cok), fa));
             c.first_pack = false;
         } else
             M3S_HIP_CHECK(launch_accum(a.mode, c.vec, grid, c.st, a.Twc, a.Xs, a.Cs,
@@ -130,6 +135,10 @@
         if (rc) return rc;
     }
     c.gathered = false;
+    if (c.asm_fused) {
+        c.asm_fused = false;
+        return M3S_OK;
+    }
     const bool reduce = a.comm && !c.plan.gather;
     if (c.sp.enabled) {
         SparsePlan& sp = c.sp;
@@ -334,7 +343,7 @@
     return M3S_OK;
 }
 
-int enqueue_inverse(const m3s_gn_args& a, Ctx& c, bool snapshot) {
+int enqueue_inverse(const m3s_gn_args& a, Ctx& c, bool snapshot, bool in_line) {
     const SparsePlan& sp = c.sp;
     const size_t shift = snapshot ? sp.o_snap - sp.o_L : 0;
     if (snapshot) {
@@ -363,7 +372,7 @@
     v.ldt = sp.pcg_ldt;
     v.flags = c.at<int>(c.L.flags);
     static const bool side = env_int("M3S_PCG_SIDE", 1) != 0;
-    if (!side) {
+    if (!side || in_line) {
         M3S_HIP_CHECK(launch_sp_inverse(c.st, v));
         return M3S_OK;
     }
diff --git a/mast3r-slam_amd/csrc/gn_host.h b/mast3r-slam_amd/csrc/gn_host.h
--- a/mast3r-slam_amd/csrc/gn_host.h
+++ b/mast3r-slam_amd/csrc/gn_host.h
@@ -32,6 +32,7 @@
 
 extern int g_dbg_flags[4];
 extern int g_dbg_pcg[5];
+extern int g_dbg_asm_fused;
 extern int g_dbg_pcg_plan[5];
 
 struct Staging {
@@ -58,7 +59,7 @@
 
 struct Layout {
     size_t partials, edgeblk, compact, x, flags, ii_loc, jj_loc, blk_ptr, blk_ent, blk_ref, grad_ptr,
-        grad_ent, ecnt, cok, sorder, sched, pack, packx, pcnt, zs, twc_save, total;
+        grad_ent, emap, ecnt, tcnt, cok, sorder, sched, pack, packx, pcnt, zs, twc_save, total;
     int nchunks, npad, nblk_max;
 };
 Layout make_layout(int mode, int64_t N, int64_t HW, int64_t E_total, int64_t E_local);
@@ -70,6 +71,8 @@
     std::vector<int> blk_ptr, blk_ent;
     std::vector<int> blk_ref;
     std::vector<int> grad_ptr, grad_ent;
+    std::vector<int> emap;
+    bool asm_fusable = false;
     std::vector<int> slotmap;
     std::vector<std::pair<int, int>> pairs;
     float K[4] = {0, 0, 0, 0};
@@ -88,6 +91,9 @@
     bool pack_issued = false;
     bool acc_enqueued = false;
     bool gathered = false;
+    bool fuse_asm = false;
+    bool asm_fused = false;
+    int n_asm_fused = 0;
     bool first_pack = false;
     RefParams R;
     Layout L;
@@ -148,7 +154,9 @@
 int build_plan(const m3s_gn_args& a, hipStream_t st, Plan& plan, const std::function<int()>& before_wait = {});
 void choose_sparse_plan(const Plan& plan, int npose, SparsePlan& sp);
 void choose_pcg(const m3s_gn_args& a, const Ctx& c, const Plan& plan, int npose, SparsePlan& sp);
-int upload_sparse_plan(SparsePlan& sp, int npose, hipStream_t st);
+int upload_sparse_plan(SparsePlan& sp, int npose, hipStream_t st, const FuseAsm* fa = nullptr);
+int assemble_map(const int64_t* ii, const int64_t* jj, int64_t E, int64_t N, int32_t* sizes, int32_t* blk_ptr,
+                 int32_t* blk_ent, int32_t* grad_ptr, int32_t* grad_ent, int32_t* emap);
 int plan_info(const int64_t* ii, const int64_t* jj, int64_t E, int64_t N, int32_t* info, int32_t* order,
               int32_t* round_ptr, int32_t round_cap);
 
@@ -157,7 +165,7 @@
 int enqueue_accumulate(const m3s_gn_args& a, Ctx& c);
 int enqueue_assembly(const m3s_gn_args& a, Ctx& c);
 int enqueue_solve(const m3s_gn_args& a, Ctx& c, bool fallback = false);
-int enqueue_inverse(const m3s_gn_args& a, Ctx& c, bool snapshot);
+int enqueue_inverse(const m3s_gn_args& a, Ctx& c, bool snapshot, bool in_line = false);
 int enqueue_pcg(const m3s_gn_args& a, Ctx& c);
 
 int setup(const m3s_gn_args& a, Ctx& c, bool early_pack = false);
diff --git a/mast3r-slam_amd/csrc/gn_kernels.h b/mast3r-slam_amd/csrc/gn_kernels.h
--- a/mast3r-slam_amd/csrc/gn_kernels.h
+++ b/mast3r-slam_amd/csrc/gn_kernels.h
@@ -16,6 +16,7 @@
 constexpr int kNaccPad = 36;
 constexpr int kEdgeBlk = 36;
 constexpr int kCholTile = 64;
+constexpr int kEdgeTargets = 6;
 constexpr int64_t kPackedMaxHW = int64_t(1) << 28;
 
 constexpr int kFlagDone = 0;
@@ -32,6 +33,20 @@
 __device__ __forceinline__ bool solve_skipped(const int* flags) {
     return (flags[kFlagDone] | flags[kFlagSkipSolve]) != 0;
 }
+
+struct FuseAsm {
+    const int* emap;
+    int* tcnt;
+    const int* blk_ptr;
+    const int* blk_ent;
+    const int* grad_ptr;
+    const int* grad_ent;
+    const double* edgeblk;
+    double* sys;
+    int nblk, nblocks, npose, bpad;
+    int nedge, pad_;
+};
+static_assert(sizeof(FuseAsm) % 8 == 0, "FuseAsm is uploaded as ints at an 8-byte boundary");
 
 struct EdgeSrc {
     const int64_t* idx[2];
@@ -107,7 +122,7 @@
                                const int4* sched, float* partials, const int* flags, const float* px,
                                const int* pcnt, int* ecnt = nullptr, double* edgeblk = nullptr,
                                const EdgeSrc* first_es = nullptr, const float* Cs = nullptr,
-                               const int* cok = nullptr);
+                               const int* cok = nullptr, const FuseAsm* fuse_asm = nullptr);
 hipError_t launch_edge_reduce(int E_local, hipStream_t st, const float* partials, int nchunks,
                               const float* Twc, const int* ii_loc, double* edgeblk,
                               const int* flags);
diff --git a/mast3r-slam_amd/csrc/gn_kernels.hip b/mast3r-slam_amd/csrc/gn_kernels.hip
--- a/mast3r-slam_amd/csrc/gn_kernels.hip
+++ b/mast3r-slam_amd/csrc/gn_kernels.hip
@@ -75,50 +75,12 @@
     const int s = blockIdx.x;
     const int tid = threadIdx.x;
     if (s < nblk) {
-        if (tid < 28) {
-            double acc = 0.0;
-            const int k1 = blk_ptr[s + 1];
-            for (int k = blk_ptr[s]; k < k1; k += 8) {
-                int code[8];
-                double v[8];
-#pragma unroll
-                for (int u = 0; u < 8; u++) code[u] = k + u < k1 ? blk_ent[k + u] : 0;
-#pragma unroll
-                for (int u = 0; u < 8; u++) v[u] = k + u < k1 ? edgeblk[(int64_t)(code[u] >> 1) * kEdgeBlk + tid] : 0.0;
-#pragma unroll
-                for (int u = 0; u < 8; u++)
-                    if (k + u < k1) acc += (code[u] & 1) ? -v[u] : v[u];
-            }
-            int a = 0, r = tid;
-            while (r >= 7 - a) {
-                r -= 7 - a;
-                a++;
-            }
-            const int b = a + r;
-            double* blk = out + bpad + (int64_t)s * 49;
-            blk[a * 7 + b] = acc;
-            blk[b * 7 + a] = acc;
-        }
+        assemble_block<false>(edgeblk, blk_ptr, blk_ent, s, tid, out + bpad + (int64_t)s * 49);
     } else if (s < nblocks) {
         if (tid < 49) out[bpad + (int64_t)s * 49 + tid] = 0.0;
     } else {
         const int p = s - nblocks;
-        if (p < npose && tid < 7) {
-            double acc = 0.0;
-            const int k1 = grad_ptr[p + 1];
-            for (int k = grad_ptr[p]; k < k1; k += 8) {
-                int code[8];
-                double v[8];
-#pragma unroll
-                for (int u = 0; u < 8; u++) code[u] = k + u < k1 ? grad_ent[k + u] : 0;
-#pragma unroll
-                for (int u = 0; u < 8; u++) v[u] = k + u < k1 ? edgeblk[(int64_t)(code[u] >> 1) * kEdgeBlk + 28 + tid] : 0.0;
-#pragma unroll
-                for (int u = 0; u < 8; u++)
-                    if (k + u < k1) acc += (code[u] & 1) ? -v[u] : v[u];
-            }
-            out[p * 7 + tid] = acc;
-        }
+        if (p < npose) assemble_grad<false>(edgeblk, grad_ptr, grad_ent, p, tid, out + (int64_t)p * 7);
     }
 }
 
diff --git a/mast3r-slam_amd/csrc/gn_plan.hip b/mast3r-slam_amd/csrc/gn_plan.hip
--- a/mast3r-slam_amd/csrc/gn_plan.hip
+++ b/mast3r-slam_amd/csrc/gn_plan.hip
@@ -136,7 +136,9 @@
     L.blk_ref = take(sizeof(int) * (size_t)E_local * 4);
     L.grad_ptr = take(sizeof(int) * ((size_t)npose + 1));
     L.grad_ent = take(sizeof(int) * (size_t)std::max(E_local, E_total) * 2);
+    L.emap = take(sizeof(int) * (size_t)E_local * kEdgeTargets);
     L.ecnt = take(sizeof(int) * (size_t)E_local);
+    L.tcnt = take(sizeof(int) * ((size_t)L.nblk_max + (size_t)npose));
     L.sorder = take(sizeof(int) * (size_t)E_local);
     L.sched = take(sizeof(int) * 4 * (size_t)E_local * L.nchunks);
     if (env_int("M3S_GN_COMPACT", 0) != 0) {
@@ -239,6 +241,73 @@
     }
     return M3S_OK;
 }
+
+void plan_lists(Plan& plan, const std::vector<int>& iopt, const std::vector<int>& jopt, const std::vector<int>& gpos,
+                int64_t E, int64_t E_local, int64_t edge_offset, int npose) {
+    auto slot = [&](int r, int c) { return plan.slotmap[(size_t)r * npose + c]; };
+    plan.ii_loc.resize(E_local);
+    plan.jj_loc.resize(E_local);
+    plan.blk_ptr.assign(plan.nblk + 1, 0);
+    plan.grad_ptr.assign(std::max(npose, 0) + 1, 0);
+    for (int pass = 0; pass < 2; pass++) {
+        std::vector<int> bfill, gfill;
+        if (pass == 1) {
+            for (int k = 0; k < plan.nblk; k++) plan.blk_ptr[k + 1] += plan.blk_ptr[k];
+            for (int k = 0; k < npose; k++) plan.grad_ptr[k + 1] += plan.grad_ptr[k];
+            plan.blk_ent.assign(plan.blk_ptr[plan.nblk], 0);
+            plan.blk_ref.assign(plan.gather ? 0 : plan.blk_ptr[plan.nblk], 0);
+            plan.grad_ent.assign(plan.grad_ptr[npose], 0);
+            bfill.assign(plan.blk_ptr.begin(), plan.blk_ptr.end() - 1);
+            gfill.assign(plan.grad_ptr.begin(), plan.grad_ptr.end() - 1);
+            plan.emap.assign(plan.gather ? 0 : (size_t)E_local * kEdgeTargets, -1);
+        }
+        const int64_t nlist = plan.gather ? E : E_local;
+        for (int64_t el = 0; el < nlist; el++) {
+            const int64_t e = plan.gather ? el : edge_offset + el;
+            const int64_t code = plan.gather ? gpos[e] : el;
+            const int i = iopt[e], j = jopt[e];
+            if (pass == 0 && !plan.gather) {
+                plan.ii_loc[el] = i + 1;
+                plan.jj_loc[el] = j + 1;
+            }
+            int* em = (pass == 1 && !plan.gather) ? &plan.emap[(size_t)el * kEdgeTargets] : nullptr;
+            const int rr[4] = {i, i, j, j}, cc[4] = {i, j, i, j}, neg[4] = {0, 1, 1, 0};
+            for (int b = 0; b < 4; b++) {
+                if (rr[b] >= 0 && cc[b] >= 0 && rr[b] <= cc[b]) {
+                    const int sl = slot(rr[b], cc[b]);
+                    if (pass == 0) {
+                        plan.blk_ptr[sl + 1]++;
+                    } else {
+                        const int type = (b == 0 || b == 3) ? 0 : (i == j ? (b == 1 ? 3 : 4) : (b == 1 ? 2 : 1));
+                        if (!plan.gather) plan.blk_ref[bfill[sl]] = (int)(el << 3) | type;
+                        if (em) *em++ = (sl << 1) | neg[b];
+                        plan.blk_ent[bfill[sl]++] = (int)(code << 1) | neg[b];
+                    }
+                }
+            }
+            if (i >= 0) {
+                if (pass == 0) plan.grad_ptr[i + 1]++;
+                else plan.grad_ent[gfill[i]++] = (int)(code << 1) | 1;
+                if (em) *em++ = ((plan.nblk + i) << 1) | 1;
+            }
+            if (j >= 0) {
+                if (pass == 0) plan.grad_ptr[j + 1]++;
+                else plan.grad_ent[gfill[j]++] = (int)(code << 1);
+                if (em) *em++ = (plan.nblk + j) << 1;
+            }
+        }
+    }
+    if (plan.gather) {
+        for (int64_t el = 0; el < E_local; el++) {
+            plan.ii_loc[el] = iopt[edge_offset + el] + 1;
+            plan.jj_loc[el] = jopt[edge_offset + el] + 1;
+        }
+        plan.blk_ref.clear();
+    }
+    plan.asm_fusable = !plan.gather && E_local > 0;
+    for (int k = 0; k < plan.nblk && plan.asm_fusable; k++) plan.asm_fusable = plan.blk_ptr[k + 1] > plan.blk_ptr[k];
+    for (int k = 0; k < npose && plan.asm_fusable; k++) plan.asm_fusable = plan.grad_ptr[k + 1] > plan.grad_ptr[k];
+}
 }
 
 double g_plan_sync_us = 0;
@@ -331,62 +400,7 @@
     std::vector<int> iopt, jopt;
     int rc = plan_pairs(hii, hjj, E, a.N, plan, iopt, jopt);
     if (rc) return rc;
-    auto slot = [&](int r, int c) { return plan.slotmap[(size_t)r * npose + c]; };
-
-    plan.ii_loc.resize(a.E_local);
-    plan.jj_loc.resize(a.E_local);
-    plan.blk_ptr.assign(plan.nblk + 1, 0);
-    plan.grad_ptr.assign(std::max(npose, 0) + 1, 0);
-    for (int pass = 0; pass < 2; pass++) {
-        std::vector<int> bfill, gfill;
-        if (pass == 1) {
-            for (int k = 0; k < plan.nblk; k++) plan.blk_ptr[k + 1] += plan.blk_ptr[k];
-            for (int k = 0; k < npose; k++) plan.grad_ptr[k + 1] += plan.grad_ptr[k];
-            plan.blk_ent.assign(plan.blk_ptr[plan.nblk], 0);
-            plan.blk_ref.assign(plan.gather ? 0 : plan.blk_ptr[plan.nblk], 0);
-            plan.grad_ent.assign(plan.grad_ptr[npose], 0);
-            bfill.assign(plan.blk_ptr.begin(), plan.blk_ptr.end() - 1);
-            gfill.assign(plan.grad_ptr.begin(), plan.grad_ptr.end() - 1);
-        }
-        const int64_t nlist = plan.gather ? E : a.E_local;
-        for (int64_t el = 0; el < nlist; el++) {
-            const int64_t e = plan.gather ? el : a.edge_offset + el;
-            const int64_t code = plan.gather ? gpos[e] : el;
-            const int i = iopt[e], j = jopt[e];
-            if (pass == 0 && !plan.gather) {
-                plan.ii_loc[el] = i + 1;
-                plan.jj_loc[el] = j + 1;
-            }
-            const int rr[4] = {i, i, j, j}, cc[4] = {i, j, i, j}, neg[4] = {0, 1, 1, 0};
-            for (int b = 0; b < 4; b++) {
-                if (rr[b] >= 0 && cc[b] >= 0 && rr[b] <= cc[b]) {
-                    const int sl = slot(rr[b], cc[b]);
-                    if (pass == 0) {
-                        plan.blk_ptr[sl + 1]++;
-                    } else {
-                        const int type = (b == 0 || b == 3) ? 0 : (i == j ? (b == 1 ? 3 : 4) : (b == 1 ? 2 : 1));
-                        if (!plan.gather) plan.blk_ref[bfill[sl]] = (int)(el << 3) | type;
-                        plan.blk_ent[bfill[sl]++] = (int)(code << 1) | neg[b];
-                    }
-                }
-            }
-            if (i >= 0) {
-                if (pass == 0) plan.grad_ptr[i + 1]++;
-                else plan.grad_ent[gfill[i]++] = (int)(code << 1) | 1;
-            }
-            if (j >= 0) {
-                if (pass == 0) plan.grad_ptr[j + 1]++;
-                else plan.grad_ent[gfill[j]++] = (int)(code << 1);
-            }
-        }
-    }
-    if (plan.gather) {
-        for (int64_t el = 0; el < a.E_local; el++) {
-            plan.ii_loc[el] = iopt[a.edge_offset + el] + 1;
-            plan.jj_loc[el] = jopt[a.edge_offset + el] + 1;
-        }
-        plan.blk_ref.clear();
-    }
+    plan_lists(plan, iopt, jopt, gpos, E, a.E_local, a.edge_offset, npose);
     return M3S_OK;
 }
 
@@ -422,7 +436,7 @@
 }
 }
 
-int upload_sparse_plan(SparsePlan& sp, int npose, hipStream_t st) {
+int upload_sparse_plan(SparsePlan& sp, int npose, hipStream_t st, const FuseAsm* fa) {
     size_t off = 0;
     auto take = [&](size_t bytes) {
         size_t o = off;
@@ -467,6 +481,12 @@
         if (parts[k] == &sp.adj) n = align_up(n, 2);
         *offs[k] = n;
         n += len(k);
+    }
+    sp.has_fa = fa != nullptr;
+    if (fa) {
+        n = align_up(n, 2);
+        sp.i_fa = n;
+        n += sizeof(FuseAsm) / sizeof(int);
     }
     sp.o_int = take(sizeof(int) * std::max<size_t>(n, 1));
     M3S_HIP_CHECK(hipMallocAsync((void**)&sp.dbuf, off, st));
@@ -486,6 +506,13 @@
             const int v[8] = {R.node_begin, R.nnodes, R.tbeg, R.nbt, R.rbeg, R.nrt, R.wbeg, R.wcount};
             std::memcpy(hr, v, sizeof(v));
             hr += 8;
+        }
+        if (fa) {
+            FuseAsm f = *fa;
+            f.sys = sp.dptr<double>(sp.o_sys);
+            f.nblocks = sp.nblocks;
+            f.bpad = sp.bpad;
+            std::memcpy(h + sp.i_fa, &f, sizeof(f));
         }
         M3S_HIP_CHECK(stagings().out.upload(sp.dbuf + sp.o_int, reinterpret_cast<const char*>(h), sizeof(int) * n, st));
         M3S_HIP_CHECK(stagings().out.mark(st));
@@ -651,6 +678,29 @@
     sp.core_df = hyb_core_df();
 }
 
+int assemble_map(const int64_t* ii, const int64_t* jj, int64_t E, int64_t N, int32_t* sizes, int32_t* blk_ptr,
+                 int32_t* blk_ent, int32_t* grad_ptr, int32_t* grad_ent, int32_t* emap) {
+    M3S_REQUIRE(sizes != nullptr && N >= 1 && E >= 0 && (E == 0 || (ii != nullptr && jj != nullptr)),
+                "gn_assemble_map: bad arguments");
+    Plan& plan = tls_plan();
+    std::vector<int> iopt, jopt;
+    int rc = plan_pairs(ii, jj, E, N, plan, iopt, jopt);
+    if (rc) return rc;
+    const int npose = (int)(N - 1);
+    plan.gather = false;
+    plan_lists(plan, iopt, jopt, {}, E, E, 0, npose);
+    sizes[0] = plan.nblk;
+    sizes[1] = (int32_t)plan.blk_ent.size();
+    sizes[2] = (int32_t)plan.grad_ent.size();
+    sizes[3] = plan.asm_fusable ? 1 : 0;
+    if (blk_ptr) std::copy(plan.blk_ptr.begin(), plan.blk_ptr.end(), blk_ptr);
+    if (blk_ent) std::copy(plan.blk_ent.begin(), plan.blk_ent.end(), blk_ent);
+    if (grad_ptr) std::copy(plan.grad_ptr.begin(), plan.grad_ptr.end(), grad_ptr);
+    if (grad_ent) std::copy(plan.grad_ent.begin(), plan.grad_ent.end(), grad_ent);
+    if (emap) std::copy(plan.emap.begin(), plan.emap.end(), emap);
+    return M3S_OK;
+}
+
 int plan_info(const int64_t* ii, const int64_t* jj, int64_t E, int64_t N, int32_t* info, int32_t* order,
               int32_t* round_ptr, int32_t round_cap) {
     M3S_REQUIRE(info != nullptr && N >= 1 && E >= 0 && (E == 0 || (ii != nullptr && jj != nullptr)),
diff --git a/mast3r-slam_amd/csrc/sparse_plan.h b/mast3r-slam_amd/csrc/sparse_plan.h
--- a/mast3r-slam_amd/csrc/sparse_plan.h
+++ b/mast3r-slam_amd/csrc/sparse_plan.h
@@ -42,6 +42,8 @@
     size_t i_nodes = 0, i_fptr = 0, i_fronts = 0, i_tg = 0, i_tc = 0, i_rtg = 0, i_rc = 0,
            i_tail = 0, i_tmap = 0, i_rounds = 0, i_tc3 = 0, i_rc4 = 0, i_inl = 0, i_apt = 0, i_adj = 0,
            nints = 0, nints_back = 0;
+    bool has_fa = false;
+    size_t i_fa = 0;
     template <typename T>
     T* dptr(size_t off) const { return reinterpret_cast<T*>(dbuf + off); }
     const int* iptr(size_t i) const { return reinterpret_cast<const int*>(dbuf + o_int) + i; }
diff --git a/mast3r-slam_amd/mast3r_slam_backends/__init__.py b/mast3r-slam_amd/mast3r_slam_backends/__init__.py
--- a/mast3r-slam_amd/mast3r_slam_backends/__init__.py
+++ b/mast3r-slam_amd/mast3r_slam_backends/__init__.py
@@ -37,6 +37,7 @@
     "retrieval_add",
     "retrieval_image",
     "gn_plan_info",
+    "gn_assemble_map",
     "library_path",
     "set_gn_order",
     "set_gn_contract",
@@ -87,6 +88,8 @@
 lib.m3s_gn_workspace_bytes.restype = ctypes.c_size_t
 lib.m3s_gn_workspace_bytes.argtypes = [_i, _c_int64, _c_int64, _c_int64, _c_int64]
 lib.m3s_gn_plan_info.argtypes = [_vp, _vp, _c_int64, _c_int64, _vp, _vp, _vp, ctypes.c_int32]
+lib.m3s_gn_fused_assemblies.restype = ctypes.c_int
+lib.m3s_gn_assemble_map.argtypes = [_vp, _vp, _c_int64, _c_int64] + [_vp] * 6
 
 
 class GNArgs(ctypes.Structure):
@@ -233,6 +236,30 @@
             "eliminated": int(info[2]), "core_poses": int(info[3]), "core_unknowns_padded": int(info[4]),
             "pairs": int(info[5]), "plan_ints": int(info[6]), "core_fits": bool(info[7]),
             "order": order[:npose].tolist(), "round_ptr": rptr[:rounds + 1].tolist()}
+
+
+def gn_assemble_map(ii, jj, N):
+    import numpy as np
+
+    ii = np.ascontiguousarray(np.asarray(ii, dtype=np.int64))
+    jj = np.ascontiguousarray(np.asarray(jj, dtype=np.int64))
+    if ii.shape != jj.shape or ii.ndim != 1:
+        raise ValueError("ii and jj must be 1-D of equal length")
+    E, npose = ii.shape[0], max(int(N) - 1, 0)
+    sizes = np.zeros(4, dtype=np.int32)
+    blk_ptr = np.zeros(npose + E + 1, dtype=np.int32)
+    blk_ent = np.zeros(4 * E + 1, dtype=np.int32)
+    grad_ptr = np.zeros(npose + 1, dtype=np.int32)
+    grad_ent = np.zeros(2 * E + 1, dtype=np.int32)
+    emap = np.full((max(E, 1), 6), -1, dtype=np.int32)
+    rc = lib.m3s_gn_assemble_map(ii.ctypes.data, jj.ctypes.data, E, int(N), sizes.ctypes.data,
+                                 blk_ptr.ctypes.data, blk_ent.ctypes.data, grad_ptr.ctypes.data,
+                                 grad_ent.ctypes.data, emap.ctypes.data)
+    _raise(rc, "gn_assemble_map")
+    nblk = int(sizes[0])
+    return {"nblk": nblk, "fusable": bool(sizes[3]), "blk_ptr": blk_ptr[:nblk + 1].copy(),
+            "blk_ent": blk_ent[:int(sizes[1])].copy(), "grad_ptr": grad_ptr[:npose + 1].copy(),
+            "grad_ent": grad_ent[:int(sizes[2])].copy(), "emap": emap[:E].copy()}
 
 
 def _stream(device):
@@ -1071,7 +1098,7 @@
     return {"done": f[0], "fail": f[1], "packed": bool(f[2]), "ray_constrained": bool(f[3]),
             "pcg_planned": bool(q[3]), "pcg_runs": q[0], "pcg_steps": q[1], "pcg_fallbacks": q[2],
             "pcg_from": q[4], "pcg_R": pl[0], "pcg_nwg": pl[1], "pcg_onex": pl[2], "pcg_lag": pl[3],
-            "pcg_nitem": pl[4]}
+            "pcg_nitem": pl[4], "fused_assemblies": lib.m3s_gn_fused_assemblies()}
 
 
 def version() -> str:
```

Result: no change. 569,000 keyframe-pair GN iters/s, median of 6 (+0.3%).
